# graphic-goose/ferreus_rbf_rs

Measured on AMD Instinct MI355X. Metric: BBFMM matvecs/s, higher is better.
Workload: dtype f64; 1 GPU; 10000000 uniform 3D points, LinearRbf, order 7, 1 rhs, adaptive sparse tree, ACA eps=1e-7, set_weights + evaluate at the sources; points=10000000, kernel=LinearRbf, order=7, nrhs=1, parallelism=single GPU

## Files before the change

### ferreus_rbf_rs_amd/_lib.py

```python
from __future__ import annotations

import ctypes
import os

HERE = os.path.dirname(os.path.abspath(__file__))
LIB_PATH = os.environ.get("FERREUS_BBFMM_HIP_LIB") or os.path.join(HERE, "libferreus_bbfmm_hip.so")

OK, POINT_OUTSIDE_TREE, KERNEL_NO_GRADIENTS, BAD_ARGUMENT, DEVICE_ERROR, UNSUPPORTED, CALLBACK_FAILED = range(7)
FLAG_HOST_ONLY = 1
FLAG_M2L_SHARED_BASIS = 2
FLAG_DIRECT_SMALL_W_LEAVES = 4
FLAG_DETERMINISTIC = 8
N_PHASES = 11
PHASE_NAMES = ["gather", "P2M", "M2M", "M2L_stage1", "M2L_stage2", "P2L", "L2L", "P2P", "M2P",
               "L2P", "scatter"]

c_i32, c_i64, c_f64, c_u32 = ctypes.c_int32, ctypes.c_int64, ctypes.c_double, ctypes.c_uint32
c_p = ctypes.c_void_p


class Params(ctypes.Structure):
    _fields_ = [("max_points_per_cell", c_i64), ("compression_type", c_i32),
                ("epsilon", c_f64), ("eval_chunk_size", c_i64)]

# ... 40 lines not shown
    "bbfmm_build_isosurfaces_ex": (ctypes.c_int, [c_p, c_p, c_f64, c_p, c_i32, c_p, c_p, c_i64, c_i32, c_p]),
    "bbfmm_isosurfaces_from_values_ex": (ctypes.c_int, [c_p, c_p, c_p, c_f64, c_p, c_i32, c_i64, c_i32, c_p]),
    "bbfmm_isosurface_stats": (ctypes.c_int, [c_p, c_i32, c_p]),
    "bbfmm_build_isosurfaces_opts": (ctypes.c_int, [c_p, c_p, c_f64, c_p, c_i32, c_p, c_p, c_p, c_p]),
    "bbfmm_isosurfaces_from_values_opts": (ctypes.c_int, [c_p, c_p, c_p, c_f64, c_p, c_i32, c_p, c_p]),
    "bbfmm_isosurfaces_from_fields_opts": (ctypes.c_int, [c_p, c_i32, c_p, c_i32, c_p, c_f64, c_p, c_i32, c_p, c_p, c_p]),
    "bbfmm_isosurfaces_from_function_opts": (ctypes.c_int, [c_p, c_p, c_p, c_p, c_f64, c_p, c_i32, c_p, c_p]),
    "bbfmm_debug_evaluate_fields": (ctypes.c_int, [c_p, c_i32, c_p, c_i32, c_p, c_i64, c_i64, c_p, c_p, c_i64]),
    "bbfmm_debug_field_program": (ctypes.c_int, [c_i32, c_i32, c_p, c_p, c_p, c_i32, c_p, c_p, c_i64, c_p, c_p]),
    "bbfmm_isosurface_finish_mesh": (ctypes.c_int, [c_p, c_p, c_i64, c_p, c_i64, c_p, c_p]),
    "bbfmm_isosurface_finish_stats": (ctypes.c_int, [c_p, c_i32, c_p]),
    "bbfmm_isosurface_close_mesh": (ctypes.c_int, [c_p, c_p, c_i64, c_p, c_i64, c_p, ctypes.c_double, c_i32, c_p]),
    "bbfmm_isosurface_closure_stats": (ctypes.c_int, [c_p, c_i32, c_p]),
    "bbfmm_debug_closure_triangulate": (ctypes.c_int, [c_i32, c_i32, c_p, c_p, c_p, c_i64, c_p, c_i64, c_p, c_i64, ctypes.c_double,
                                                       ctypes.c_double, c_i64, c_p, c_p, c_i64, c_p, c_p, c_p, c_i64]),
    "bbfmm_debug_orient2d": (ctypes.c_int, [c_p, c_i64, c_p]),
    "bbfmm_isosurface_follow_stats": (ctypes.c_int, [c_p, c_i32, c_p]),
    "bbfmm_isosurface_follow_times": (ctypes.c_int, [c_p, c_i32, c_p]),
    "bbfmm_isosurface_follow_bricks": (ctypes.c_int, [c_p, c_i32, c_p, c_p]),
    "bbfmm_isosurface_intersection_stats": (ctypes.c_int, [c_p, c_i32, c_p]),
    "bbfmm_isosurface_self_intersections": (ctypes.c_int, [c_p, c_p, c_i64, c_p, c_i64, c_p, c_p]),
    "bbfmm_isosurface_intersection_ids": (ctypes.c_int, [c_p, c_i32, c_p, c_p]),
    "bbfmm_isosurface_triangle_pair": (ctypes.c_int, [c_p, c_p, c_p, c_p, c_p, c_p]),
    "bbfmm_isosurface_clip_triangle": (ctypes.c_int, [c_p, c_p, c_p, c_p, c_p]),
    "bbfmm_isosurface_topology": (ctypes.c_int, [ctypes.c_uint32, c_p, c_p, c_p]),
    "bbfmm_isosurface_cluster_tables": (ctypes.c_int, [c_p, c_p, c_p]),
    "bbfmm_isosurface_curvature_tables": (ctypes.c_int, [c_p, c_p, c_p]),
    "bbfmm_isosurface_curvature_weight": (ctypes.c_int, [c_p, c_p, c_i32, c_p, c_p, c_p, c_p]),
    "bbfmm_isosurface_curvature_stats": (ctypes.c_int, [c_p, c_i32, c_p]),
    "bbfmm_isosurface_count": (c_i32, [c_p]),
    "bbfmm_isosurface_size": (ctypes.c_int, [c_p, c_i32, c_p, c_p]),
    "bbfmm_isosurface_copy": (ctypes.c_int, [c_p, c_i32, c_p, c_p]),
    "bbfmm_isosurface_error": (ctypes.c_char_p, [c_p]),
    "bbfmm_isosurface_destroy": (None, [c_p]),
    "bbfmm_prepare_target_subset": (ctypes.c_int, [c_p, c_p, c_i64]),
    "bbfmm_fast_matrix_vector_product": (ctypes.c_int, [c_p, c_p, c_i64, c_i64, c_p, c_i64, c_p,
                                                        c_i64, c_f64, c_p]),
    "bbfmm_matvec_device": (ctypes.c_int, [c_p, c_p, c_i64, c_i32, c_p, c_i64, c_i32]),
    "bbfmm_target_subset_create": (ctypes.c_int, [c_p, c_p, c_i64, c_p]),
    "bbfmm_matvec_subset_device": (ctypes.c_int, [c_p, c_i32, c_p, c_p, c_i32]),
    "bbfmm_stream": (c_p, [c_p]),
    "bbfmm_set_partition": (ctypes.c_int, [c_p, c_i32, c_i32]),
    "bbfmm_partition_row_count": (c_i64, [c_p]),
    "bbfmm_partition_rows": (ctypes.c_int, [c_p, c_p]),
    "bbfmm_partition_coarse_count": (c_i64, [c_p]),
    "bbfmm_matvec_partition_upward": (ctypes.c_int, [c_p, c_p, c_i64, c_i32, c_p, c_p]),
    "bbfmm_matvec_partition_finish": (ctypes.c_int, [c_p, c_p, c_p, c_i64, c_i32, c_p]),
    "bbfmm_partition_world": (c_i32, [c_p]),
    "bbfmm_partition_rank": (c_i32, [c_p]),
    "bbfmm_partition_bounds": (ctypes.c_int, [c_p, c_i32, c_p]),
    "bbfmm_matvec_partition_finish_sorted": (ctypes.c_int, [c_p, c_p, c_p, c_i64, c_p]),
    "bbfmm_partition_scatter": (ctypes.c_int, [c_p, c_p, c_i32, c_i32, c_i64, c_i32, c_p, c_i64]),
    "bbfmm_debug_partition_upward_counts": (ctypes.c_int, [c_p, c_p, c_p, c_p]),
    "bbfmm_debug_host_copy_rates": (ctypes.c_int, [c_i64, c_p]),
    "bbfmm_get_tree_stats": (ctypes.c_int, [c_p, c_p]),
    "bbfmm_tree_built_on_device": (ctypes.c_int, [c_p]),
    "bbfmm_last_evaluate_at_sources": (ctypes.c_int, [c_p]),
    "bbfmm_debug_targets_are_sources": (ctypes.c_int, [c_p, c_p, c_i64, c_i64]),
    "bbfmm_debug_rows_of_sources": (ctypes.c_int, [c_p, c_p, c_i64, c_i64, c_p]),
    "bbfmm_get_cells": (ctypes.c_int, [c_p, c_p, c_p]),
    "bbfmm_get_leaf_sources": (ctypes.c_int, [c_p, c_p, c_p]),
    "bbfmm_get_list": (ctypes.c_int, [c_p, ctypes.c_char, c_p, c_p, c_p]),
    "bbfmm_get_m2l_ranks": (ctypes.c_int, [c_p, c_p, c_p]),
    "bbfmm_get_m2l_operator": (ctypes.c_int, [c_p, c_i32, c_i32, c_p]),
    "bbfmm_get_m2l_factors": (ctypes.c_int, [c_p, c_i32, c_i32, c_p, c_p]),
    "bbfmm_get_permutation_tables": (ctypes.c_int, [c_p, c_p, c_p, c_p, c_p, c_p]),
    "bbfmm_points_to_leaves": (ctypes.c_int, [c_p, c_p, c_i64, c_i64, c_p, c_p]),
    "bbfmm_set_profiling": (ctypes.c_int, [c_p, c_i32]),
    "bbfmm_get_phase_ms": (ctypes.c_int, [c_p, c_p, c_p]),
    "bbfmm_reset_phase_ms": (ctypes.c_int, [c_p]),
    "bbfmm_mfma_f64_selftest": (ctypes.c_int, [c_p, c_p, c_p]),
    "bbfmm_fp64_valu_selftest": (ctypes.c_int, [c_p, c_p]),
    "bbfmm_debug_kernel_values": (ctypes.c_int, [c_i32, c_i32, ctypes.c_double, ctypes.c_double, c_p, c_i64, c_p, c_p, c_p]),
    "bbfmm_debug_math": (ctypes.c_int, [c_i32, c_i32, c_p, c_i64, c_p, c_p]),
    "bbfmm_debug_dense_m2m": (ctypes.c_int, [c_p, c_i32, c_p]),
    "bbfmm_debug_apply_m2l_tables_host": (ctypes.c_int, [c_p, c_p, c_p]),
    "bbfmm_debug_m2l_variants": (ctypes.c_int, [c_p, c_p, c_p]),
    "bbfmm_debug_m2l_pairs": (ctypes.c_int, [c_p, c_p, c_i64, c_p, c_p]),
    "bbfmm_debug_m2l_pairs_axes": (ctypes.c_int, [c_p, c_p, c_i64, c_p]),
    "bbfmm_debug_m2l_pairs_stage2": (ctypes.c_int, [c_p, c_p, c_i64, c_p, c_p]),
    "bbfmm_debug_m2l_pairs_axes_stage2": (ctypes.c_int, [c_p, c_p, c_i64, c_p]),
    "bbfmm_debug_m2l_table_digests": (ctypes.c_int, [c_p, c_p, c_i32, c_p, c_p, c_i32, c_p]),
    "bbfmm_debug_m2l_s2_last_ksplit": (ctypes.c_int, [c_p, c_p]),
    "bbfmm_debug_m2l_parity_len": (ctypes.c_int, [c_p, c_p]),
    "bbfmm_debug_get_coefficients": (ctypes.c_int, [c_p, ctypes.c_char, c_i32, c_p]),
    "bbfmm_debug_morton_encode": (ctypes.c_uint64, [c_i32, c_p, ctypes.c_uint64]),
    "bbfmm_debug_morton_decode": (None, [c_i32, ctypes.c_uint64, c_p, c_p]),
    "bbfmm_debug_morton_neighbours": (c_i32, [c_i32, ctypes.c_uint64, c_p]),
    "bbfmm_debug_direction_vectors": (c_i32, [c_i32, c_p]),
    "bbfmm_debug_reference_vectors": (ctypes.c_int, [c_p, c_p, c_p]),
    "bbfmm_givens_rotation": (None, [c_f64, c_f64, c_p, c_p, c_p]),
    "bbfmm_fgmres": (ctypes.c_int, [c_i64, c_p, c_p, c_p, c_p, c_p, c_p, c_i32, c_i32, c_i32, c_f64,
                                    c_p, c_p, c_p, c_p, c_p]),
    "bbfmm_schwarz_ddm_solver": (ctypes.c_int, [c_i64, c_p, c_p, c_p, c_p, c_p, c_i32, c_i32, c_f64,
                                                c_p, c_p, c_p, c_p, c_p]),
    "bbfmm_rbf_system_apply": (ctypes.c_int, [c_p, c_p, c_p, c_i64]),
    "bbfmm_rbf_system_device_create": (ctypes.c_int, [c_p, c_i64, c_p, c_i64, c_f64, c_p]),
    "bbfmm_rbf_system_device_destroy": (None, [c_p]),
    "bbfmm_rbf_system_apply_device": (ctypes.c_int, [c_p, c_p, c_p, c_i64, c_p]),
    "bbfmm_fgmres_device": (ctypes.c_int, [c_i64, c_p, c_p, c_p, c_p, c_p, c_p, c_i32, c_i32, c_i32, c_f64,
                                           c_p, c_p, c_p, c_p, c_p, c_p]),
    "bbfmm_schwarz_ddm_solver_device": (ctypes.c_int, [c_i64, c_p, c_p, c_p, c_p, c_p, c_i32, c_i32, c_f64,
                                                       c_p, c_p, c_p, c_p, c_p, c_p]),
    "bbfmm_debug_solver_vector_op": (ctypes.c_int, [c_i32, c_i32, c_i64, c_p, c_p, c_p, c_f64, c_i32, c_p, c_i32, c_p, c_p]),
    "bbfmm_ddm_params_defaults": (None, [c_p]),
    "bbfmm_ddm_params_for_points": (None, [c_i64, c_p]),
    "bbfmm_ddm_build": (ctypes.c_int, [c_p, c_i64, c_i32, c_i64, c_p, c_p]),
    "bbfmm_ddm_destroy": (None, [c_p]),
    "bbfmm_ddm_num_levels": (c_i32, [c_p]),
    "bbfmm_ddm_level_size": (c_i64, [c_p, c_i32]),
    "bbfmm_ddm_level_points": (ctypes.c_int, [c_p, c_i32, c_p]),
    "bbfmm_ddm_num_domains": (c_i64, [c_p, c_i32]),
    "bbfmm_ddm_domain_size": (c_i64, [c_p, c_i32, c_i64]),
    "bbfmm_ddm_domain": (ctypes.c_int, [c_p, c_i32, c_i64, c_p, c_p, c_p]),
    "bbfmm_schwarz_create": (ctypes.c_int, [c_p, c_p, c_i64, c_i32, c_i64, c_p, c_p, c_p]),
    "bbfmm_schwarz_create_sharded": (ctypes.c_int, [c_p, c_p, c_i64, c_i32, c_i64, c_p, c_p, c_i32, c_i32, c_p, c_i64, c_p, c_p, c_p]),
    "bbfmm_schwarz_factor_bytes": (c_i64, [c_p]),
    "bbfmm_schwarz_domains_owned": (c_i64, [c_p, c_i32, ctypes.POINTER(c_i64), ctypes.POINTER(c_i64)]),
    "bbfmm_schwarz_destroy": (None, [c_p]),
    "bbfmm_schwarz_basis_size": (c_i64, [c_p]),
    "bbfmm_schwarz_num_levels": (c_i32, [c_p]),
    "bbfmm_schwarz_monomial_matrix": (c_p, [c_p]),
    "bbfmm_debug_evaluate_monomials": (ctypes.c_int, [c_p, c_i64, c_i32, c_i64, c_i32, c_p, c_p, c_p]),
    "bbfmm_schwarz_apply": (ctypes.c_int, [c_p, c_p, c_p, c_i64]),
    "bbfmm_schwarz_apply_device": (ctypes.c_int, [c_p, c_p, c_p, c_i64, c_p]),
    "bbfmm_schwarz_debug_trace_steps": (c_i32, [c_p]),
    "bbfmm_schwarz_debug_apply_trace": (ctypes.c_int, [c_p, c_p, c_p, c_i64, c_i32, c_p, c_p, c_p, c_p, c_p]),
    "bbfmm_schwarz_debug_ortho_matrix": (c_p, [c_p]),
    "bbfmm_schwarz_level_size": (c_i64, [c_p, c_i32]),
    "bbfmm_schwarz_level_points": (ctypes.c_int, [c_p, c_i32, c_p]),
    "bbfmm_schwarz_debug_level_solve": (ctypes.c_int, [c_p, c_i32, c_p, c_p, c_i64, c_i32]),
    "bbfmm_ddm_debug_level_create": (ctypes.c_int, [c_p, c_i64, c_i32, c_i64, c_i64, c_p, c_p, c_p, c_p, c_i32, c_i32, c_p]),
    "bbfmm_ddm_debug_level_destroy": (None, [c_p]),
    "bbfmm_ddm_debug_level_info": (ctypes.c_int, [c_p, c_p]),
    "bbfmm_ddm_debug_level_layout": (ctypes.c_int, [c_p, c_p, c_p, c_p, c_p, c_p]),
    "bbfmm_ddm_debug_level_assembled": (ctypes.c_int, [c_p, c_p]),
    "bbfmm_ddm_debug_level_factor": (ctypes.c_int, [c_p, c_p]),
    "bbfmm_ddm_debug_level_solve": (ctypes.c_int, [c_p, c_p, c_p, c_i64, c_i32]),
    "bbfmm_schwarz_create_ex": (ctypes.c_int, [c_p, c_p, c_i64, c_i32, c_i64, c_p, c_i64, c_p, c_p, c_p]),
    "bbfmm_schwarz_create_sharded_ex": (ctypes.c_int, [c_p, c_p, c_i64, c_i32, c_i64, c_p, c_i64, c_p, c_p, c_i32, c_i32, c_p, c_i64,
                                                       c_p, c_p, c_p]),
    "bbfmm_ddm_debug_level_create_ex": (ctypes.c_int, [c_p, c_i64, c_i32, c_i64, c_p, c_i64, c_i64, c_p, c_p, c_p, c_p, c_i32, c_i32,
                                                       c_p]),
    "bbfmm_global_trend_transform": (ctypes.c_int, [c_i32, c_p, c_p, c_p, c_p]),
    "bbfmm_duplicate_cutoff_distance": (ctypes.c_int, [c_p, c_f64, c_p]),
    "bbfmm_remove_duplicates": (ctypes.c_int, [c_p, c_i64, c_i32, c_i64, c_f64, c_i32, c_p, c_p, c_p]),
    "bbfmm_debug_interpolant_terms": (ctypes.c_int, [c_i32, c_i32, c_p, c_p, c_i64, c_i64, c_p, c_i64, c_p, c_i64, c_p, c_i64]),
    "bbfmm_evaluate_interpolant": (ctypes.c_int, [c_p, c_i32, c_i32, c_p, c_i64, c_i32, c_i64, c_p, c_i64, c_i64, c_p, c_f64,
                                                  c_p, c_i64, c_p, c_i64, c_p]),
    "bbfmm_evaluate_device": (ctypes.c_int, [c_p, c_i32, c_p, c_i64, c_i64, c_p, c_p, c_i64, c_p, c_i64, c_p, c_p]),
    "bbfmm_evaluate_grid": (ctypes.c_int, [c_p, c_i32, c_p, c_p, c_p, c_i64, c_p, c_i64, c_p, c_p]),
    "bbfmm_evaluate_grid_stats": (ctypes.c_int, [c_p, c_p]),
    "bbfmm_debug_grid_coords": (ctypes.c_int, [c_i32, c_p, c_i64, c_i64, c_p, c_i64]),
    "bbfmm_debug_split_runs": (ctypes.c_int, [c_i32, c_p, c_p, c_p, c_i64, c_i32, c_p, c_p, c_p, c_i64, c_p]),
}


class Interpolant(ctypes.Structure):
    _fields_ = [("kernel_type", c_i32), ("polynomial_degree", c_i32), ("nugget", c_f64), ("base_range", c_f64),
                ("total_sill", c_f64), ("flags", c_u32)]


FLAG_GLOBAL_SCALING = 1


class IsosurfaceOptions(ctypes.Structure):
# ... 77 lines not shown
```

### ferreus_rbf_rs_amd/csrc/capi_debug.cpp

```cpp
#include <algorithm>
#include <chrono>
#include <cstring>
#include <vector>

#include "capi_handle.hpp"
#include "morton.hpp"

namespace {
template <int ID>
void debug_kernel_values_host(const bbfmm::KernelSpec &ks, const double *r2, int64_t n, double *value, double *value_g, double *factor) {
    for (int64_t i = 0; i < n; ++i) {
        value[i] = bbfmm::kernel_value_r2<ID>(ks, r2[i]);
        value_g[i] = bbfmm::kernel_value_grad_r2<ID>(ks, r2[i], &factor[i]);
    }
}
}

extern "C" {

int bbfmm_debug_targets_are_sources(const bbfmm_handle *h, const double *x, int64_t m, int64_t ldx) {
    return (h && h->tree.targets_are_sources(x, m, ldx)) ? 1 : 0;
}
int bbfmm_debug_rows_of_sources(bbfmm_handle *h, const double *x, int64_t m, int64_t ldx, int64_t *rows_out) {
    if (!h || !rows_out) return 0;
// ... 133 lines not shown
}
int32_t bbfmm_debug_direction_vectors(int32_t d, int32_t *out) {
    if (d < 1 || d > 3 || !out) return -1;
    const int(*dirs)[3];
    const int n = bbfmm::direction_vectors(d, &dirs);
    for (int i = 0; i < n; ++i)
        for (int a = 0; a < d; ++a) out[i * d + a] = dirs[i][a];
    return n;
}
int bbfmm_debug_reference_vectors(const bbfmm_handle *h, int32_t *out, int32_t *n_ref_out) {
    if (!h) return BBFMM_BAD_ARGUMENT;
    const bbfmm::Operators &ops = h->tree.ops();
    if (n_ref_out) *n_ref_out = ops.n_ref;
    if (out) std::copy(ops.ref_vecs.begin(), ops.ref_vecs.end(), out);
    return BBFMM_OK;
}

int bbfmm_debug_m2l_variants(const bbfmm_handle *h, int64_t *n_variants, int64_t *n_cells) {
    if (!h) return BBFMM_BAD_ARGUMENT;
    int64_t nv = 0, nc = 0;
    h->tree.m2l_variant_stats(&nv, &nc);
    if (n_variants) *n_variants = nv;
    if (n_cells) *n_cells = nc;
    return BBFMM_OK;
}

int bbfmm_debug_m2l_pairs(const bbfmm_handle *h, int32_t *out, int64_t cap, int64_t *n_out, int32_t *pairs_on) {
    if (!h || !n_out) return BBFMM_BAD_ARGUMENT;
    std::vector<int32_t> v;
    h->tree.debug_m2l_pairs(&v);
    *n_out = static_cast<int64_t>(v.size());
    if (pairs_on) *pairs_on = h->tree.m2l_pairs() ? 1 : 0;
    if (out) std::copy(v.begin(), v.begin() + std::min<int64_t>(cap, *n_out), out);
    return BBFMM_OK;
}

int bbfmm_debug_m2l_pairs_axes(const bbfmm_handle *h, int32_t *out, int64_t cap, int64_t *n_out) {
    if (!h || !n_out) return BBFMM_BAD_ARGUMENT;
    std::vector<int32_t> v;
    h->tree.debug_m2l_pairs_axes(&v);
    *n_out = static_cast<int64_t>(v.size());
    if (out) std::copy(v.begin(), v.begin() + std::min<int64_t>(cap, *n_out), out);
    return BBFMM_OK;
}

int bbfmm_debug_m2l_pairs_stage2(const bbfmm_handle *h, int32_t *out, int64_t cap, int64_t *n_out, int32_t *pairs_on) {
    if (!h || !n_out) return BBFMM_BAD_ARGUMENT;
    std::vector<int32_t> v;
    h->tree.debug_m2l_pairs_stage2(&v);
    *n_out = static_cast<int64_t>(v.size());
    if (pairs_on) *pairs_on = h->tree.m2l_pairs_stage2() ? 1 : 0;
    if (out) std::copy(v.begin(), v.begin() + std::min<int64_t>(cap, *n_out), out);
    return BBFMM_OK;
}

int bbfmm_debug_m2l_pairs_axes_stage2(const bbfmm_handle *h, int32_t *out, int64_t cap, int64_t *n_out) {
    if (!h || !n_out) return BBFMM_BAD_ARGUMENT;
    std::vector<int32_t> v;
    h->tree.debug_m2l_pairs_axes_stage2(&v);
    *n_out = static_cast<int64_t>(v.size());
    if (out) std::copy(v.begin(), v.begin() + std::min<int64_t>(cap, *n_out), out);
    return BBFMM_OK;
}

int bbfmm_debug_m2l_table_digests(const bbfmm_handle *h, uint64_t *digests, int32_t cap, int32_t *n_out, double *flops_level,
                                  int32_t flops_cap, int32_t *n_levels_out) {
    if (!h || !n_out) return BBFMM_BAD_ARGUMENT;
    std::vector<uint64_t> v;
    h->tree.debug_m2l_table_digests(&v);
    *n_out = static_cast<int32_t>(v.size());
    if (digests) std::copy(v.begin(), v.begin() + std::min<int32_t>(cap, *n_out), digests);
    const std::vector<double> &fl = h->tree.m2l_flops_level();
    if (n_levels_out) *n_levels_out = static_cast<int32_t>(fl.size());
    if (flops_level) std::copy(fl.begin(), fl.begin() + std::min<int32_t>(flops_cap, static_cast<int32_t>(fl.size())), flops_level);
    return BBFMM_OK;
}

int bbfmm_debug_m2l_s2_last_ksplit(const bbfmm_handle *h, int32_t *ksplit) {
    if (!h || !ksplit) return BBFMM_BAD_ARGUMENT;
    *ksplit = h->tree.debug_m2l_s2_last_ksplit();
    return BBFMM_OK;
}

int bbfmm_debug_m2l_parity_len(const bbfmm_handle *h, int32_t *len) {
    if (!h || !len) return BBFMM_BAD_ARGUMENT;
    *len = h->tree.debug_m2l_parity_len();
    return BBFMM_OK;
}

int bbfmm_debug_get_coefficients(bbfmm_handle *h, char which, int32_t k, double *out) {
    GUARD(h) return h->tree.debug_get_coefficients(which, k, out);
    END_GUARD(h)
}

}
```

### ferreus_rbf_rs_amd/csrc/device.hpp

```cpp
#pragma once
#include <hip/hip_runtime.h>

#include <cstdint>

#include "kernels.hpp"

namespace bbfmm {

constexpr int kMaxOrder = 16;
constexpr int kM2lTile = 128;
constexpr int kM2lS1Block = 176;
constexpr int kM2lS1BlockPairs = 160;
constexpr int kM2lSlotWindow = 128;
constexpr int kM2lBlkTwoDst = 1 << 30;

struct DevCheb {
    int p, d, n, n_pad;
    double polyn[kMaxOrder * kMaxOrder];
    double nodes[kMaxOrder];
    double xfer[2 * kMaxOrder * kMaxOrder];
};

struct ChebRef {
    const DevCheb *dev;
    int p, d, n, n_pad;
};

struct M2lClass {
    const double *vt_all;
    const int32_t *row_dst;
    const int32_t *row_dst2;
    const int32_t *blk_t0;
    int32_t yb0;
    int32_t n_rows;
    int32_t r_pad16;
    int32_t n_t;
    const double *u_all;
    int32_t k_pad;
    int32_t kp;
    int32_t kpy;
    const int32_t *cells;
    int32_t n_cells;
    const int32_t *cslot;
    const int64_t *cbase;
};

struct M2lTileDesc {
    int32_t level_class;
    int32_t first;
    int32_t count;
    int32_t q_first;
    int32_t q_count;
    int32_t pad;
};

void launch_gather_weights(const double *w, int64_t ldw, int K, const int32_t *order, int64_t N,
                           double *w_sorted, hipStream_t s);
void launch_gather_weights_subset(const double *w, int64_t ldw, int K, const int32_t *order, const int32_t *pos, int64_t n_pos,
                                  int64_t N, double *w_sorted, hipStream_t s);
constexpr int kMaxScatterParts = 64;
struct ScatterParts {
    int n;
    int64_t bound[kMaxScatterParts + 1];
};
void launch_scatter_parts(const double *all, const ScatterParts &parts, int64_t m_max, int K, const int32_t *order, double *out,
                          int64_t ldo, hipStream_t s);
void launch_sum_slots(const double *slots, int n_slots, int64_t len, double *out, hipStream_t s);
void launch_scatter_output(const double *out_sorted, int64_t n, int K, const int32_t *perm,
                           double *out, int64_t ldo, int accumulate, hipStream_t s);
void launch_gather_rows(const double *src, int64_t ld_src, int ncols, const int32_t *idx, int64_t n,
                        double *dst, int64_t ld_dst, hipStream_t s);

void launch_p2m(const ChebRef &ch, const double *const *src_xyz, const double *w_sorted, int64_t N,
                int K, int64_t C, const int32_t *leaf_cells, int n_leaves, const int32_t *pt_begin,
                const int32_t *pt_end, const double *centers, const double *lengths, double *M,
                hipStream_t s);
struct M2lParityRowArgs;
struct M2lUnparityRowArgs;
int launch_m2m(const ChebRef &ch, int K, int64_t C, const int32_t *parents, int n_parents,
               const int64_t *child_ptr, const int32_t *child_idx, const int32_t *octant, double *M,
               hipStream_t s, const M2lParityRowArgs *par = nullptr, double *Mp = nullptr);
bool m2m_writes_parity(const ChebRef &ch);
int launch_l2l(const ChebRef &ch, int K, int64_t C, const int32_t *cells, int n_cells,
               const int32_t *parent, const int32_t *octant, const uint8_t *active, double *L,
               hipStream_t s, const M2lUnparityRowArgs *unp = nullptr, const double *Lp = nullptr,
               const uint8_t *has_m2l = nullptr, const uint8_t *has_x = nullptr);
bool l2l_reads_parity(const ChebRef &ch);
void launch_zero_rows(const int32_t *cells, int n_cells, int n_pad, int K, int64_t C, double *L, hipStream_t s);

void launch_m2l_stage1(const M2lClass *classes, const M2lTileDesc *tiles, const int32_t *tile_idx, int n_tiles,
                       int n_pad, int max_slot_t, int K, int64_t C, const double *M, double *cbuf,
                       int64_t cbuf_len, hipStream_t s, bool own_blocks = false, int max_blocks = 8, int ne16 = 0, int s_ee = 0,
                       int s_eo = 0);
void launch_m2l_parity(const double *M, int n_pad, double *Mp, int n_par, int ne16, int n_e, int n_o, int p, int64_t rows,
                       hipStream_t s);
struct M2lParityOffsets {
    int32_t v[4];
};
void launch_m2l_parity2(const double *M, int n_pad, double *Mp, int n_par, M2lParityOffsets off, int p, int p2, int64_t rows,
                        hipStream_t s);
void launch_m2l_stage2(const M2lClass *classes, const M2lTileDesc *tiles, const int32_t *tile_idx, int n_tiles,
// ... 22 lines not shown
    int p2 = 0;
};

struct M2lUnparityRowArgs {
    int axes = 0;
    int n_par = 0;
    int p = 0;
    int ne16 = 0, n_e = 0, n_o = 0, p1 = 0;
    M2lS2PairsPlan plan{1, 1, 1, 1};
    int p2 = 0;
};
void launch_m2l_parity_cells(const double *M, int n_pad, double *Mp, const M2lParityRowArgs &par, const int32_t *cells, int n_cells,
                             int K, int64_t C, hipStream_t s);
int m2l_s2_pairs_ksplit(int n_tiles, const M2lS2PairsPlan &plan, int K, bool allow_ksplit);
bool launch_m2l_stage2_pairs(const M2lClass *classes, const M2lTileDesc *tiles, const int32_t *tile_idx, int n_tiles,
                             const M2lS2PairsPlan &plan, int K, int64_t C, const double *cbuf, int64_t cbuf_len,
                             const uint16_t *qlist, double *Lp, hipStream_t s, bool allow_ksplit = true, int *ksplit_out = nullptr);
void launch_m2l_unparity(const double *Lp, int n_par, int ne16, double *L, int n, int n_pad, int n_e, int n_o, int p, int64_t rows,
                         hipStream_t s);
void launch_m2l_unparity2(const double *Lp, const M2lS2PairsPlan &plan, double *L, int n, int n_pad, int p, int p2, int64_t rows,
                          hipStream_t s);
void launch_m2l_zero_segments(const int32_t *segs, int64_t n_segs, int K, double *cbuf, int64_t cbuf_len, hipStream_t s);
void launch_m2l_basis(const M2lClass *classes, const M2lTileDesc *tiles, int n_tiles, int in_ld, int out_ld, int K,
                      int64_t C, const double *in, double *out, hipStream_t s);
void launch_small_gemm(bool trans_a, int M, int N, int Kd, const double *A, int64_t lda, const double *B, int64_t ldb,
                       double *Cm, int64_t ldc, hipStream_t s);

struct M2lAssembleTv {
    int32_t perm;
    int32_t rank;
    int32_t row;
    int64_t vt_off;
    int64_t u_off;
};
struct M2lAssembleClass {
    const M2lAssembleTv *src, *tgt;
    int32_t n_src, n_tgt, r_pad16, k_pad, max_rank;
    int32_t n_e, n_o, ne16, n_par, p;
    int32_t u_npar, u_ne16, u_rows, u_ne, u_no;
    int32_t s1_axes;
    M2lParityOffsets s1_off;
    M2lS2PairsPlan u_plan;
};
void launch_m2l_assemble(const M2lAssembleClass &c, int n, int n_pad, bool compressed, const double *ops,
                         const int32_t *invperm, double *vt_all, double *u_all, hipStream_t s);

struct DirectJobs {
    int n_jobs;
    const int32_t *job_cell;
    const int32_t *tgt_begin, *tgt_end;
    const int64_t *run_ptr;
    const int32_t *runs;
};
void launch_p2p(const KernelSpec &ks, int d, const DirectJobs &jobs, const double *const *tgt_xyz,
                int64_t n_tgt, const double *const *src_xyz, const double *w_sorted, int64_t N, int K,
                double *out_sorted, double *grad_sorted, hipStream_t s, bool fixed_plan = false);
constexpr int kSymMaxRhs = 4;
void launch_p2p_sym(const KernelSpec &ks, int n_jobs, const int32_t *tgt_begin, const int32_t *tgt_end,
                    const int64_t *run_range, int n_leaf_jobs, const int32_t *l_tgt_begin, const int32_t *l_tgt_end,
                    const int64_t *l_run_range, int n_wave_jobs, const int32_t *w_tgt_begin, const int32_t *w_tgt_end,
                    const int64_t *w_run_range, const int32_t *runs3, int32_t tgt_off, const double *const *src_xyz,
                    const double *w_sorted, int64_t ldw, int K, double *out_sorted, int64_t ldo, hipStream_t s);
int p2p_sym_rows_per_job();
int p2p_sym3_rows_per_job();
int p2p_sym_wave_rows();
int64_t p2p_sym_wave_min_jobs();
int wx_sym_rows_per_job();
int wx_sym3_rows_per_job();
void launch_wx_sym(const KernelSpec &ks, const ChebRef &ch, int n_jobs, const int32_t *tgt_begin, const int32_t *tgt_end,
                   const int64_t *w_range, int n_leaf_jobs, const int32_t *l_tgt_begin, const int32_t *l_tgt_end,
                   const int64_t *l_w_range, const int32_t *w_cells, const double *centers, const double *lengths,
                   const double *const *src_xyz, const double *w_sorted, int64_t ldw, int K, const double *M, double *L,
                   int64_t ld_ml, double *out_sorted, int64_t ldo, int out_off, int out_n, hipStream_t s);
void launch_m2p(const KernelSpec &ks, const ChebRef &ch, int n_jobs, const int32_t *tgt_begin,
                const int32_t *tgt_end, const int64_t *w_begin, const int64_t *w_end,
                const int32_t *w_cells,
                const double *centers, const double *lengths, const double *const *tgt_xyz,
                int64_t n_tgt, int K, int64_t C, const double *M, double *out_sorted,
                double *grad_sorted, hipStream_t s, bool fixed_plan = false);
void launch_p2l(const KernelSpec &ks, const ChebRef &ch, int n_jobs, const int32_t *cells,
                const int64_t *run_ptr, const int32_t *runs, const double *centers,
                const double *lengths, const double *const *src_xyz, const double *w_sorted,
                int64_t N, int K, int64_t C, double *L, hipStream_t s);
void launch_l2p(const ChebRef &ch, int n_jobs, const int32_t *leaf_cells, const int32_t *tgt_begin,
                const int32_t *tgt_end, const double *centers, const double *lengths,
                const double *const *tgt_xyz, int64_t n_tgt, int K, int64_t C, const double *L,
                double *out_sorted, double *grad_sorted, hipStream_t s, const int32_t *perm = nullptr,
                double *user_out = nullptr, int64_t ldo = 0);

bool l2p_order_supported(int p, int d);

int mfma_f64_selftest(double *tflops, int *layout_errors, double *info);
int valu_f64_selftest(double *tflops, double *mhz);
int debug_kernel_values_device(const KernelSpec &ks, const double *r2, int64_t n, double *value, double *value_g, double *factor);
int debug_math_device(int which, const double *x, int64_t n, double *out, double *out2);

}
```

### ferreus_rbf_rs_amd/csrc/device_common.hpp

```cpp
#pragma once
#include "device.hpp"

#include <algorithm>
#include <atomic>
#include <cstdlib>
#include <type_traits>

namespace bbfmm {

typedef double v4f64 __attribute__((ext_vector_type(4)));

struct Xyz {
    const double *x, *y, *z;
};
inline Xyz make_xyz(const double *const *p) { return Xyz{p[0], p[1], p[2]}; }

__device__ inline void axis_sizes(int p, int d, int &P0, int &P1, int &P2) {
    P0 = p;
    P1 = d > 1 ? p : 1;
    P2 = d > 2 ? p : 1;
}

template <int P, bool GRAD>
__device__ inline void cheb_S_reg(double x, const double *__restrict__ polyn, double (&S)[P], double (&dS)[P]) {
    double T[P], dT[P];
    T[0] = 1.0;
    dT[0] = 0.0;
    if (P > 1) {
        T[1] = x;
        dT[1] = 1.0;
    }
#pragma unroll
    for (int j = 2; j < P; ++j) {
        T[j] = 2.0 * x * T[j - 1] - T[j - 2];
        if (GRAD) dT[j] = 2.0 * T[j - 1] + 2.0 * x * dT[j - 1] - dT[j - 2];
    }
#pragma unroll
    for (int j = 0; j < P; ++j) {
        double s = 0.0, ds = 0.0;
#pragma unroll
        for (int k = 0; k < P; ++k) {
            const double pk = polyn[j * P + k];
            s += T[k] * pk;
            if (GRAD) ds += dT[k] * pk;
        }
        S[j] = (s * 2.0 - 1.0) / (double)P;
        dS[j] = GRAD ? ds * (2.0 / (double)P) : 0.0;
    }
}

inline int env_int(const char *name, int dflt) {
    const char *e = std::getenv(name);
    return e ? std::atoi(e) : dflt;
}

template <int V> using int_c = std::integral_constant<int, V>;

template <class F> inline void dispatch_kernel_id(int id, F &&f) {
    switch (id) {
    case kLinear: f(std::integral_constant<int, kLinear>{}); break;
    case kThinPlateSpline: f(std::integral_constant<int, kThinPlateSpline>{}); break;
    case kCubic: f(std::integral_constant<int, kCubic>{}); break;
    case kSpheroidal3: f(std::integral_constant<int, kSpheroidal3>{}); break;
    case kSpheroidal5: f(std::integral_constant<int, kSpheroidal5>{}); break;
    case kSpheroidal7: f(std::integral_constant<int, kSpheroidal7>{}); break;
    case kSpheroidal9: f(std::integral_constant<int, kSpheroidal9>{}); break;
    case kLaplacian: f(std::integral_constant<int, kLaplacian>{}); break;
    case kOneOverR2: f(std::integral_constant<int, kOneOverR2>{}); break;
    case kOneOverR4: f(std::integral_constant<int, kOneOverR4>{}); break;
    case kGaussianExt: f(std::integral_constant<int, kGaussianExt>{}); break;
    case kMultiquadricExt: f(std::integral_constant<int, kMultiquadricExt>{}); break;
    default: break;
    }
}

template <int LO, int HI, class F> inline bool dispatch_order(int p, F &&f) {
    if constexpr (LO <= HI) {
        if (p != LO) return dispatch_order<LO + 1, HI>(p, f);
        f(std::integral_constant<int, LO>{});
        return true;
    }
    return false;
}

inline int device_cu_count() {
    static std::atomic<int> cache[64];
    int dev = 0;
    if (hipGetDevice(&dev) != hipSuccess) return 256;
    if (dev >= 0 && dev < 64) {
        const int c = cache[dev].load(std::memory_order_relaxed);
        if (c > 0) return c;
    }
    int n_cu = 256;
    if (hipDeviceGetAttribute(&n_cu, hipDeviceAttributeMultiprocessorCount, dev) != hipSuccess || n_cu <= 0) n_cu = 256;
    if (dev >= 0 && dev < 64) cache[dev].store(n_cu, std::memory_order_relaxed);
    return n_cu;
}

inline hipError_t allow_large_dynamic_lds(const void *fn, size_t bytes, std::atomic<uint64_t> *done) {
    if (bytes <= 64 * 1024) return hipSuccess;
    int dev = 0;
    (void)hipGetDevice(&dev);
    const bool cached = dev >= 0 && dev < 256;
    if (cached && ((done[dev >> 6].load(std::memory_order_acquire) >> (dev & 63)) & 1)) return hipSuccess;
    const hipError_t e = hipFuncSetAttribute(fn, hipFuncAttributeMaxDynamicSharedMemorySize, 160 * 1024);
    if (e == hipSuccess && cached) done[dev >> 6].fetch_or(uint64_t(1) << (dev & 63), std::memory_order_release);
    return e;
}

}
```

### ferreus_rbf_rs_amd/csrc/device_l2p.hip

```cpp
#include "device_common.hpp"

namespace bbfmm {

constexpr int L2P_WAVES = 4;
template <int P, int D> constexpr int l2p_waves() { return D == 3 && P > 12 ? (P > 14 ? 1 : 2) : L2P_WAVES; }

template <int P, int D, bool GRAD>
__global__ __launch_bounds__((64 * l2p_waves<P, D>())) void l2p_kernel(const DevCheb *__restrict__ chp, int n_jobs,
                                                             const int32_t *__restrict__ leaf_cells,
                                                             const int32_t *__restrict__ tgt_begin,
                                                             const int32_t *__restrict__ tgt_end,
                                                             const double *__restrict__ centers,
                                                             const double *__restrict__ lengths, Xyz tgt,
                                                             int64_t n_tgt, int K, int64_t C,
                                                             const double *__restrict__ L,
                                                             double *__restrict__ out, double *__restrict__ grad,
                                                             const int32_t *__restrict__ perm, double *__restrict__ user_out,
                                                             int64_t ldo) {
    constexpr int P1 = D > 1 ? P : 1, P2 = D > 2 ? P : 1, N = P * P1 * P2;
    constexpr int WAVES = l2p_waves<P, D>();
    __shared__ double s_L[WAVES][N];
    const int tid = threadIdx.x, wave = tid >> 6, lane = tid & 63;
    __shared__ double s_polyn_lds[GRAD ? P * P : 1];
    if constexpr (GRAD) {
        for (int i = tid; i < P * P; i += 64 * WAVES) s_polyn_lds[i] = chp->polyn[i];
        __syncthreads();
    }
    const double *__restrict__ s_polyn = GRAD ? s_polyn_lds : chp->polyn;
    const int job = blockIdx.x * WAVES + wave;
    if (job >= n_jobs) return;
    const int n_pad = chp->n_pad;
    const int cell = leaf_cells[job];
    const int b = tgt_begin[job], e = tgt_end[job];
    const double len = lengths[cell];
    const double cc[3] = {centers[cell * 3 + 0], centers[cell * 3 + 1], centers[cell * 3 + 2]};
    double *Lw = s_L[wave];
    for (int base = b; base < e; base += 64) {
        const int t = base + lane;
        const bool valid = t < e;
        double S0[P], S1[P1], S2[P2], D0[P], D1[P1], D2[P2];
        {
            const double x0 = valid ? (tgt.x[t] - cc[0]) / (len * 0.5) : 0.0;
            cheb_S_reg<P, GRAD>(x0, s_polyn, S0, D0);
            if (D > 1) {
                const double x1 = valid ? (tgt.y[t] - cc[1]) / (len * 0.5) : 0.0;
                double s[P], d[P];
                cheb_S_reg<P, GRAD>(x1, s_polyn, s, d);
#pragma unroll
                for (int j = 0; j < P1; ++j) { S1[j] = s[j]; D1[j] = d[j]; }
            } else {
                S1[0] = 1.0;
                D1[0] = 0.0;
            }
            if (D > 2) {
                const double x2 = valid ? (tgt.z[t] - cc[2]) / (len * 0.5) : 0.0;
                double s[P], d[P];
                cheb_S_reg<P, GRAD>(x2, s_polyn, s, d);
#pragma unroll
                for (int j = 0; j < P2; ++j) { S2[j] = s[j]; D2[j] = d[j]; }
            } else {
                S2[0] = 1.0;
                D2[0] = 0.0;
            }
        }
        const double gs = 2.0 / len;
        for (int k = 0; k < K; ++k) {
            const double *Lc = L + ((int64_t)k * C + cell) * n_pad;
            for (int I = lane; I < N; I += 64) Lw[I] = Lc[I];
            __builtin_amdgcn_s_waitcnt(0xc07f);
            double y = 0.0, gx = 0.0, gy = 0.0, gz = 0.0;
#pragma unroll
            for (int a = 0; a < P; ++a) {
                double ua = 0.0, uay = 0.0, uaz = 0.0;
#pragma unroll
                for (int bb = 0; bb < P1; ++bb) {
                    double t0 = 0.0, t0z = 0.0;
#pragma unroll
                    for (int c = 0; c < P2; ++c) {
                        const double lv = Lw[(a * P1 + bb) * P2 + c];
                        t0 += S2[c] * lv;
                        if (GRAD) t0z += D2[c] * lv;
                    }
                    ua += S1[bb] * t0;
                    if (GRAD) {
                        uay += D1[bb] * t0;
                        uaz += S1[bb] * t0z;
                    }
                }
                y += S0[a] * ua;
                if (GRAD) {
                    gx += D0[a] * ua;
                    gy += S0[a] * uay;
                    gz += S0[a] * uaz;
                }
            }
            if (valid) {
                if (!GRAD && perm) user_out[(int64_t)k * ldo + perm[t]] = out[(int64_t)k * n_tgt + t] + y;
                else out[(int64_t)k * n_tgt + t] += y;
                if (GRAD) {
                    grad[((int64_t)k * D + 0) * n_tgt + t] += gx * gs;
                    if (D > 1) grad[((int64_t)k * D + 1) * n_tgt + t] += gy * gs;
                    if (D > 2) grad[((int64_t)k * D + 2) * n_tgt + t] += gz * gs;
                }
            }
        }
    }
}

template <int P, int D>
static void l2p_launch_pd(const ChebRef &ch, int n_jobs, const int32_t *leaf_cells, const int32_t *tgt_begin,
                          const int32_t *tgt_end, const double *centers, const double *lengths, Xyz tgt,
                          int64_t n_tgt, int K, int64_t C, const double *L, double *out_sorted, double *grad_sorted,
                          hipStream_t s, const int32_t *perm, double *user_out, int64_t ldo) {
    constexpr int WAVES = l2p_waves<P, D>();
    const int blocks = (n_jobs + WAVES - 1) / WAVES;
    if (grad_sorted)
        hipLaunchKernelGGL((l2p_kernel<P, D, true>), dim3(blocks), dim3(64 * WAVES), 0, s, ch.dev, n_jobs,
                           leaf_cells, tgt_begin, tgt_end, centers, lengths, tgt, n_tgt, K, C, L, out_sorted,
                           grad_sorted, perm, user_out, ldo);
    else
        hipLaunchKernelGGL((l2p_kernel<P, D, false>), dim3(blocks), dim3(64 * WAVES), 0, s, ch.dev, n_jobs,
                           leaf_cells, tgt_begin, tgt_end, centers, lengths, tgt, n_tgt, K, C, L, out_sorted,
                           grad_sorted, perm, user_out, ldo);
}

template <int P>
static void l2p_launch_p(const ChebRef &ch, int n_jobs, const int32_t *leaf_cells, const int32_t *tgt_begin,
                         const int32_t *tgt_end, const double *centers, const double *lengths, Xyz tgt, int64_t n_tgt,
                         int K, int64_t C, const double *L, double *out_sorted, double *grad_sorted, hipStream_t s,
                         const int32_t *perm, double *user_out, int64_t ldo) {
    if (ch.d == 3) {
        l2p_launch_pd<P, 3>(ch, n_jobs, leaf_cells, tgt_begin, tgt_end, centers, lengths, tgt, n_tgt, K, C, L, out_sorted, grad_sorted, s, perm, user_out, ldo);
    } else if (ch.d == 2) {
        l2p_launch_pd<P, 2>(ch, n_jobs, leaf_cells, tgt_begin, tgt_end, centers, lengths, tgt, n_tgt, K, C, L, out_sorted, grad_sorted, s, perm, user_out, ldo);
    } else {
        l2p_launch_pd<P, 1>(ch, n_jobs, leaf_cells, tgt_begin, tgt_end, centers, lengths, tgt, n_tgt, K, C, L, out_sorted, grad_sorted, s, perm, user_out, ldo);
    }
}

bool l2p_order_supported(int p, int d) { return p >= 2 && p <= kMaxOrder && d >= 1 && d <= 3; }

void launch_l2p(const ChebRef &ch, int n_jobs, const int32_t *leaf_cells, const int32_t *tgt_begin,
                const int32_t *tgt_end, const double *centers, const double *lengths, const double *const *tgt_xyz,
                int64_t n_tgt, int K, int64_t C, const double *L, double *out_sorted, double *grad_sorted,
                hipStream_t s, const int32_t *perm, double *user_out, int64_t ldo) {
    if (n_jobs == 0) return;
    if (perm && grad_sorted) return;
    const Xyz tgt = make_xyz(tgt_xyz);
    dispatch_order<2, 16>(ch.p, [&](auto pc) {
        l2p_launch_p<decltype(pc)::value>(ch, n_jobs, leaf_cells, tgt_begin, tgt_end, centers, lengths, tgt, n_tgt, K, C, L,
                                          out_sorted, grad_sorted, s, perm, user_out, ldo);
    });
}

}
```

### ferreus_rbf_rs_amd/csrc/device_p2m.hip

```cpp
#include "device_common.hpp"

namespace bbfmm {

constexpr int P2M_WAVES = 4;
template <int P, int D> constexpr int p2m_waves() { return D == 3 && P > 12 ? 2 : P2M_WAVES; }
constexpr int P2M_PTS = 64;

template <int P, int D, int P2M_KB>
__global__ __launch_bounds__((64 * p2m_waves<P, D>())) void p2m_kernel(const DevCheb *__restrict__ chp, int n_leaves, Xyz src,
                                                             const double *__restrict__ ws, int64_t N, int K,
                                                             int64_t C, const int32_t *__restrict__ leaf_cells,
                                                             const int32_t *__restrict__ pt_begin,
                                                             const int32_t *__restrict__ pt_end,
                                                             const double *__restrict__ centers,
                                                             const double *__restrict__ lengths,
                                                             double *__restrict__ M) {
    constexpr int P1 = D > 1 ? P : 1, P2 = D > 2 ? P : 1, NPAIR = P1 * P2;
    constexpr int NPASS = (NPAIR + 63) / 64;
    constexpr int SROW = 3 * P + P2M_KB;
    __shared__ double s_polyn[P * P];
    constexpr int WAVES = p2m_waves<P, D>();
    __shared__ double s_pts[WAVES][P2M_PTS][SROW];
    const int tid = threadIdx.x, wave = tid >> 6, lane = tid & 63;
    for (int i = tid; i < P * P; i += 64 * WAVES) s_polyn[i] = chp->polyn[i];
    __syncthreads();
    const int job = blockIdx.x * WAVES + wave;
    if (job >= n_leaves) return;
    const int n_pad = chp->n_pad;
    const int cell = leaf_cells[job];
    const int b = pt_begin[cell], e = pt_end[cell];
    const double len = lengths[cell];
    const double cc[3] = {centers[cell * 3 + 0], centers[cell * 3 + 1], centers[cell * 3 + 2]};
    double(*sp)[SROW] = s_pts[wave];
    for (int k0 = 0; k0 < K; k0 += P2M_KB) {
        double acc[NPASS][P2M_KB][P];
#pragma unroll
        for (int ps = 0; ps < NPASS; ++ps)
#pragma unroll
            for (int kk = 0; kk < P2M_KB; ++kk)
#pragma unroll
                for (int i0 = 0; i0 < P; ++i0) acc[ps][kk][i0] = 0.0;
        for (int base = b; base < e; base += P2M_PTS) {
            const int npts = min(P2M_PTS, e - base);
            if (lane < npts) {
                const int pt = base + lane;
                double S[P], dS[P];
                cheb_S_reg<P, false>((src.x[pt] - cc[0]) / (len * 0.5), s_polyn, S, dS);
#pragma unroll
                for (int jx = 0; jx < P; ++jx) sp[lane][jx] = S[jx];
                if (D > 1) {
                    cheb_S_reg<P, false>((src.y[pt] - cc[1]) / (len * 0.5), s_polyn, S, dS);
#pragma unroll
                    for (int jx = 0; jx < P; ++jx) sp[lane][P + jx] = S[jx];
                } else {
                    sp[lane][P] = 1.0;
                }
                if (D > 2) {
                    cheb_S_reg<P, false>((src.z[pt] - cc[2]) / (len * 0.5), s_polyn, S, dS);
#pragma unroll
                    for (int jx = 0; jx < P; ++jx) sp[lane][2 * P + jx] = S[jx];
                } else {
                    sp[lane][2 * P] = 1.0;
                }
#pragma unroll
                for (int kk = 0; kk < P2M_KB; ++kk)
                    sp[lane][3 * P + kk] = (k0 + kk < K) ? ws[(int64_t)(k0 + kk) * N + pt] : 0.0;
            }
            __builtin_amdgcn_s_waitcnt(0xc07f);
#pragma unroll
            for (int ps = 0; ps < NPASS; ++ps) {
                const int q = lane + 64 * ps;
                if (q < NPAIR) {
                    const int i1 = q / P2, i2 = q - i1 * P2;
                    for (int pt = 0; pt < npts; ++pt) {
                        const double *row = sp[pt];
                        const double s12 = row[P + i1] * row[2 * P + i2];
#pragma unroll
                        for (int kk = 0; kk < P2M_KB; ++kk) {
                            const double v = s12 * row[3 * P + kk];
#pragma unroll
                            for (int i0 = 0; i0 < P; ++i0) acc[ps][kk][i0] += v * row[i0];
                        }
                    }
                }
            }
            __builtin_amdgcn_s_waitcnt(0xc07f);
        }
#pragma unroll
        for (int ps = 0; ps < NPASS; ++ps) {
            const int q = lane + 64 * ps;
            if (q < NPAIR) {
#pragma unroll
                for (int kk = 0; kk < P2M_KB; ++kk) {
                    if (k0 + kk < K) {
                        double *Mc = M + ((int64_t)(k0 + kk) * C + cell) * n_pad + q;
#pragma unroll
                        for (int i0 = 0; i0 < P; ++i0) Mc[i0 * NPAIR] = acc[ps][kk][i0];
                    }
                }
            }
        }
    }
}

template <int P>
__global__ __launch_bounds__(64 * P2M_WAVES) void p2m_mfma_kernel(const DevCheb *__restrict__ chp, int n_leaves, Xyz src,
                                                                 const double *__restrict__ ws, int64_t N, int K, int64_t C,
                                                                 const int32_t *__restrict__ leaf_cells,
                                                                 const int32_t *__restrict__ pt_begin,
                                                                 const int32_t *__restrict__ pt_end,
                                                                 const double *__restrict__ centers,
                                                                 const double *__restrict__ lengths, double *__restrict__ M) {
    constexpr int NPAIR = P * P, RB = (P + 3) / 4, G = (NPAIR + 15) / 16;
    constexpr int SROW = 3 * P + 2;
    __shared__ double s_pts[P2M_WAVES][64][SROW];
    const int tid = threadIdx.x, wave = tid >> 6, lane = tid & 63;
    const double *__restrict__ s_polyn = chp->polyn;
    const int job = blockIdx.x * P2M_WAVES + wave;
    if (job >= n_leaves) return;
    const int n_pad = chp->n_pad;
    const int cell = leaf_cells[job];
    const int b = pt_begin[cell], e = pt_end[cell];
    const double len = lengths[cell];
    const double cc[3] = {centers[cell * 3 + 0], centers[cell * 3 + 1], centers[cell * 3 + 2]};
    double(*sp)[SROW] = s_pts[wave];
    const int hi = lane >> 4, blk = (lane >> 2) & 3, lo = lane & 3;
    int o1[G], o2[G];
#pragma unroll
    for (int g = 0; g < G; ++g) {
        const int q = min(16 * g + 4 * blk + lo, NPAIR - 1);
        o1[g] = P + q / P;
        o2[g] = 2 * P + q % P;
    }
    for (int k = 0; k < K; ++k) {
        double acc[RB][G];
#pragma unroll
        for (int rb = 0; rb < RB; ++rb)
#pragma unroll
            for (int g = 0; g < G; ++g) acc[rb][g] = 0.0;
        for (int base = b; base < e; base += 64) {
            const int npts = min(64, e - base);
            if (k == 0 || e - b > 64) {
                double S[P], dS[P];
                const int pt = base + min(lane, npts - 1);
                const bool live = lane < npts;
                cheb_S_reg<P, false>((src.x[pt] - cc[0]) / (len * 0.5), s_polyn, S, dS);
#pragma unroll
                for (int jx = 0; jx < P; ++jx) sp[lane][jx] = live ? S[jx] : 0.0;
                cheb_S_reg<P, false>((src.y[pt] - cc[1]) / (len * 0.5), s_polyn, S, dS);
#pragma unroll
                for (int jx = 0; jx < P; ++jx) sp[lane][P + jx] = live ? S[jx] : 0.0;
                cheb_S_reg<P, false>((src.z[pt] - cc[2]) / (len * 0.5), s_polyn, S, dS);
#pragma unroll
                for (int jx = 0; jx < P; ++jx) sp[lane][2 * P + jx] = live ? S[jx] : 0.0;
            }
            sp[lane][3 * P] = lane < npts ? ws[(int64_t)k * N + base + lane] : 0.0;
            __builtin_amdgcn_s_waitcnt(0xc07f);
            const int nsteps = (npts + 3) >> 2;
            for (int st = 0; st < nsteps; ++st) {
                const double *row = sp[4 * st + hi];
                const double wv = row[3 * P];
                double av[RB], bv[G];
#pragma unroll
                for (int rb = 0; rb < RB; ++rb) av[rb] = 4 * rb + lo < P ? row[4 * rb + lo] * wv : 0.0;
#pragma unroll
                for (int g = 0; g < G; ++g) bv[g] = row[o1[g]] * row[o2[g]];
#pragma unroll
                for (int rb = 0; rb < RB; ++rb)
#pragma unroll
                    for (int g = 0; g < G; ++g) acc[rb][g] = __builtin_amdgcn_mfma_f64_4x4x4f64(av[rb], bv[g], acc[rb][g], 0, 0, 0);
            }
            __builtin_amdgcn_s_waitcnt(0xc07f);
        }
        double *Mc = M + ((int64_t)k * C + cell) * n_pad;
#pragma unroll
        for (int rb = 0; rb < RB; ++rb) {
            const int i0 = 4 * rb + hi;
#pragma unroll
            for (int g = 0; g < G; ++g) {
                const int q = 16 * g + 4 * blk + lo;
                if (i0 < P && q < NPAIR) Mc[i0 * NPAIR + q] = acc[rb][g];
            }
        }
    }
}

template <int P, int D>
static void p2m_launch_pd(const ChebRef &ch, Xyz src, const double *w_sorted, int64_t N, int K, int64_t C,
                          const int32_t *leaf_cells, int n_leaves, const int32_t *pt_begin, const int32_t *pt_end,
                          const double *centers, const double *lengths, double *M, hipStream_t s) {
    constexpr int WAVES = p2m_waves<P, D>();
    const int blocks = (n_leaves + WAVES - 1) / WAVES;
    if constexpr (D == 3 && P >= 4 && P <= 10) {
        hipLaunchKernelGGL((p2m_mfma_kernel<P>), dim3((n_leaves + P2M_WAVES - 1) / P2M_WAVES), dim3(64 * P2M_WAVES), 0, s, ch.dev,
                           n_leaves, src, w_sorted, N, K, C, leaf_cells, pt_begin, pt_end, centers, lengths, M);
        return;
    }
    if (K == 1 || (D == 3 && P > 12))
        hipLaunchKernelGGL((p2m_kernel<P, D, 1>), dim3(blocks), dim3(64 * WAVES), 0, s, ch.dev, n_leaves, src,
                           w_sorted, N, K, C, leaf_cells, pt_begin, pt_end, centers, lengths, M);
    else
        hipLaunchKernelGGL((p2m_kernel<P, D, 2>), dim3(blocks), dim3(64 * WAVES), 0, s, ch.dev, n_leaves, src,
                           w_sorted, N, K, C, leaf_cells, pt_begin, pt_end, centers, lengths, M);
}

void launch_p2m(const ChebRef &ch, const double *const *src_xyz, const double *w_sorted, int64_t N, int K, int64_t C,
                const int32_t *leaf_cells, int n_leaves, const int32_t *pt_begin, const int32_t *pt_end,
                const double *centers, const double *lengths, double *M, hipStream_t s) {
    if (n_leaves == 0) return;
    const Xyz src = make_xyz(src_xyz);
    dispatch_order<2, 16>(ch.p, [&](auto pc) {
        constexpr int P = decltype(pc)::value;
        if (ch.d == 3) p2m_launch_pd<P, 3>(ch, src, w_sorted, N, K, C, leaf_cells, n_leaves, pt_begin, pt_end, centers, lengths, M, s);
        else if (ch.d == 2) p2m_launch_pd<P, 2>(ch, src, w_sorted, N, K, C, leaf_cells, n_leaves, pt_begin, pt_end, centers, lengths, M, s);
        else p2m_launch_pd<P, 1>(ch, src, w_sorted, N, K, C, leaf_cells, n_leaves, pt_begin, pt_end, centers, lengths, M, s);
    });
}

}
```

### ferreus_rbf_rs_amd/csrc/fmm_plans.cpp

```cpp
#include "fmm_tree_impl.hpp"

namespace bbfmm {

static void add_w_jobs(const HostTree &t, int32_t c, int32_t tb, int32_t te, std::vector<int32_t> *wtb,
                       std::vector<int32_t> *wte, std::vector<int64_t> *wb, std::vector<int64_t> *we, bool whole = false) {
    const int64_t kChunk = whole ? std::max<int64_t>(t.w.ptr[c + 1] - t.w.ptr[c], 1) : 8;
    for (int64_t q = t.w.ptr[c]; q < t.w.ptr[c + 1]; q += kChunk) {
        wtb->push_back(tb);
        wte->push_back(te);
        wb->push_back(q);
        we->push_back(std::min(q + kChunk, t.w.ptr[c + 1]));
    }
}

int FmmTree::build_source_target_set() {
    const HostTree &t = tree_;
    TargetSet &ts = src_targets_;
    ts.m = t.n_points;
    for (int a = 0; a < 3; ++a) ts.xyz_ptr[a] = src_ptr_[a];
    ts.perm = d_order_;
    std::vector<int32_t> jc, tb, te, wtb, wte;
    std::vector<int64_t> wb, we;
    for (int32_t c : src_leaves_) {
        jc.push_back(c);
        tb.push_back(static_cast<int32_t>(t.pt_begin[c]));
        te.push_back(static_cast<int32_t>(t.pt_end[c]));
        add_w_jobs(t, c, tb.back(), te.back(), &wtb, &wte, &wb, &we, deterministic_);
    }
    ts.n_jobs = static_cast<int>(jc.size());
    ts.n_w_jobs = static_cast<int>(wtb.size());
    CHK(dupload(&ts.job_cell, jc));
    CHK(dupload(&ts.tgt_begin, tb));
    CHK(dupload(&ts.tgt_end, te));
    CHK(dupload(&ts.w_tgt_begin, wtb));
    CHK(dupload(&ts.w_tgt_end, wte));
    CHK(dupload(&ts.w_begin, wb));
    CHK(dupload(&ts.w_end, we));
    CHK(build_sym_runs(&ts, jc, 0, t.n_points));
    return BBFMM_OK;
}

int FmmTree::build_sym_runs(TargetSet *ts, const std::vector<int32_t> &job_cells, int64_t pb, int64_t pe,
                            const std::vector<uint8_t> *part_active) {
    const HostTree &t = tree_;
    const int64_t max_rows = p2p_sym_rows_per_job(), leaf_rows = p2p_sym3_rows_per_job();
    const int64_t nj_cells = static_cast<int64_t>(job_cells.size());
    int64_t wave_rows = p2p_sym_wave_rows();
    if (wave_rows > 0) {
        int64_t n_wave = 0;
        for (const int32_t c : job_cells) n_wave += (t.pt_end[c] - t.pt_begin[c]) <= wave_rows;
        if (n_wave < p2p_sym_wave_min_jobs()) wave_rows = 0;
    }
    constexpr int64_t kChunkS = 2048;
    const int64_t nch = (nj_cells + kChunkS - 1) / kChunkS;
    struct Part {
        std::vector<int32_t> runs, tb, te, wtb, wte, ltb, lte;
        std::vector<int64_t> range, wrange, lrange;
    };
    std::vector<Part> parts(static_cast<size_t>(std::max<int64_t>(nch, 1)));
    parallel_for_chunks(nj_cells, kChunkS, [&](int64_t lo, int64_t hi) {
        for (int64_t c0 = lo; c0 < hi; c0 += kChunkS) {
            Part &P = parts[static_cast<size_t>(c0 / kChunkS)];
            auto add = [&](int64_t b, int64_t e, int two) {
                if (e <= b) return;
                P.runs.push_back(static_cast<int32_t>(b));
                P.runs.push_back(static_cast<int32_t>(e));
                P.runs.push_back(two);
            };
            for (int64_t j = c0; j < std::min(hi, c0 + kChunkS); ++j) {
                const int32_t c = job_cells[static_cast<size_t>(j)];
                const int64_t a0 = t.pt_begin[c], a1 = t.pt_end[c];
                const int64_t first = static_cast<int64_t>(P.runs.size() / 3);
                add(a0, a1, 0);
                for (int64_t r = u_runs_.ptr[c]; r < u_runs_.ptr[c + 1]; ++r) {
                    const int64_t b = u_runs_.idx[2 * r], e = u_runs_.idx[2 * r + 1];
                    add(b, std::min({e, a0, pb}), 0);
                    add(std::max(b, a1), std::min(e, pe), 1);
                    add(std::max({b, a1, pe}), e, 0);
                }
                const int64_t last = static_cast<int64_t>(P.runs.size() / 3);
                const int64_t na = a1 - a0;
                if (na <= wave_rows) {
                    P.wtb.push_back(static_cast<int32_t>(a0 - pb));
                    P.wte.push_back(static_cast<int32_t>(a1 - pb));
                    P.wrange.push_back(first);
                    P.wrange.push_back(last);
                } else {
                    const int64_t nj = (na + max_rows - 1) / max_rows;
                    for (int64_t i = 0; i < nj; ++i) {
                        P.tb.push_back(static_cast<int32_t>(a0 - pb + na * i / nj));
                        P.te.push_back(static_cast<int32_t>(a0 - pb + na * (i + 1) / nj));
                        P.range.push_back(first);
                        P.range.push_back(last);
                    }
                    if (leaf_rows > 0) {
                        const int64_t nl = (na + leaf_rows - 1) / leaf_rows;
                        for (int64_t i = 0; i < nl; ++i) {
                            P.ltb.push_back(static_cast<int32_t>(a0 - pb + na * i / nl));
                            P.lte.push_back(static_cast<int32_t>(a0 - pb + na * (i + 1) / nl));
                            P.lrange.push_back(first);
                            P.lrange.push_back(last);
                        }
                    }
                }
            }
        }
    });
    std::vector<int64_t> range, wrange, lrange;
    std::vector<int32_t> runs, tb, te, wtb, wte, ltb, lte;
    {
        size_t nr = 0, njobs = 0, nwjobs = 0;
        for (const Part &P : parts) nr += P.runs.size(), njobs += P.tb.size(), nwjobs += P.wtb.size();
        runs.reserve(nr);
        tb.reserve(njobs);
        te.reserve(njobs);
        range.reserve(2 * njobs);
        wtb.reserve(nwjobs);
        wte.reserve(nwjobs);
        wrange.reserve(2 * nwjobs);
        for (const Part &P : parts) {
            const int64_t base = static_cast<int64_t>(runs.size() / 3);
// ... 301 lines not shown
}

int FmmTree::build_target_set_host(const double *x, int64_t m, int64_t ldx, TargetSet *ts, int64_t *bad_point_index,
                                   std::vector<int32_t> *leaves_out) {
    const HostTree &t = tree_;
    std::vector<int32_t> cell(static_cast<size_t>(m));
    const int64_t bad = points_to_leaves(t, x, m, ldx, cell.data());
    if (bad >= 0) {
        if (bad_point_index) *bad_point_index = bad;
        return fail(BBFMM_POINT_OUTSIDE_TREE, "FMM evaluation failed: target point at row " + std::to_string(bad) +
                                                  " lies outside the tree extents");
    }
    const int64_t C = t.n_cells();
    std::vector<int32_t> leaves, jc, tb, te, wtb, wte;
    std::vector<int64_t> wb, we;
    std::vector<int32_t> perm(static_cast<size_t>(m));
    if (m * 8 < C) {
        std::iota(perm.begin(), perm.end(), 0);
        std::stable_sort(perm.begin(), perm.end(), [&](int32_t a, int32_t b) { return cell[a] < cell[b]; });
        for (int64_t i = 0; i < m;) {
            const int32_t c = cell[perm[i]];
            int64_t e = i + 1;
            while (e < m && cell[perm[e]] == c) ++e;
            leaves.push_back(c);
            jc.push_back(c);
            tb.push_back(static_cast<int32_t>(i));
            te.push_back(static_cast<int32_t>(e));
            add_w_jobs(t, c, tb.back(), te.back(), &wtb, &wte, &wb, &we, deterministic_);
            i = e;
        }
    } else {
        std::vector<int64_t> cnt(static_cast<size_t>(C) + 1, 0);
        for (int64_t i = 0; i < m; ++i) ++cnt[cell[i] + 1];
        for (int64_t c = 0; c < C; ++c)
            if (cnt[c + 1] > 0) leaves.push_back(static_cast<int32_t>(c));
        std::vector<int64_t> start(static_cast<size_t>(C), 0);
        int64_t cur = 0;
        for (int32_t c : leaves) {
            start[c] = cur;
            jc.push_back(c);
            tb.push_back(static_cast<int32_t>(cur));
            cur += cnt[c + 1];
            te.push_back(static_cast<int32_t>(cur));
            add_w_jobs(t, c, tb.back(), te.back(), &wtb, &wte, &wb, &we, deterministic_);
        }
        for (int64_t i = 0; i < m; ++i) perm[start[cell[i]]++] = static_cast<int32_t>(i);
    }
    ts->m = m;
    std::vector<double> tmp(static_cast<size_t>(m));
    for (int a = 0; a < 3; ++a) {
        if (a < d_) {
            for (int64_t i = 0; i < m; ++i) tmp[i] = x[a * ldx + perm[i]];
            CHK(tupload(&ts->xyz[a], tmp));
            ts->xyz_ptr[a] = ts->xyz[a].p;
        } else {
            if (static_cast<size_t>(m) > d_zero_axis_.n) {
                CHK(talloc(&ts->xyz[a], static_cast<size_t>(m), true));
                ts->xyz_ptr[a] = ts->xyz[a].p;
            } else {
                ts->xyz_ptr[a] = d_zero_axis_.p;
            }
        }
    }
    CHK(tupload(&ts->perm, perm));
    ts->n_jobs = static_cast<int>(jc.size());
    ts->n_w_jobs = static_cast<int>(wtb.size());
    CHK(tupload(&ts->job_cell, jc));
    CHK(tupload(&ts->tgt_begin, tb));
    CHK(tupload(&ts->tgt_end, te));
    CHK(tupload(&ts->w_tgt_begin, wtb));
    CHK(tupload(&ts->w_tgt_end, wte));
    CHK(tupload(&ts->w_begin, wb));
    CHK(tupload(&ts->w_end, we));
    if (leaves_out) leaves_out->swap(leaves);
    return BBFMM_OK;
}

void FmmTree::free_target_set(TargetSet *ts) {
    for (int a = 0; a < 3; ++a) dfree(&ts->xyz[a]);
    dfree(&ts->perm);
    dfree(&ts->job_cell);
    dfree(&ts->tgt_begin);
    dfree(&ts->tgt_end);
    dfree(&ts->w_tgt_begin);
    dfree(&ts->w_tgt_end);
    dfree(&ts->w_begin);
    dfree(&ts->w_end);
    dfree(&ts->out);
    dfree(&ts->grad);
    dfree(&ts->sym_tb);
    dfree(&ts->sym_te);
    dfree(&ts->sym_ptr);
    dfree(&ts->sym_runs);
    dfree(&ts->symw_tb);
    dfree(&ts->symw_te);
    dfree(&ts->symw_ptr);
    ts->n_symw_jobs = 0;
    dfree(&ts->syml_tb);
    dfree(&ts->syml_te);
    dfree(&ts->syml_ptr);
    ts->n_syml_jobs = 0;
    dfree(&ts->wx_tb);
    dfree(&ts->wx_te);
    dfree(&ts->wx_range);
    ts->n_wx_jobs = 0;
    dfree(&ts->wxl_tb);
    dfree(&ts->wxl_te);
    dfree(&ts->wxl_range);
    ts->n_wxl_jobs = 0;
    ts->sym = false;
}

int FmmTree::build_downward_plan(const std::vector<int32_t> &target_leaves, DownwardPlan *dp, bool restrict_upward,
                                 int64_t own_b, int64_t own_e) {
    const HostTree &t = tree_;
    const int64_t C = t.n_cells();
    dp->active.assign(static_cast<size_t>(C), 0);
    for (int32_t leaf : target_leaves) {
        int32_t c = leaf;
        while (c >= 0 && !dp->active[c]) {
            dp->active[c] = 1;
            c = t.parent[c];
        }
    }
    const std::vector<uint8_t> &active = dp->active;
    std::vector<int32_t> cls_of(static_cast<size_t>(C), -1), pos_of(static_cast<size_t>(C), -1);
    for (size_t lc = 0; lc < m2l_host_.size(); ++lc) {
        const HostM2lClass &hc = m2l_host_[lc];
        for (size_t i = 0; i < hc.cells.size(); ++i) {
            cls_of[hc.cells[i]] = static_cast<int32_t>(lc);
            pos_of[hc.cells[i]] = static_cast<int32_t>(i);
        }
    }
    auto group_of_class = [&](int32_t lc) { return m2l_batches_[static_cast<size_t>(m2l_batch_of_class_[static_cast<size_t>(lc)])].group; };
    std::vector<uint8_t> needed(static_cast<size_t>(C), 0);
    auto flag = [](uint8_t *p) { __atomic_store_n(p, uint8_t(1), __ATOMIC_RELAXED); };
    parallel_for_chunks(C, 4096, [&](int64_t lo, int64_t hi) {
        for (int64_t B = lo; B < hi; ++B) {
            if (!active[B] || t.level[B] < 2 || cls_of[B] < 0) continue;
            const uint8_t bit = static_cast<uint8_t>(1u << group_of_class(cls_of[B]));
            for (int64_t q = t.v.ptr[B]; q < t.v.ptr[B + 1]; ++q) __atomic_fetch_or(&needed[t.v.idx[q]], bit, __ATOMIC_RELAXED);
        }
    });
    dp->tiles2_h.clear();
    dp->tiles1_h.clear();
    dp->tile_idx_h.clear();
    dp->qlist_h.clear();
    const size_t nb = m2l_batches_.size();
    std::vector<std::vector<M2lTileDesc>> t1b(nb), t2b(nb);
    struct SrcOp {
        int32_t dev_class;
        const HostM2lClass *h;
        uint8_t bit;
    };
    std::vector<SrcOp> sops;
    std::vector<std::vector<int32_t>> sops_of_class(m2l_host_.size());
    for (size_t lc = 0; lc < m2l_host_.size(); ++lc) {
        if (m2l_host_[lc].cells.empty()) continue;
        if (m2l_group_ops_[lc].empty()) {
            sops_of_class[lc].push_back(static_cast<int32_t>(sops.size()));
            sops.push_back(SrcOp{static_cast<int32_t>(lc), &m2l_host_[lc], uint8_t(0xff)});
        } else {
            sops_of_class[lc].assign(8, -1);
            for (int32_t v : m2l_group_ops_[lc]) {
                const int32_t dev = static_cast<int32_t>(m2l_host_.size()) + v;
                const int g = m2l_batches_[static_cast<size_t>(m2l_batch_of_class_[static_cast<size_t>(dev)])].group;
// ... 490 lines not shown
```

### ferreus_rbf_rs_amd/csrc/fmm_tree.cpp

```cpp
#include "fmm_tree_impl.hpp"
#include "interpolant_terms.hpp"

namespace bbfmm {

int FmmTree::fail(int code, const std::string &msg) {
    err_ = msg;
    return code;
}
int FmmTree::hip_fail(hipError_t e, const char *what) {
    err_ = std::string("HIP error: ") + hipGetErrorString(e) + " in " + what;
    return BBFMM_DEVICE_ERROR;
}

void FmmTree::arena_begin() {
    arena_active_ = true;
    arena_used_ = 0;
    arena_need_ = 0;
}
int FmmTree::arena_end() {
    arena_active_ = false;
    if (arena_need_ > arena_.n) {
        dfree(&arena_);
        CHK(dalloc(&arena_, arena_need_ + arena_need_ / 4));
    }
// ... 251 lines not shown
        }
    }
    if (!tree_built_on_device_)
        build_tree(pts_.data(), n, n, d, center, radius, params_.max_points_per_cell, !sparse, adaptive, &tree_);
    timer.lap("tree + interaction lists");
    if ((flags & BBFMM_FLAG_DIRECT_SMALL_W_LEAVES) && adaptive) {
        int64_t n_nodes = 1;
        for (int a = 0; a < d; ++a) n_nodes *= order;
        const int64_t moved = direct_small_w_leaves(&tree_, n_nodes);
        if (std::getenv("BBFMM_VERBOSE"))
            std::fprintf(stderr, "[bbfmm] direct small W leaves: %lld W-list entries became near field\n", static_cast<long long>(moved));
        timer.lap("W leaves -> near field");
    }
    precompute_operators(order, d, radius, tree_.depth, kernel_, params_.compression_type, params_.epsilon, &ops_);
    timer.lap("operators (ACA/SVD)");

    const HostTree &t = tree_;
    const int64_t C = t.n_cells();
    level_cells_.assign(t.depth + 1, {});
    m2m_parents_.assign(t.depth + 1, {});
    for (int64_t c = 0; c < C; ++c) {
        level_cells_[t.level[c]].push_back(static_cast<int32_t>(c));
        if (t.children.ptr[c + 1] > t.children.ptr[c]) m2m_parents_[t.level[c]].push_back(static_cast<int32_t>(c));
        if (t.is_leaf[c] && t.pt_end[c] > t.pt_begin[c]) src_leaves_.push_back(static_cast<int32_t>(c));
    }
    std::sort(src_leaves_.begin(), src_leaves_.end(),
              [&](int32_t a, int32_t b) { return t.pt_begin[a] < t.pt_begin[b]; });
    u_runs_.ptr.assign(C + 1, 0);
    x_runs_.ptr.assign(C + 1, 0);
    {
        constexpr int64_t kChunkR = 4096;
        const int64_t nch = (C + kChunkR - 1) / kChunkR;
        std::vector<std::vector<int32_t>> ub(static_cast<size_t>(nch)), xb(static_cast<size_t>(nch));
        parallel_for_chunks(C, kChunkR, [&](int64_t lo, int64_t hi) {
            for (int64_t c0 = lo; c0 < hi; c0 += kChunkR) {
                auto &uu = ub[static_cast<size_t>(c0 / kChunkR)];
                auto &xx = xb[static_cast<size_t>(c0 / kChunkR)];
                for (int64_t c = c0; c < std::min(hi, c0 + kChunkR); ++c) {
                    const size_t u0 = uu.size(), x0 = xx.size();
                    merged_runs(t, t.u.idx.data() + t.u.ptr[c], t.u.ptr[c + 1] - t.u.ptr[c], &uu);
                    merged_runs(t, t.x.idx.data() + t.x.ptr[c], t.x.ptr[c + 1] - t.x.ptr[c], &xx);
                    u_runs_.ptr[c + 1] = static_cast<int64_t>((uu.size() - u0) / 2);
                    x_runs_.ptr[c + 1] = static_cast<int64_t>((xx.size() - x0) / 2);
                }
            }
        });
        for (int64_t c = 0; c < C; ++c) {
            if (x_runs_.ptr[c + 1] > 0) x_cells_.push_back(static_cast<int32_t>(c));
            u_runs_.ptr[c + 1] += u_runs_.ptr[c];
            x_runs_.ptr[c + 1] += x_runs_.ptr[c];
        }
        u_runs_.idx.resize(static_cast<size_t>(2 * u_runs_.ptr[C]));
        x_runs_.idx.resize(static_cast<size_t>(2 * x_runs_.ptr[C]));
        parallel_for(nch, 1, [&](int64_t ch) {
            const int64_t c0 = ch * kChunkR;
            std::copy(ub[static_cast<size_t>(ch)].begin(), ub[static_cast<size_t>(ch)].end(), u_runs_.idx.begin() + 2 * u_runs_.ptr[c0]);
            std::copy(xb[static_cast<size_t>(ch)].begin(), xb[static_cast<size_t>(ch)].end(), x_runs_.idx.begin() + 2 * x_runs_.ptr[c0]);
        });
    }
    part_rows_.clear();
    timer.lap("run lists");

    CHK(build_m2l_tables());
    timer.lap("stacked M2L tables");
    if (!host_only_) {
        CHK(upload());
        CHK(build_source_target_set());
        HIPCHK(hipStreamSynchronize(stream_));
        timer.lap("upload");
    }
    return BBFMM_OK;
}

int FmmTree::upload() {
    const HostTree &t = tree_;
    const int d = d_;
    const int64_t N = t.n_points, C = t.n_cells();
    DevCheb hc{};
    hc.p = order_;
    hc.d = d;
    hc.n = ops_.n;
    hc.n_pad = round_up(ops_.n, 32);
    std::copy(ops_.polyn.begin(), ops_.polyn.end(), hc.polyn);
    std::copy(ops_.nodes.begin(), ops_.nodes.end(), hc.nodes);
    std::copy(ops_.xfer.begin(), ops_.xfer.end(), hc.xfer);
    CHK(dalloc(&d_cheb_, 1));
    HIPCHK(hipMemcpy(d_cheb_.p, &hc, sizeof hc, hipMemcpyHostToDevice));
    cheb_ = ChebRef{d_cheb_.p, hc.p, hc.d, hc.n, hc.n_pad};

    CHK(dalloc(&d_zero_axis_, static_cast<size_t>(N), true));
    if (dev_points_.order && dev_points_.n == N) {
        for (int a = 0; a < 3; ++a) {
            if (a < d) {
                CHK(dalloc(&d_src_[a], static_cast<size_t>(N)));
                src_ptr_[a] = d_src_[a].p;
            } else {
                src_ptr_[a] = d_zero_axis_.p;
            }
        }
        launch_gather_targets(dev_points_.xyz[0], dev_points_.xyz[1], dev_points_.xyz[2],
                              reinterpret_cast<const int32_t *>(dev_points_.order), N, d > 0 ? d_src_[0].p : nullptr,
                              d > 1 ? d_src_[1].p : nullptr, d > 2 ? d_src_[2].p : nullptr, stream_);
        d_order_.p = reinterpret_cast<int32_t *>(dev_points_.order);
        d_order_.n = static_cast<size_t>(N);
        owned_.push_back(dev_points_.order);
        dev_points_.order = nullptr;
        HIPCHK(hipStreamSynchronize(stream_));
        free_dev_tree_points(&dev_points_);
    } else {
        std::vector<double> tmp(static_cast<size_t>(N));
        for (int a = 0; a < 3; ++a) {
            if (a < d) {
                const double *col = &pts_[static_cast<size_t>(a) * N];
                parallel_for(N, 1 << 16, [&](int64_t i) { tmp[i] = col[t.order[i]]; });
                CHK(dupload(&d_src_[a], tmp));
                src_ptr_[a] = d_src_[a].p;
            } else {
                src_ptr_[a] = d_zero_axis_.p;
            }
        }
        std::vector<int32_t> ord(static_cast<size_t>(N));
        for (int64_t i = 0; i < N; ++i) ord[i] = static_cast<int32_t>(t.order[i]);
        CHK(dupload(&d_order_, ord));
    }
    {
        std::vector<double> c3(static_cast<size_t>(C) * 3, 0.0);
        for (int64_t c = 0; c < C; ++c)
            for (int a = 0; a < d; ++a) c3[c * 3 + a] = t.centers[c * d + a];
        CHK(dupload(&d_centers_, c3));
        CHK(dupload(&d_lengths_, t.lengths));
        std::vector<int32_t> b(C), e(C);
        for (int64_t c = 0; c < C; ++c) {
            b[c] = static_cast<int32_t>(t.pt_begin[c]);
            e[c] = static_cast<int32_t>(t.pt_end[c]);
        }
        CHK(dupload(&d_pt_begin_, b));
        CHK(dupload(&d_pt_end_, e));
        CHK(dupload(&d_parent_, t.parent));
        CHK(dupload(&d_octant_, t.octant));
        CHK(dupload(&d_child_ptr_, t.children.ptr));
        CHK(dupload(&d_child_idx_, t.children.idx));
        CHK(dupload(&d_src_leaves_, src_leaves_));
    }
    d_m2m_parents_.resize(level_cells_.size());
    d_level_cells_.resize(level_cells_.size());
    for (size_t l = 0; l < level_cells_.size(); ++l) {
        CHK(dupload(&d_m2m_parents_[l], m2m_parents_[l]));
        CHK(dupload(&d_level_cells_[l], level_cells_[l]));
    }
    CHK(dupload(&d_u_run_ptr_, u_runs_.ptr));
    CHK(dupload(&d_u_runs_, u_runs_.idx));
    CHK(dupload(&d_w_ptr_, t.w.ptr));
    CHK(dupload(&d_w_idx_, t.w.idx));
    {
        std::vector<int64_t> job_ptr(x_cells_.size() + 1, 0);
        std::vector<int32_t> job_runs;
        for (size_t j = 0; j < x_cells_.size(); ++j) {
            const int32_t c = x_cells_[j];
            for (int64_t r = x_runs_.ptr[c]; r < x_runs_.ptr[c + 1]; ++r) {
                job_runs.push_back(x_runs_.idx[2 * r]);
                job_runs.push_back(x_runs_.idx[2 * r + 1]);
            }
            job_ptr[j + 1] = static_cast<int64_t>(job_runs.size() / 2);
        }
        CHK(dupload(&d_x_cells_, x_cells_));
        CHK(dupload(&d_x_job_run_ptr_, job_ptr));
// ... 54 lines not shown
                const int ref = ops_.ref_lookup[tv];
                const int rank = lops[ref].rank;
                src_tv.push_back(M2lAssembleTv{ops_.perm_lookup[tv], rank, h.src_row0[pos], vt_off[h.level][ref], u_off[h.level][ref]});
            }
            for (size_t pos = 0; pos < h.tgt_tv.size(); ++pos) {
                if (m2l_pairs2_ && h.tgt_pair[pos] == -2) continue;
                const int tv = h.tgt_tv[pos];
                const int ref = ops_.ref_lookup[tv];
                const int rank = lops[ref].rank;
                max_rank = std::max(max_rank, rank);
                const int row = m2l_pairs2_ && h.tgt_pair[pos] < 0 ? h.tgt_off[pos] - h.kp : h.tgt_off[pos];
                tgt_tv.push_back(M2lAssembleTv{ops_.perm_lookup[tv], rank, row, vt_off[h.level][ref], u_off[h.level][ref]});
            }
            DevBuf<M2lAssembleTv> d_src, d_tgt;
            CHK(dupload(&d_src, src_tv));
            CHK(dupload(&d_tgt, tgt_tv));
            const M2lAssembleClass ac{d_src.p, d_tgt.p, static_cast<int32_t>(src_tv.size()), static_cast<int32_t>(tgt_tv.size()),
                                      h.r_pad16, h.k_pad, max_rank,
                                      m2l_pairs_ ? m2l_ne_ : 0, m2l_no_, m2l_ne16_, m2l_npar_, ops_.p,
                                      m2l_pairs2_ ? m2l_s2_plan_.n_par() : 0, m2l_s2_plan_.ne16(), h.k_pad - h.kp, m2l_ne_, m2l_no_,
                                      m2l_axes_, m2l_s1_off_, m2l_pairs2_ && m2l_s2_axes_ == 2 ? m2l_s2_plan_ : M2lS2PairsPlan{1, 1, 1, 1}};
            static const bool host_fill = std::getenv("BBFMM_M2L_ASSEMBLE_HOST") != nullptr;
            if (host_fill) {
                std::vector<double> hv, hu;
                fill_m2l_operator_arrays(h, &hv, &hu);
                HIPCHK(hipMemcpy(vt.p, hv.data(), hv.size() * sizeof(double), hipMemcpyHostToDevice));
                HIPCHK(hipMemcpy(ua.p, hu.data(), hu.size() * sizeof(double), hipMemcpyHostToDevice));
            } else {
                launch_m2l_assemble(ac, ops_.n, cheb_.n_pad, compressed, d_level_ops[h.level].p, d_invperm.p, vt.p, ua.p, stream_);
            }
            assemble_tmp.push_back(d_src);
            assemble_tmp.push_back(d_tgt);
            if (shared_basis_) {
                DevBuf<double> vt2, ua2;
                CHK(dalloc(&vt2, static_cast<size_t>(m2l_len) * h.r_pad16));
                CHK(dalloc(&ua2, static_cast<size_t>(h.k_pad) * m2l_len));
                const double *W = d_basis_c_[static_cast<size_t>(h.level)].p;
                launch_small_gemm(true, m2l_len, h.r_pad16, cheb_.n_pad, W, m2l_len, vt.p, h.r_pad16, vt2.p, h.r_pad16, stream_);
                launch_small_gemm(false, h.k_pad, m2l_len, cheb_.n_pad, ua.p, cheb_.n_pad, W, m2l_len, ua2.p, m2l_len, stream_);
                natural_tmp.push_back(vt);
                natural_tmp.push_back(ua);
                vt = vt2;
                ua = ua2;
            }
        }
        CHK(dupload(&rt, h.row_dst));
        CHK(dupload(&rt2, h.row_dst2));
        CHK(dupload(&ro, h.blk_t0));
        CHK(dupload(&ce, h.cells));
        CHK(dalloc(&cs, h.cslot.size()));
        if (!h.cslot.empty()) HIPCHK(hipMemcpy(cs.p, h.cslot.data(), h.cslot.size() * sizeof(int32_t), hipMemcpyHostToDevice));
        CHK(dupload(&cb, h.cbase));
        c.vt_all = vt.p;
        c.u_all = ua.p;
        c.row_dst = rt.p;
        c.row_dst2 = rt2.p;
        c.blk_t0 = ro.p;
        c.cells = ce.p;
        c.cslot = cs.p;
        c.cbase = cb.p;
        decltype(h.cslot)().swap(h.cslot);
    }
    HIPCHK(hipStreamSynchronize(stream_));
    HIPCHK(hipGetLastError());
    for (auto &b : assemble_tmp) dfree(&b);
    for (auto &b : natural_tmp) dfree(&b);
    for (auto &b : d_level_ops) dfree(&b);
    dfree(&d_invperm);
    ut.lap("  upload: M2L operators, tables");
    CHK(dupload(&d_m2l_classes_, m2l_classes_h_));
    CHK(dupload(&d_m2l_tiles_, m2l_tiles_h_));
    CHK(dupload(&d_m2l_tiles1_, m2l_tiles1_h_));
    CHK(dupload(&d_tile_idx1_, m2l_tile_idx1_h_));
    CHK(dupload(&d_m2l_tiles2_, m2l_tiles2_h_));
    CHK(dupload(&d_m2l_zero_, m2l_zero_h_));
    decltype(m2l_zero_h_)().swap(m2l_zero_h_);
    CHK(dupload(&d_m2l_qlist_, m2l_qlist_h_));
    std::vector<uint8_t> act(static_cast<size_t>(C), 1);
    CHK(dupload(&d_active_, act));
    {
        const char *e = std::getenv("BBFMM_FUSED_PASSES");
        fused_mask_ = e ? static_cast<unsigned>(std::atoi(e)) & 15u : 15u;
        if (!(fused_mask_ & 2u)) fused_mask_ &= ~4u;
        std::vector<uint8_t> has_m2l(static_cast<size_t>(C), 0), has_x(static_cast<size_t>(C), 0);
        fused_flags_ok_ = true;
        for (const M2lTileDesc &td : m2l_tiles2_h_) {
            const size_t lc = static_cast<size_t>(td.level_class);
            const HostM2lClass &h = lc < m2l_host_.size() ? m2l_host_[lc] : m2l_variants_[lc - m2l_host_.size()];
            if (td.pad != 0 || td.first < 0 || static_cast<size_t>(td.first) + td.count > h.cells.size()) {
                fused_flags_ok_ = false;
                break;
            }
            for (int32_t q = 0; q < td.count; ++q) has_m2l[static_cast<size_t>(h.cells[static_cast<size_t>(td.first + q)])] = 1;
        }
        for (int32_t c : x_cells_) has_x[static_cast<size_t>(c)] = 1;
        CHK(dupload(&d_has_m2l_, has_m2l));
        CHK(dupload(&d_has_x_, has_x));
        std::vector<int32_t> top;
        for (size_t l = 0; l < level_cells_.size() && l < 2; ++l) top.insert(top.end(), level_cells_[l].begin(), level_cells_[l].end());
        n_top_cells_ = static_cast<int>(top.size());
        CHK(dupload(&d_top_cells_, top));
    }
    return BBFMM_OK;
}

M2lParityRowArgs FmmTree::mp_row_args() const {
    M2lParityRowArgs a;
    a.axes = m2l_axes_;
    a.n_par = m2l_npar_;
    a.p = ops_.p;
    a.ne16 = m2l_ne16_;
    a.n_e = m2l_ne_;
    a.n_o = m2l_no_;
    a.p1 = m2l_ne_ / ((ops_.p + 1) / 2);
    a.off = m2l_s1_off_;
    a.p2 = ops_.n / (ops_.p * ops_.p);
    return a;
}

M2lUnparityRowArgs FmmTree::lp_row_args() const {
    M2lUnparityRowArgs a;
    a.axes = m2l_s2_axes_;
    a.n_par = m2l_s2_plan_.n_par();
    a.p = ops_.p;
    a.ne16 = m2l_s2_plan_.ne16();
    a.n_e = m2l_ne_;
    a.n_o = m2l_no_;
    a.p1 = m2l_ne_ / ((ops_.p + 1) / 2);
    a.plan = m2l_s2_plan_;
    a.p2 = ops_.n / (ops_.p * ops_.p);
    return a;
}

bool FmmTree::m2m_fusable() const {
    return (fused_mask_ & 1u) && m2l_pairs_ && !m2l_batches_.empty() && !shared_basis_ && ops_.d == 3 && ops_.p == cheb_.p &&
           m2m_writes_parity(cheb_);
}

bool FmmTree::l2l_fusable(int k) const {
    return (fused_mask_ & 2u) && fused_flags_ok_ && m2l_pairs2_ && !m2l_batches_.empty() && !shared_basis_ && ops_.d == 3 &&
           ops_.p == cheb_.p && l2l_reads_parity(cheb_) && k <= m2l_rhs_chunk_;
}

int FmmTree::ensure_rhs_capacity(int k) {
    if (k <= k_cap_) return BBFMM_OK;
    const int64_t N = tree_.n_points, C = tree_.n_cells();
    pin_w_k_ = 0;
    dfree(&d_w_sorted_);
    dfree(&d_M_);
    dfree(&d_L_);
    dfree(&d_cbuf_);
    dfree(&d_out_);
    dfree(&src_targets_.out);
    dfree(&src_targets_.grad);
    const size_t coef = static_cast<size_t>(k) * C * cheb_.n_pad;
    CHK(dalloc(&d_w_sorted_, static_cast<size_t>(k) * N));
    CHK(dalloc(&d_M_, coef, true));
    CHK(dalloc(&d_L_, coef, true));
    if (m2l_pairs_) {
        dfree(&d_Mp_);
        CHK(dalloc(&d_Mp_, static_cast<size_t>(k) * C * m2l_npar_, true));
        mp_current_k_ = 0;
    }
    if (shared_basis_) {
        dfree(&d_Mc_);
        dfree(&d_Lc_);
// ... 378 lines not shown
    if (t.adaptive && wx) {
        launch_wx_sym(kernel_, cheb_, wx->n_wx_jobs, wx->wx_tb.p, wx->wx_te.p, wx->wx_range.p, wx->n_wxl_jobs, wx->wxl_tb.p, wx->wxl_te.p,
                      wx->wxl_range.p, d_w_idx_.p, d_centers_.p,
                      d_lengths_.p, src_ptr_, d_w_sorted_.p, t.n_points, k, d_M_.p, d_L_.p, C * cheb_.n_pad, wx->out.p,
                      static_cast<int64_t>(wx->m), wx->sym_off, static_cast<int>(wx->m), stream_);
    } else if (t.adaptive) {
        if (dp)
            launch_p2l(kernel_, cheb_, dp->n_x_jobs, dp->d_x_cells.p, dp->d_x_ptr.p, dp->d_x_runs.p, d_centers_.p,
                       d_lengths_.p, src_ptr_, d_w_sorted_.p, t.n_points, k, C, d_L_.p, stream_);
        else
            launch_p2l(kernel_, cheb_, static_cast<int>(x_cells_.size()), d_x_cells_.p, d_x_job_run_ptr_.p,
                       d_x_runs_.p, d_centers_.p, d_lengths_.p, src_ptr_, d_w_sorted_.p, t.n_points, k, C, d_L_.p,
                       stream_);
    }
    phase_end(kPhP2L);
    phase_begin();
    for (int level = 2; level <= t.depth; ++level) {
        const int rc = launch_l2l(cheb_, k, C, d_level_cells_[level].p, static_cast<int>(level_cells_[level].size()), d_parent_.p,
                                  d_octant_.p, dp ? dp->d_active.p : d_active_.p, d_L_.p, stream_, fuse_lp ? &lp_args : nullptr,
                                  fuse_lp ? d_Lp_.p : nullptr, fuse_lp ? d_has_m2l_.p : nullptr, fuse_lp ? d_has_x_.p : nullptr);
        if (rc != 0) return hip_fail(static_cast<hipError_t>(rc), "L2L: dynamic LDS attribute");
    }
    phase_end(kPhL2L);
    HIPCHK(hipGetLastError());
    have_locals_ = dp == nullptr;
    return BBFMM_OK;
}

hipError_t FmmTree::columns_to_host(double *dst, int64_t ld, const double *d_src, int64_t m, int ncols) {
    if (m <= 0 || ncols <= 0) return hipSuccess;
    if (ld == m) return hipMemcpyAsync(dst, d_src, static_cast<size_t>(m) * ncols * sizeof(double), hipMemcpyDeviceToHost, stream_);
    for (int j = 0; j < ncols; ++j) {
        const hipError_t e = hipMemcpyAsync(dst + static_cast<size_t>(j) * ld, d_src + static_cast<size_t>(j) * m,
                                            static_cast<size_t>(m) * sizeof(double), hipMemcpyDeviceToHost, stream_);
        if (e != hipSuccess) return e;
    }
    return hipSuccess;
}

int FmmTree::leaf_pass(const TargetSet &ts, int k, bool with_grads, bool fixed_plan) {
    CHK(leaf_pass_near(ts, k, with_grads, stream_, 3, false, fixed_plan));
    return leaf_pass_far(ts, k, with_grads);
}

int FmmTree::leaf_pass_near(const TargetSet &ts, int k, bool with_grads, hipStream_t st, int parts, bool wx_done,
                            bool fixed_plan) {
    const HostTree &t = tree_;
    const int64_t C = t.n_cells();
    double *grad = with_grads ? ts.grad.p : nullptr;
    const bool timed = st == stream_;
    if (parts & 1) {
        if (!wx_done)
            HIPCHK(hipMemsetAsync(ts.out.p, 0, static_cast<size_t>(k) * ts.m * sizeof(double), st));
        if (with_grads) HIPCHK(hipMemsetAsync(grad, 0, static_cast<size_t>(k) * d_ * ts.m * sizeof(double), st));
        DirectJobs jobs{ts.n_jobs, ts.job_cell.p, ts.tgt_begin.p, ts.tgt_end.p, d_u_run_ptr_.p, d_u_runs_.p};
        static const bool sym_on = [] {
            const char *e = std::getenv("BBFMM_P2P_SYM");
            return !e || std::atoi(e) != 0;
        }();
        if (timed) phase_begin();
        if (ts.sym && sym_on && !deterministic_ && !with_grads)
            launch_p2p_sym(kernel_, ts.n_sym_jobs, ts.sym_tb.p, ts.sym_te.p, ts.sym_ptr.p, ts.n_syml_jobs, ts.syml_tb.p, ts.syml_te.p,
                           ts.syml_ptr.p, ts.n_symw_jobs, ts.symw_tb.p, ts.symw_te.p,
                           ts.symw_ptr.p, ts.sym_runs.p, ts.sym_off, src_ptr_, d_w_sorted_.p, t.n_points, k, ts.out.p, ts.m, st);
        else
            launch_p2p(kernel_, d_, jobs, ts.xyz_ptr, ts.m, src_ptr_, d_w_sorted_.p, t.n_points, k, ts.out.p, grad, st,
                       fixed_plan);
        if (timed) phase_end(kPhP2P);
    }
    if (parts & 2) {
        if (timed) phase_begin();
        if (t.adaptive && !wx_done)
            launch_m2p(kernel_, cheb_, ts.n_w_jobs, ts.w_tgt_begin.p, ts.w_tgt_end.p, ts.w_begin.p, ts.w_end.p,
                       d_w_idx_.p, d_centers_.p, d_lengths_.p, ts.xyz_ptr, ts.m, k, C, d_M_.p, ts.out.p, grad, st, fixed_plan);
        if (timed) phase_end(kPhM2P);
    }
    HIPCHK(hipGetLastError());
    return BBFMM_OK;
}

int FmmTree::leaf_pass_far(const TargetSet &ts, int k, bool with_grads, double *user_out, int64_t ldo) {
    const int64_t C = tree_.n_cells();
    double *grad = with_grads ? ts.grad.p : nullptr;
    phase_begin();
    launch_l2p(cheb_, ts.n_jobs, ts.job_cell.p, ts.tgt_begin.p, ts.tgt_end.p, d_centers_.p, d_lengths_.p, ts.xyz_ptr,
               ts.m, k, C, d_L_.p, ts.out.p, grad, stream_, user_out ? ts.perm.p : nullptr, user_out, ldo);
    phase_end(kPhL2P);
    HIPCHK(hipGetLastError());
    return BBFMM_OK;
}

int FmmTree::set_weights(const double *w, int64_t rows, int k, int64_t ldw) {
    if (host_only_) return fail(BBFMM_DEVICE_ERROR, "handle was created with BBFMM_FLAG_HOST_ONLY");
    part_pending_k_ = 0;
    pin_w_k_ = 0;
    static const bool verbose = std::getenv("BBFMM_VERBOSE") != nullptr;
    const auto t_0 = std::chrono::steady_clock::now();
    CHK(put_weights(w, rows, k, ldw));
    const auto t_1 = std::chrono::steady_clock::now();
    nrhs_ = k;
    have_locals_ = locals_requested_ = false;
    CHK(upward(k));
    const auto t_2 = std::chrono::steady_clock::now();
    HIPCHK(hipStreamSynchronize(stream_));
    if (verbose) {
        const auto t_3 = std::chrono::steady_clock::now();
        auto ms = [](auto a, auto b) { return std::chrono::duration<double, std::milli>(b - a).count(); };
        std::fprintf(stderr, "[bbfmm] set_weights: weights staged and their copies queued %.3f ms, upward pass queued %.3f ms, waited for the device %.3f ms\n",
                     ms(t_0, t_1), ms(t_1, t_2), ms(t_2, t_3));
    }
    return BBFMM_OK;
}

static const char kPartialMultipoles[] =
    "the multipoles are one partition's share (bbfmm_matvec_partition_upward ran last): bbfmm_set_weights must be called first";

int FmmTree::set_local_coefficients(const double *w, int64_t rows, int k, int64_t ldw) {
    if (host_only_) return fail(BBFMM_DEVICE_ERROR, "handle was created with BBFMM_FLAG_HOST_ONLY");
    part_pending_k_ = 0;
    if (nrhs_ == 0) return fail(BBFMM_BAD_ARGUMENT, "set_weights must be called first");
    if (multipoles_partial_) return fail(BBFMM_BAD_ARGUMENT, kPartialMultipoles);
    if (k != nrhs_) return fail(BBFMM_BAD_ARGUMENT, "weights must have the column count given to set_weights");
    CHK(put_weights(w, rows, k, ldw));
    CHK(downward(k));
    HIPCHK(hipStreamSynchronize(stream_));
    locals_requested_ = true;
    return BBFMM_OK;
}

int FmmTree::evaluate(const double *w, int64_t rows, int k, int64_t ldw, const double *x, int64_t m, int64_t ldx,
                      double *out, int64_t ldo, double *grad, int64_t ldg, bool with_grads, bool leaves_only,
                      int64_t *bad_point_index) {
    if (host_only_) return fail(BBFMM_DEVICE_ERROR, "handle was created with BBFMM_FLAG_HOST_ONLY");
    part_pending_k_ = 0;
    if (nrhs_ == 0) return fail(BBFMM_BAD_ARGUMENT, "set_weights must be called first");
    if (multipoles_partial_) return fail(BBFMM_BAD_ARGUMENT, kPartialMultipoles);
    if (k != nrhs_) return fail(BBFMM_BAD_ARGUMENT, "weights must have the column count given to set_weights");
    if (m < 0 || (m > 0 && (!x || !out || ldx < m || ldo < m))) return fail(BBFMM_BAD_ARGUMENT, "bad target/output arrays");
    if (with_grads && m > 0 && (!grad || ldg < m)) return fail(BBFMM_BAD_ARGUMENT, "bad gradient array");
    if (leaves_only && !have_locals_) return fail(BBFMM_BAD_ARGUMENT, "set_local_coefficients must be called first");
    if (m >= (int64_t(1) << 31)) return fail(BBFMM_BAD_ARGUMENT, "more than 2^31-1 target points");
    static const bool verbose = std::getenv("BBFMM_VERBOSE") != nullptr;
    const auto t_begin = std::chrono::steady_clock::now();
    static const bool sources_fast = [] {
        const char *e = std::getenv("BBFMM_EVAL_SOURCES_FAST");
        return !e || std::atoi(e) != 0;
    }();
    bool m2l_queued = false;
    last_eval_at_sources_ = false;
    if (sources_fast && !leaves_only && !with_grads && !have_part_ && !locals_requested_ && m == tree_.n_points && src_targets_.m == m && w && rows >= m &&
        ldw >= rows && static_cast<size_t>(2) * k * m <= kMaxPinnedDoubles) {
        CHK(ensure_rhs_capacity(k));
        CHK(downward_m2l(k, nullptr));
        m2l_queued = true;
        if (targets_are_sources(x, m, ldx)) {
            const int64_t N = m;
            const TargetSet &ts = src_targets_;
            const auto t_cmp = std::chrono::steady_clock::now();
            CHK(put_weights(w, rows, k, ldw));
            const auto t_put = std::chrono::steady_clock::now();
            static const bool wx_on = [] {
                const char *e = std::getenv("BBFMM_WX_FUSED");
                const char *e2 = std::getenv("BBFMM_P2P_SYM");
                return (!e || std::atoi(e) != 0) && (!e2 || std::atoi(e2) != 0);
            }();
            const bool wx = wx_on && !deterministic_ && ts.sym && ts.n_wx_jobs > 0;
            if (wx) HIPCHK(hipMemsetAsync(ts.out.p, 0, static_cast<size_t>(k) * ts.m * sizeof(double), stream_));
            CHK(downward_tail(k, nullptr, wx ? &ts : nullptr));
            CHK(leaf_pass_near(ts, k, false, stream_, 3, wx));
// ... 636 lines not shown
```

### ferreus_rbf_rs_amd/csrc/fmm_tree.hpp

```cpp
#pragma once
#include <hip/hip_runtime.h>

#include <cstdint>
#include <string>
#include <memory>
#include <vector>

#include "device.hpp"
#include "targets.hpp"
#include "ferreus_bbfmm_hip.h"
#include "kernels.hpp"
#include "operators.hpp"
#include "parallel.hpp"
#include "tree.hpp"
#include "tree_device.hpp"

namespace bbfmm {

enum Phase {
    kPhGather = 0, kPhP2M, kPhM2M, kPhM2L1, kPhM2L2, kPhP2L, kPhL2L, kPhP2P, kPhM2P, kPhL2P, kPhScatter,
    kNumPhases
};
static_assert(kNumPhases == BBFMM_N_PHASES, "phase table");

template <class T> struct DevBuf {
    T *p = nullptr;
    size_t n = 0;
    bool borrowed = false;
};

struct HostM2lClass {
    int level = 0, octant = 0;
    int n_rows = 0, r_pad16 = 16, n_t = 0, k_pad = 16;
    std::vector<double> vt_all, u_all;
    std::vector<int> src_tv, tgt_tv, tgt_off;
    std::vector<int32_t> row_tpos, row_off, row_dst, blk_t0, cells;
    std::vector<int32_t, DefaultInitAllocator<int32_t>> cslot;
    std::vector<int32_t> src_row0, src_row1;
    std::vector<int32_t> row_tpos2, row_off2, row_dst2;
    std::vector<int32_t> src_pair;
    std::vector<int8_t> src_kind;
    int yb0 = 0;
    int pad_cols = 0;
    int kp = 0;
    std::vector<int32_t> tgt_pair;
    std::vector<int8_t> tgt_kind;
    int kpy = 0;
    int tgt_pad = 0;
    std::vector<int64_t> cbase;
};

struct M2lBatch {
    int level_lo = 0, level_hi = 0;
    int groups = 1, group = 0;
    int64_t len = 0;
    int32_t t1_first = 0, t1_count = 0;
    int32_t t2_first = 0, t2_count = 0;
};

struct TargetSet {
    int64_t m = 0;
    DevBuf<double> xyz[3];
    const double *xyz_ptr[3] = {nullptr, nullptr, nullptr};
    DevBuf<int32_t> perm;
    DevBuf<int32_t> job_cell, tgt_begin, tgt_end;
    int n_jobs = 0;
    DevBuf<int32_t> w_tgt_begin, w_tgt_end;
    DevBuf<int64_t> w_begin, w_end;
    int n_w_jobs = 0;
    DevBuf<double> out, grad;
    bool sym = false;
    int32_t sym_off = 0;
    int n_sym_jobs = 0;
    DevBuf<int32_t> sym_tb, sym_te;
    DevBuf<int64_t> sym_ptr;
    DevBuf<int32_t> sym_runs;
    int n_syml_jobs = 0;
    DevBuf<int32_t> syml_tb, syml_te;
    DevBuf<int64_t> syml_ptr;
    int n_symw_jobs = 0;
    DevBuf<int32_t> symw_tb, symw_te;
    DevBuf<int64_t> symw_ptr;
    int n_wx_jobs = 0;
    DevBuf<int32_t> wx_tb, wx_te;
    DevBuf<int64_t> wx_range;
    int n_wxl_jobs = 0;
    DevBuf<int32_t> wxl_tb, wxl_te;
    DevBuf<int64_t> wxl_range;
};

struct DownwardPlan {
    std::vector<uint8_t> active;
    std::vector<M2lTileDesc> tiles2_h;
    std::vector<M2lTileDesc> tiles1_h;
    std::vector<int32_t> batch_t1, batch_t2;
    int64_t n_tiles1_blocks = 0;
    std::vector<int32_t> tile_idx_h;
    std::vector<uint16_t> qlist_h;
    int n_x_jobs = 0;
    bool restrict_upward = false;
    int coarse_level = 0;
    int64_t coarse_cells = 0;
    std::vector<int32_t> up_leaves_h;
    std::vector<std::vector<int32_t>> up_parents_h;
    std::vector<int64_t> part_child_ptr_h;
    std::vector<int32_t> part_child_idx_h;
    std::vector<uint8_t> reads_h;
    std::vector<int32_t> gather_pos_h;
    DevBuf<int32_t> d_gather_pos;
    DevBuf<int32_t> d_up_leaves;
    std::vector<DevBuf<int32_t>> d_up_parents;
    DevBuf<int64_t> d_part_child_ptr;
    DevBuf<int32_t> d_part_child_idx;
    DevBuf<uint8_t> d_active;
    DevBuf<M2lTileDesc> d_tiles2, d_tiles1;
    DevBuf<int32_t> d_tile_idx, d_x_cells, d_x_runs;
    DevBuf<int64_t> d_x_ptr;
    DevBuf<uint16_t> d_qlist;
};

struct TargetSetStats {
    int64_t runs = 0, jobs = 0, largest = 0, w_jobs = 0;
};

struct SubsetPlan {
    uint64_t key = 0;
    int64_t n_idx = 0;
    std::vector<int64_t> idx;
    uint64_t last_use = 0;
    TargetSet ts;
    DownwardPlan dp;
};

class DeviceGroup;
struct InterpolantTerms;

class FmmTree {
    friend class DeviceGroup;
  public:
    FmmTree() = default;
    ~FmmTree();
    FmmTree(const FmmTree &) = delete;
    FmmTree &operator=(const FmmTree &) = delete;

    int create(const double *pts, int64_t n, int d, int64_t ld, int order, int kernel_type, double base_range,
               double total_sill, bool adaptive, bool sparse, const double *extents, const bbfmm_params *params,
               uint32_t flags);
    int set_weights(const double *w, int64_t rows, int k, int64_t ldw);
    int set_local_coefficients(const double *w, int64_t rows, int k, int64_t ldw);
    int evaluate_leaves_device(const double *d_x0, const double *d_x1, const double *d_x2, int64_t m, double *d_out,
                               int64_t *bad_point_index, double *d_grad = nullptr, bool batch_independent = false);
    int evaluate_device(const double *d_x, int64_t m, int64_t ldx, const InterpolantTerms *terms, double *d_values, int64_t ldo,
                        double *d_grad, int64_t ldg, bool batch_independent, int32_t max_job_targets, int64_t *bad_point_index,
                        TargetSetStats *stats = nullptr);
    int nrhs() const { return nrhs_; }
    bool supports_gradients() const;
    int evaluate(const double *w, int64_t rows, int k, int64_t ldw, const double *x, int64_t m, int64_t ldx,
                 double *out, int64_t ldo, double *grad, int64_t ldg, bool with_grads, bool leaves_only,
                 int64_t *bad_point_index);
    int prepare_target_subset(const int64_t *target_indices, int64_t n_target_indices);
    bool is_identity_subset(const int64_t *idx, int64_t n_idx) const;
    int fast_matrix_vector_product(const double *w, int64_t rows, int64_t basis_size, const int64_t *target_indices,
                                   int64_t n_target_indices, const double *poly, int64_t ldp, double nugget,
                                   double *result);
    int matvec_device(const double *d_w, int64_t ldw, int k, double *d_out, int64_t ldo, bool sync);
    int64_t partition_coarse_count() const;
    int matvec_partition_upward(const double *d_w, int64_t ldw, int k, double *d_coarse, hipStream_t comm_stream, bool near_field = true);
    int partition_subset_finish(const double *d_coarse, const int64_t *idx, int64_t n_idx, double *h_out, hipStream_t comm_stream);
    int matvec_partition_finish(const double *d_coarse, double *d_out, int64_t ldo, bool sync, hipStream_t comm_stream);
    int matvec_partition_finish_sorted(const double *d_coarse, double *d_seg, int64_t ld, hipStream_t comm_stream);
    int partition_scatter(const double *d_all, int first_part, int n_parts, int64_t m_max, int k, double *d_out, int64_t ldo);
    int matvec_partition_finish_host(const double *d_coarse, double *h_seg, int64_t ld, hipStream_t comm_stream);
    const std::vector<int64_t> &partition_bounds() const { return part_bounds_; }
    int register_subset(const int64_t *idx, int64_t n_idx, int *id_out);
    int matvec_subset_device(int id, const double *d_w, double *d_y, bool sync);
    int set_partition(int rank, int world);

    const HostTree &tree() const { return tree_; }
    const Operators &ops() const { return ops_; }
    const PodDoubles &source_points() const { return pts_; }
    int order() const { return order_; }
    const char *last_error() const { return err_.c_str(); }
    hipStream_t stream() const { return stream_; }
    bool host_only() const { return host_only_; }
    bool deterministic() const { return deterministic_; }
    bool leaves_ready() const { return nrhs_ == 1 && have_locals_; }
    void bind_device() const {
        if (device_ >= 0) (void)hipSetDevice(device_);
    }
    int device() const { return device_; }
    bool tree_built_on_device() const { return tree_built_on_device_; }
    bool last_evaluate_at_sources() const { return last_eval_at_sources_; }
    int last_evaluate_path() const { return last_eval_at_sources_ ? 1 : (last_eval_rows_of_sources_ ? 2 : 0); }
    bool targets_are_rows_of_sources(const double *x, int64_t m, int64_t ldx, std::vector<int64_t> *rows);
    bool targets_are_sources(const double *x, int64_t m, int64_t ldx) const;
    void stats(bbfmm_tree_stats *out) const;
    void set_profiling(bool on) { profiling_ = on; }
    const double *phase_ms() { collect_phase_times(); return phase_ms_; }
    const int64_t *phase_count() { collect_phase_times(); return phase_count_; }
    void reset_phase_ms() {
        collect_phase_times();
        for (double &v : phase_ms_) v = 0.0;
        for (int64_t &v : phase_count_) v = 0;
    }
    const std::vector<int64_t> &partition_rows() const { return part_rows_; }
    bool partitioned() const { return part_world_ > 1; }
    int partition_rank() const { return part_rank_; }
    const std::vector<HostM2lClass> &m2l_host() const { return m2l_host_; }
    void m2l_variant_stats(int64_t *n_variants, int64_t *n_cells) const {
        *n_variants = static_cast<int64_t>(m2l_variants_.size());
        *n_cells = 0;
        for (const HostM2lClass &v : m2l_variants_) *n_cells += static_cast<int64_t>(v.cells.size());
    }
    void debug_m2l_pairs(std::vector<int32_t> *out) const;
    bool m2l_pairs() const { return m2l_pairs_; }
    void debug_m2l_pairs_axes(std::vector<int32_t> *out) const;
    void debug_m2l_pairs_stage2(std::vector<int32_t> *out) const;
    bool m2l_pairs_stage2() const { return m2l_pairs2_; }
    void debug_m2l_pairs_axes_stage2(std::vector<int32_t> *out) const;
    static constexpr int kM2lDigestFamilies = 8;
    void debug_m2l_table_digests(std::vector<uint64_t> *out) const;
    const std::vector<double> &m2l_flops_level() const { return m2l_flops_level_; }
    int debug_m2l_s2_last_ksplit() const { return m2l_s2_last_ksplit_; }
    int debug_apply_m2l_tables_host(const double *M, double *L) const;
    int debug_get_coefficients(char which, int k, double *out);
    int debug_m2l_parity_len() const { return m2l_pairs_ ? m2l_npar_ : 0; }
    int debug_partition_upward_counts(int64_t *counts_out, uint8_t *reads_out, int64_t *info_out) const;

  private:
    int fail(int code, const std::string &msg);
    int hip_fail(hipError_t e, const char *what);
    int upload();
    int build_m2l_tables();
    struct M2lSwitches;
    struct M2lLists;
    struct M2lSlotLayout;
    struct M2lPairSplit;
    struct M2lStage1Marks;
    struct M2lTargetOrder;
    struct M2lLevel;
    struct M2lBuildState;
    void clear_m2l_tables();
    void init_m2l_parity_basis(const M2lSwitches &sw);
    std::vector<int32_t> m2l_reflection_partners(int axis) const;
    M2lPairSplit m2l_split_pairs(const std::vector<int> &list, bool with_y) const;
    void m2l_order_stage1(bool with_y, std::vector<int> *list, std::vector<int> *carry) const;
    M2lStage1Marks m2l_mark_stage1(int level, int axes, const std::vector<int> &tvs) const;
    M2lTargetOrder m2l_target_order(const std::vector<std::vector<int>> &tgt, int axes) const;
    M2lSlotLayout m2l_slot_layout(int level, const M2lTargetOrder &order) const;
    std::vector<uint8_t> m2l_classes_present(int level) const;
    void choose_m2l_stage1_axes(const M2lSwitches &sw, M2lLists *lists);
    void choose_m2l_stage2_axes(const M2lSwitches &sw, M2lLists *lists, std::vector<M2lSlotLayout> *layouts);
    void plan_m2l_batches(const M2lSwitches &sw, const std::vector<M2lSlotLayout> &layouts, M2lLists *lists);
    int build_m2l_level(const M2lLevel &lv, const M2lSwitches &sw, M2lBuildState *st);
    void sort_m2l_class_cells(const M2lLevel &lv, M2lBuildState *st);
    bool m2l_stage1_rows(const M2lLevel &lv, int o, const std::vector<int> &tvs, HostM2lClass *hc);
    int fill_m2l_classes(const M2lLevel &lv);
    void fill_m2l_cslot(const M2lLevel &lv, M2lBuildState *st);
    void m2l_zero_segments(const M2lLevel &lv, M2lBuildState *st) const;
    void m2l_stage2_tiles(const M2lLevel &lv);
    bool m2l_restricted_operator(const M2lLevel &lv, const HostM2lClass &hc, const std::vector<int> &tvs, const std::vector<int> &keep,
                                 size_t first, size_t count, HostM2lClass *v);
    int m2l_group_operators(const M2lLevel &lv, M2lBuildState *st);
    int m2l_boundary_variants(const M2lLevel &lv, const M2lSwitches &sw, M2lBuildState *st);
    int finish_m2l_launch_lists(const M2lLists &lists, const M2lBuildState &st);
    void fill_m2l_operator_arrays(const HostM2lClass &hc, std::vector<double> *vt_all,
                                  std::vector<double> *u_all) const;
    void fill_m2l_operator_arrays(const HostM2lClass &hc, double *vt_all, double *u_all) const;
    int ensure_rhs_capacity(int k);
    int upward(int k, const DownwardPlan *dp = nullptr);
    int downward(int k, const DownwardPlan *dp = nullptr, const TargetSet *wx = nullptr);
    int downward_m2l(int k, const DownwardPlan *dp);
    int downward_tail(int k, const DownwardPlan *dp, const TargetSet *wx);
    int leaf_pass(const TargetSet &ts, int k, bool with_grads, bool fixed_plan = false);
    int leaf_pass_near(const TargetSet &ts, int k, bool with_grads, hipStream_t st, int parts, bool wx_done = false,
                       bool fixed_plan = false);
    int leaf_pass_far(const TargetSet &ts, int k, bool with_grads, double *user_out = nullptr, int64_t ldo = 0);
    int build_target_set(const double *x, int64_t m, int64_t ldx, TargetSet *ts, int64_t *bad_point_index,
                         std::vector<int32_t> *leaves_out = nullptr);
    int build_target_set_device(const double *x, int64_t m, int64_t ldx, TargetSet *ts, int64_t *bad_point_index,
                                std::vector<int32_t> *leaves_out, const double *const *d_x = nullptr, int32_t cap = 0,
                                TargetSetStats *stats = nullptr);
    int ensure_leaf_lookup();
    int build_target_set_host(const double *x, int64_t m, int64_t ldx, TargetSet *ts, int64_t *bad_point_index,
                              std::vector<int32_t> *leaves_out);
    int build_source_target_set();
    int build_sym_runs(TargetSet *ts, const std::vector<int32_t> &job_cells, int64_t pb, int64_t pe, const std::vector<uint8_t> *part_active = nullptr);
    void free_target_set(TargetSet *ts);
    hipError_t columns_to_host(double *dst, int64_t ld, const double *d_src, int64_t m, int ncols);
    int upload_weights(const double *w, int64_t rows, int k, int64_t ldw);
    void phase_begin();
    void phase_end(int ph);
    void collect_phase_times();
    hipEvent_t get_event();

    std::string err_;
    bool host_only_ = false;
    bool deterministic_ = false;
    bool tree_built_on_device_ = false;
    DevTreePoints dev_points_;
    int order_ = 0, d_ = 0;
    KernelSpec kernel_{};
    bbfmm_params params_{};
    PodDoubles pts_;
    HostTree tree_;
    Operators ops_;
    int nrhs_ = 0;
    bool have_locals_ = false;
    bool locals_requested_ = false;
    Csr u_runs_;
    Csr x_runs_;
    std::vector<int32_t> src_leaves_;
    std::vector<std::vector<int32_t>> m2m_parents_;
    std::vector<std::vector<int32_t>> level_cells_;
    std::vector<int32_t> x_cells_;
    std::vector<HostM2lClass> m2l_host_;
    std::vector<HostM2lClass> m2l_variants_;
    std::vector<M2lTileDesc> m2l_tiles1_h_;
    std::vector<int32_t> m2l_tile_idx1_h_;
    std::vector<M2lClass> m2l_classes_h_;
    std::vector<M2lTileDesc> m2l_tiles_h_;
    std::vector<uint16_t> m2l_qlist_h_;
    std::vector<M2lBatch> m2l_batches_;
    std::vector<int32_t> m2l_batch_of_class_;
    std::vector<std::vector<int32_t>> m2l_group_ops_;
    std::vector<int32_t> m2l_zero_h_;
    std::vector<int64_t> m2l_zero_ptr_;
    int64_t cbuf_batch_len_ = 0;
    int64_t cbuf_total_len_ = 0;
    int64_t m2l_budget_bytes_ = int64_t(16384) << 20;
    int m2l_rhs_chunk_ = 1;
    double m2l_flops_k1_ = 0;
    int n_cu_ = 256;
    int device_ = -1;
    std::vector<M2lTileDesc> m2l_tiles2_h_;
    int m2l_slot_t_ = 1;
    int m2l_max_blocks_ = 1;
    int m2l_s1_block_ = kM2lS1Block;
    bool m2l_pairs_ = false;
    int m2l_ne_ = 0, m2l_no_ = 0;
    int m2l_ne16_ = 0, m2l_npar_ = 0;
    std::vector<int32_t> m2l_partner_;
    int m2l_axes_ = 1;
    M2lParityOffsets m2l_s1_off_{{0, 0, 0, 0}};
    int m2l_s_ee_ = 0, m2l_s_eo_ = 0;
    int64_t m2l_work_[2] = {0, 0};
    std::vector<int32_t> m2l_partner_y_;
    std::vector<int32_t> m2l_par_node_;
    std::vector<int8_t> m2l_par_sign_;
    int m2l_rho_y(int m) const {
        const int p2 = ops_.n / (ops_.p * ops_.p);
        return m + (ops_.p - 1 - 2 * ((m / p2) % ops_.p)) * p2;
    }
    int m2l_rho(int m) const {
        const int p1 = ops_.n / ops_.p;
        return m + (ops_.p - 1 - 2 * (m / p1)) * p1;
    }
    DevBuf<double> d_Mp_;
    bool m2l_pairs2_ = false;
    M2lS2PairsPlan m2l_s2_plan_{1, 1, 1, 1};
    DevBuf<double> d_Lp_;
    int m2l_s2_last_ksplit_ = 0;
    int m2l_s2_axes_ = 1;
    int64_t m2l_s2_work_[2] = {0, 0};
    std::vector<int32_t> m2l_s2_node_;
    std::vector<int8_t> m2l_s2_sign_;
    std::vector<int8_t> m2l_s2_part_;
    unsigned fused_mask_ = 15;
    int mp_current_k_ = 0;
    bool lp_pending_ = false;
    bool fused_flags_ok_ = false;
    M2lParityRowArgs mp_row_args() const;
    M2lUnparityRowArgs lp_row_args() const;
    bool m2m_fusable() const;
    bool l2l_fusable(int k) const;
    DevBuf<uint8_t> d_has_m2l_, d_has_x_;
    DevBuf<int32_t> d_top_cells_;
    int n_top_cells_ = 0;
    int part_rank_ = 0, part_world_ = 1;
    std::vector<int64_t> part_rows_, part_bounds_;
    int partition_finish_core(const double *d_coarse, hipStream_t comm_stream, int *k_out);
    bool part_empty_ = false;
    DownwardPlan part_plan_;
    std::vector<std::unique_ptr<SubsetPlan>> subset_plans_;
    uint64_t subset_clock_ = 0;
    int build_downward_plan(const std::vector<int32_t> &target_leaves, DownwardPlan *dp, bool restrict_upward = false,
                            int64_t own_b = 0, int64_t own_e = 0);
    int part_pending_k_ = 0;
    bool multipoles_partial_ = false;
    void free_downward_plan(DownwardPlan *dp);
    int subset_plan(const int64_t *idx, int64_t n_idx, SubsetPlan **out);
    uint64_t subset_key(const int64_t *idx, int64_t n_idx) const;
    bool subset_plan_cached(const int64_t *idx, int64_t n_idx, uint64_t key) const;
    uint64_t last_subset_miss_ = 0;
    int fill_subset_plan(const int64_t *idx, int64_t n_idx, SubsetPlan *sp);
    std::vector<std::unique_ptr<SubsetPlan>> registered_plans_;

    hipStream_t stream_ = nullptr;
    hipEvent_t ev_pack_ = nullptr, ev_comm_ = nullptr;
    struct PendingPhase {
        int phase;
        hipEvent_t e0, e1;
    };
    std::vector<PendingPhase> pending_;
    std::vector<hipEvent_t> event_pool_;
    hipEvent_t pending_begin_ = nullptr;
    bool profiling_ = false;
    double phase_ms_[kNumPhases] = {0};
    int64_t phase_count_[kNumPhases] = {0};
    std::vector<void *> owned_;
    template <class T> int dalloc(DevBuf<T> *b, size_t n, bool zero = false);
    template <class T> int dupload(DevBuf<T> *b, const std::vector<T> &v);
    template <class T> int talloc(DevBuf<T> *b, size_t n, bool zero = false);
    template <class T> int tupload(DevBuf<T> *b, const std::vector<T> &v);
    void arena_begin();
    int arena_end();
    template <class T> void dfree(DevBuf<T> *b);

    ChebRef cheb_{};
    DevBuf<DevCheb> d_cheb_;
    DevBuf<double> d_src_[3];
    const double *src_ptr_[3] = {nullptr, nullptr, nullptr};
    DevBuf<double> d_zero_axis_;
    DevBuf<uint8_t> arena_;
    size_t arena_used_ = 0, arena_need_ = 0;
    bool arena_active_ = false;
    DevBuf<uint64_t> d_tab_keys_;
    DevBuf<int32_t> d_tab_vals_;
    DevBuf<uint8_t> d_is_leaf_;
    DevBuf<uint8_t> d_tscratch_;
    DevLeafLookup lk_;
    bool lk_ready_ = false;
    int64_t device_targets_min_ = 4096;
    DevBuf<int32_t> d_order_;
    DevBuf<double> d_centers_, d_lengths_;
    DevBuf<int32_t> d_pt_begin_, d_pt_end_, d_parent_, d_octant_;
    DevBuf<int64_t> d_child_ptr_;
    DevBuf<int32_t> d_child_idx_;
    DevBuf<int32_t> d_src_leaves_;
    std::vector<DevBuf<int32_t>> d_m2m_parents_, d_level_cells_;
    DevBuf<int64_t> d_u_run_ptr_, d_x_run_ptr_, d_w_ptr_;
    DevBuf<int32_t> d_u_runs_, d_x_runs_, d_w_idx_, d_x_cells_;
    DevBuf<int64_t> d_x_job_run_ptr_;
    DevBuf<M2lClass> d_m2l_classes_;
    DevBuf<M2lTileDesc> d_m2l_tiles_, d_m2l_tiles2_, d_m2l_tiles1_;
    DevBuf<int32_t> d_tile_idx1_;
    DevBuf<int32_t> d_m2l_zero_;
    DevBuf<uint16_t> d_m2l_qlist_;

    DevBuf<uint8_t> d_active_;
    int k_cap_ = 0;
// ... 46 lines not shown
```

### ferreus_rbf_rs_amd/csrc/operators.cpp

```cpp
#include "operators.hpp"

#include <algorithm>
#include <cmath>
#include <cstring>
#include <numeric>

#include "parallel.hpp"

namespace bbfmm {
namespace {

int ipow(int b, int e) {
    int r = 1;
    for (int i = 0; i < e; ++i) r *= b;
    return r;
}

void cheb_T(int p, double x, double *T) {
    T[0] = 1.0;
    if (p > 1) T[1] = x;
    for (int j = 2; j < p; ++j) T[j] = 2.0 * x * T[j - 1] - T[j - 2];
}

inline int cart_index(int i, int j, int base, int ncols) {
// ... 231 lines not shown
        for (int i = 0; i < k - 1; ++i) {
            double *wi = &w[static_cast<size_t>(i) * m];
            for (int j = i + 1; j < k; ++j) {
                double *wj = &w[static_cast<size_t>(j) * m];
                double alpha = 0.0, beta = 0.0, gamma = 0.0;
                for (int r = 0; r < m; ++r) {
                    alpha += wi[r] * wi[r];
                    beta += wj[r] * wj[r];
                    gamma += wi[r] * wj[r];
                }
                if (gamma == 0.0 || std::fabs(gamma) <= eps * std::sqrt(alpha * beta)) continue;
                rotated = true;
                const double zeta = (beta - alpha) / (2.0 * gamma);
                const double t = (zeta >= 0 ? 1.0 : -1.0) / (std::fabs(zeta) + std::sqrt(1.0 + zeta * zeta));
                const double c = 1.0 / std::sqrt(1.0 + t * t), s = c * t;
                for (int r = 0; r < m; ++r) {
                    const double x = wi[r], y = wj[r];
                    wi[r] = c * x - s * y;
                    wj[r] = s * x + c * y;
                }
                double *vi = &v[static_cast<size_t>(i) * k], *vj = &v[static_cast<size_t>(j) * k];
                for (int r = 0; r < k; ++r) {
                    const double x = vi[r], y = vj[r];
                    vi[r] = c * x - s * y;
                    vj[r] = s * x + c * y;
                }
            }
        }
        if (!rotated) break;
    }
    std::vector<double> sig(k);
    for (int j = 0; j < k; ++j) {
        double nn = 0.0;
        const double *wj = &w[static_cast<size_t>(j) * m];
        for (int r = 0; r < m; ++r) nn += wj[r] * wj[r];
        sig[j] = std::sqrt(nn);
    }
    std::vector<int> order(k);
    std::iota(order.begin(), order.end(), 0);
    std::stable_sort(order.begin(), order.end(), [&](int x, int y) { return sig[x] > sig[y]; });
    u_out->assign(static_cast<size_t>(m) * k, 0.0);
    s_out->assign(k, 0.0);
    vt_out->assign(static_cast<size_t>(k) * k, 0.0);
    for (int jj = 0; jj < k; ++jj) {
        const int j = order[jj];
        (*s_out)[jj] = sig[j];
        const double inv = sig[j] > 0.0 ? 1.0 / sig[j] : 0.0;
        for (int r = 0; r < m; ++r) (*u_out)[static_cast<size_t>(jj) * m + r] = w[static_cast<size_t>(j) * m + r] * inv;
        for (int r = 0; r < k; ++r) (*vt_out)[static_cast<size_t>(r) * k + jj] = v[static_cast<size_t>(j) * k + r];
    }
}

void dense_m2m_matrix(const Operators &o, int ci, std::vector<double> *out) {
    const int n = o.n, p = o.p, d = o.d;
    out->assign(static_cast<size_t>(n) * n, 0.0);
    for (int pr = 0; pr < n; ++pr)
        for (int ch = 0; ch < n; ++ch) {
            double v = 1.0;
            for (int a = 0; a < d; ++a) {
                const int ia = cart_index(pr, a, p, d), ca = cart_index(ch, a, p, d);
                const int side = (ci >> a) & 1;
                v *= o.xfer[static_cast<size_t>(side) * p * p + ca * p + ia];
            }
            (*out)[static_cast<size_t>(ch) * n + pr] = v;
        }
}

void precompute_operators(int p, int d, double radius, int depth, const KernelSpec &kernel,
                          int compression, double epsilon, Operators *out) {
    Operators &o = *out;
    o = Operators();
    o.p = p;
    o.d = d;
    const int n = o.n = ipow(p, d);
    o.compression = compression;

    o.nodes.resize(p);
    for (int i = 0; i < p; ++i) {
        const int ii = p - 1 - i;
        o.nodes[i] = std::cos(M_PI * (static_cast<double>(ii) + 0.5) / static_cast<double>(p));
    }
    o.polyn.resize(static_cast<size_t>(p) * p);
    for (int j = 0; j < p; ++j) cheb_T(p, o.nodes[j], &o.polyn[static_cast<size_t>(j) * p]);
    o.nodes_nd.resize(static_cast<size_t>(n) * d);
    for (int i = 0; i < n; ++i)
        for (int a = 0; a < d; ++a) o.nodes_nd[static_cast<size_t>(i) * d + a] = o.nodes[cart_index(i, a, p, d)];

    o.xfer.resize(static_cast<size_t>(2) * p * p);
    for (int row = 0; row < 2 * p; ++row) {
        const double child = (row < p ? o.nodes[row] - 1.0 : o.nodes[row - p] + 1.0) * 0.5;
        double T[64];
        cheb_T(p, child, T);
        for (int j = 0; j < p; ++j) {
            double s = 0.0;
            for (int k = 0; k < p; ++k) s += T[k] * o.polyn[static_cast<size_t>(j) * p + k];
            o.xfer[static_cast<size_t>(row) * p + j] = (s * 2.0 - 1.0) / static_cast<double>(p);
        }
    }

    o.n_vec = ipow(7, d);
    o.all_vecs.resize(static_cast<size_t>(o.n_vec) * d);
    for (int v = 0; v < o.n_vec; ++v)
        for (int a = 0; a < d; ++a) o.all_vecs[static_cast<size_t>(v) * d + a] = cart_index(v, a, 7, d) - 3;
    o.ref_vecs.clear();
    for (int b = 0; b < ipow(4, d); ++b) {
        int row[3];
        for (int a = 0; a < d; ++a) row[a] = cart_index(b, a, 4, d);
        bool valid = row[0] >= 2;
        for (int a = 1; a < d && valid; ++a) valid = row[a] <= row[a - 1];
        if (valid)
            for (int a = 0; a < d; ++a) o.ref_vecs.push_back(row[a]);
    }
    o.n_ref = static_cast<int>(o.ref_vecs.size()) / d;
    permutation_lookups(o);

    o.m2l.assign(static_cast<size_t>(depth) + 1, {});
    for (int level = 2; level <= depth; ++level) o.m2l[level].resize(o.n_ref);
    const int n_tasks = depth >= 2 ? (depth - 1) * o.n_ref : 0;
    parallel_for(n_tasks, 1, [&](int64_t task) {
        const int level = 2 + static_cast<int>(task) / o.n_ref;
        const int ref = static_cast<int>(task) % o.n_ref;
        const double length = radius / static_cast<double>(uint64_t(1) << (level - 1));
        std::vector<double> tp(static_cast<size_t>(n) * d), sp(static_cast<size_t>(n) * d);
        for (int i = 0; i < n; ++i)
            for (int a = 0; a < d; ++a) {
                const double node = o.nodes[cart_index(i, a, p, d)];
                tp[static_cast<size_t>(i) * d + a] = node * (0.5 * length);
                sp[static_cast<size_t>(i) * d + a] =
                    (static_cast<double>(o.ref_vecs[static_cast<size_t>(ref) * d + a]) + node * 0.5) * length;
            }
        auto entry = [&](int i, int j) {
            double r2 = 0.0;
            for (int a = 0; a < d; ++a) {
                const double df = sp[static_cast<size_t>(i) * d + a] - tp[static_cast<size_t>(j) * d + a];
                r2 += df * df;
            }
            return kernel_value_r2_rt(kernel, r2);
        };
        M2lOperator &op = o.m2l[level][ref];
        if (compression == kCompressionAca) {
            std::vector<double> u, v;
            const int k = aca_partial_pivoting(n, n, entry, epsilon, &u, &v);
            std::vector<double> qu, ru, qv, rv;
            thin_qr(u, n, k, &qu, &ru);
            thin_qr(v, n, k, &qv, &rv);
            std::vector<double> core(static_cast<size_t>(k) * k, 0.0);
            for (int c = 0; c < k; ++c)
                for (int r = 0; r < k; ++r) {
                    double s = 0.0;
                    for (int q = 0; q < k; ++q) s += ru[static_cast<size_t>(q) * k + r] * rv[static_cast<size_t>(q) * k + c];
                    core[static_cast<size_t>(c) * k + r] = s;
                }
            std::vector<double> ur, sr, vrt;
            jacobi_svd(core, k, k, &ur, &sr, &vrt);
            const int rank = singular_values_cutoff(sr, epsilon);
            op.rank = rank;
            op.u.assign(static_cast<size_t>(n) * rank, 0.0);
            op.vt.assign(static_cast<size_t>(rank) * n, 0.0);
            for (int c = 0; c < rank; ++c)
                for (int q = 0; q < k; ++q) {
                    const double f = ur[static_cast<size_t>(c) * k + q] * sr[c];
                    const double *quq = &qu[static_cast<size_t>(q) * n];
                    double *uc = &op.u[static_cast<size_t>(c) * n];
                    for (int r = 0; r < n; ++r) uc[r] += quq[r] * f;
                }
            for (int j = 0; j < n; ++j)
// ... 30 lines not shown
```

### ferreus_rbf_rs_amd/csrc/operators.hpp

```cpp
#pragma once
#include <cstdint>
#include <vector>

#include "kernels.hpp"

namespace bbfmm {

enum Compression : int { kCompressionNone = 0, kCompressionSvd = 1, kCompressionAca = 2 };

struct M2lOperator {
    int rank = 0;
    std::vector<double> u;
    std::vector<double> vt;
};

struct Operators {
    int p = 0, d = 0, n = 0;
    std::vector<double> nodes;
    std::vector<double> polyn;
    std::vector<double> nodes_nd;
    std::vector<double> xfer;
    int n_vec = 0;
    int n_ref = 0;
    int n_perm = 0;
    std::vector<int32_t> all_vecs;
    std::vector<int32_t> ref_vecs;
    std::vector<int32_t> perm;
    std::vector<int32_t> invperm;
    std::vector<int32_t> perm_lookup;
    std::vector<int32_t> ref_lookup;
    std::vector<std::vector<M2lOperator>> m2l;
    int compression = kCompressionAca;
};

void precompute_operators(int p, int d, double radius, int depth, const KernelSpec &kernel,
                          int compression, double epsilon, Operators *out);

void dense_m2m_matrix(const Operators &ops, int ci, std::vector<double> *out);

void thin_qr(const std::vector<double> &a, int m, int k, std::vector<double> *q,
             std::vector<double> *r);
void jacobi_svd(const std::vector<double> &a, int m, int k, std::vector<double> *u,
                std::vector<double> *s, std::vector<double> *vt);
int singular_values_cutoff(const std::vector<double> &sigma, double epsilon);

}
```

### ferreus_rbf_rs_amd/fmm_tree.py

```python
from __future__ import annotations

import ctypes
import enum
from typing import Optional

import numpy as np

from . import _lib as L


class KernelType(enum.IntEnum):
    LinearRbf = 0
    ThinPlateSplineRbf = 1
    CubicRbf = 2
    Spheroidal3Rbf = 3
    Spheroidal5Rbf = 4
    Spheroidal7Rbf = 5
    Spheroidal9Rbf = 6
    Laplacian = 7
    OneOverR2 = 8
    OneOverR4 = 9
    GaussianExt = 100
    MultiquadricExt = 101

# ... 549 lines not shown
        rc = self._lib.bbfmm_points_to_leaves(self._h, x.ctypes.data, m, max(m, 1),
                                              cells.ctypes.data, ctypes.byref(bad))
        self._raise(rc, bad)
        return cells[:m]

    def debug_dense_m2m(self, child_index: int):
        n = self.stats().n_nodes
        out = np.zeros((n, n), order="F")
        self._raise(self._lib.bbfmm_debug_dense_m2m(self._h, child_index, out.ctypes.data))
        return out

    def debug_m2l_variants(self):
        nv, nc = ctypes.c_int64(), ctypes.c_int64()
        self._raise(self._lib.bbfmm_debug_m2l_variants(self._h, ctypes.byref(nv), ctypes.byref(nc)))
        return nv.value, nc.value

    def debug_m2l_pairs(self, stage=1):
        fn = self._lib.bbfmm_debug_m2l_pairs if stage == 1 else self._lib.bbfmm_debug_m2l_pairs_stage2
        n, on = ctypes.c_int64(), ctypes.c_int32()
        self._raise(fn(self._h, None, 0, ctypes.byref(n), ctypes.byref(on)))
        buf = np.zeros(max(n.value, 1), dtype=np.int32)
        self._raise(fn(self._h, buf.ctypes.data, n.value, ctypes.byref(n), ctypes.byref(on)))
        d, ops, i = self.dim, [], 0
        while i < n.value:
            level, octant, kind, ne = (int(v) for v in buf[i:i + 4])
            ent = buf[i + 4:i + 4 + ne * (d + 1)].reshape(ne, d + 1)
            ops.append({"level": level, "octant": octant, "kind": kind,
                        "pairs": [tuple(int(x) for x in e[1:]) for e in ent if e[0] == 1],
                        "singles": [tuple(int(x) for x in e[1:]) for e in ent if e[0] == 0]})
            i += 4 + ne * (d + 1)
        return bool(on.value), ops

    def debug_m2l_pairs_axes(self, stage=1):
        if stage == 2:
            fn = self._lib.bbfmm_debug_m2l_pairs_axes_stage2
            n = ctypes.c_int64()
            self._raise(fn(self._h, None, 0, ctypes.byref(n)))
            buf = np.zeros(max(n.value, 1), dtype=np.int32)
            self._raise(fn(self._h, buf.ctypes.data, n.value, ctypes.byref(n)))
            info = {"axes": int(buf[0]), "work_x": int(buf[1]), "work_xy": int(buf[2])}
            d, ops, i = self.dim, [], 3
            while i < n.value:
                level, octant, kp, kpy, k_pad, pad, ne = (int(v) for v in buf[i:i + 7])
                ent = buf[i + 7:i + 7 + ne * (d + 4)].reshape(ne, d + 4)
                by_kind = [{tuple(int(x) for x in e[4:]): (int(e[1]), int(e[2]), int(e[3])) for e in ent if e[0] == k}
                           for k in range(3)]
                ops.append({"level": level, "octant": octant, "kp": kp, "kpy": kpy, "k_pad": k_pad, "pad": pad,
                            "singles": by_kind[0], "x_pairs": by_kind[1], "y_pairs": by_kind[2]})
                i += 7 + ne * (d + 4)
            return info, ops
        fn = self._lib.bbfmm_debug_m2l_pairs_axes
        n = ctypes.c_int64()
        self._raise(fn(self._h, None, 0, ctypes.byref(n)))
        buf = np.zeros(max(n.value, 1), dtype=np.int32)
        self._raise(fn(self._h, buf.ctypes.data, n.value, ctypes.byref(n)))
        info = {"axes": int(buf[0]), "work_x": int(buf[1]), "work_xy": int(buf[2])}
        d, ops, i = self.dim, [], 3
        while i < n.value:
            level, octant, kind, pad_cols, yb0, n_blk, ne = (int(v) for v in buf[i:i + 7])
            kinds = [int(v) for v in buf[i + 7:i + 7 + n_blk]]
            ent = buf[i + 7 + n_blk:i + 7 + n_blk + ne * (d + 3)].reshape(ne, d + 3)
            by_kind = [{tuple(int(x) for x in e[3:]): (int(e[1]), int(e[2])) for e in ent if e[0] == k} for k in range(3)]
            ops.append({"level": level, "octant": octant, "kind": kind, "pad_cols": pad_cols, "yb0": yb0, "block_kinds": kinds,
                        "singles": by_kind[0], "x_pairs": by_kind[1], "y_pairs": by_kind[2]})
            i += 7 + n_blk + ne * (d + 3)
        return info, ops

    M2L_DIGEST_FAMILIES = ("scalars", "partners_orbits", "class_lists", "class_rows", "class_cells", "tiles1", "tiles2", "batches")

    def debug_m2l_table_digests(self):
        n, nl = ctypes.c_int32(), ctypes.c_int32()
        self._raise(self._lib.bbfmm_debug_m2l_table_digests(self._h, None, 0, ctypes.byref(n), None, 0, ctypes.byref(nl)))
        assert n.value == len(self.M2L_DIGEST_FAMILIES)
        dig, fl = np.zeros(n.value, dtype=np.uint64), np.zeros(max(nl.value, 1))
        self._raise(self._lib.bbfmm_debug_m2l_table_digests(self._h, dig.ctypes.data, n.value, ctypes.byref(n), fl.ctypes.data,
                                                            nl.value, ctypes.byref(nl)))
        return {k: f"{int(v):016x}" for k, v in zip(self.M2L_DIGEST_FAMILIES, dig)}, [float(v) for v in fl[:nl.value]]

    def debug_m2l_s2_last_ksplit(self) -> int:
        ks = ctypes.c_int32()
        self._raise(self._lib.bbfmm_debug_m2l_s2_last_ksplit(self._h, ctypes.byref(ks)))
        return ks.value

    def debug_get_coefficients(self, which: str, k: int) -> np.ndarray:
        s = self.stats()
        n = s.n_nodes
        if which in ("P", "p"):
            ln = ctypes.c_int32(0)
            self._raise(self._lib.bbfmm_debug_m2l_parity_len(self._h, ctypes.byref(ln)))
            n = ln.value
        out = np.zeros((k, s.n_cells, n))
        self._raise(self._lib.bbfmm_debug_get_coefficients(self._h, which.encode()[0:1], k,
                                                           out.ctypes.data))
        return out

    def debug_apply_m2l_tables_host(self, M: np.ndarray) -> np.ndarray:
        M = np.ascontiguousarray(M, dtype=np.float64)
        Lc = np.zeros_like(M)
        self._raise(self._lib.bbfmm_debug_apply_m2l_tables_host(self._h, M.ctypes.data,
                                                                Lc.ctypes.data))
        return Lc


def make_grid(origin, steps, shape) -> L.Grid:
    origin = np.asarray(origin, dtype=np.float64).reshape(-1)
    d = origin.size
    steps = np.asarray(steps, dtype=np.float64)
    shape = [int(n) for n in np.asarray(shape).reshape(-1)]
    if not 1 <= d <= 3 or steps.shape != (d, d) or len(shape) != d:
        raise ValueError("a d-D grid needs an origin of d coordinates, (d, d) steps and d counts, d = 1..3")
    g = L.Grid()
    g.size, g.d = ctypes.sizeof(L.Grid), d
    for a in range(3):
        g.shape[a] = shape[a] if a < d else 1
    for j in range(d):
        g.origin[j] = origin[j]
        for a in range(d):
            g.steps[3 * j + a] = steps[j, a]
    return g


def debug_grid_coords(where: int, origin, steps, shape, r0: int, n: int) -> np.ndarray:
    g = make_grid(origin, steps, shape)
    out = np.zeros((n, g.d), order="F")
    rc = L.load().bbfmm_debug_grid_coords(int(where), ctypes.byref(g), int(r0), int(n), out.ctypes.data, max(n, 1))
    if rc != L.OK:
        raise (RuntimeError if rc == L.DEVICE_ERROR else ValueError)(f"bbfmm_debug_grid_coords failed with status {rc}")
    return out


def debug_split_runs(where: int, tgt_begin, tgt_end, job_cell, cap: int):
    tb = np.ascontiguousarray(tgt_begin, dtype=np.int32)
    te = np.ascontiguousarray(tgt_end, dtype=np.int32)
    jc = np.ascontiguousarray(job_cell, dtype=np.int32)
    if not tb.shape == te.shape == jc.shape or tb.ndim != 1:
        raise ValueError("one begin, end and cell per run")
    lib, n, nj = L.load(), tb.size, ctypes.c_int64(0)

    def check(rc):
        if rc != L.OK:
            raise (RuntimeError if rc == L.DEVICE_ERROR else ValueError)(f"bbfmm_debug_split_runs failed with status {rc}")

    check(lib.bbfmm_debug_split_runs(int(where), tb.ctypes.data, te.ctypes.data, jc.ctypes.data, n, int(cap), None, None, None, 0,
                                     ctypes.byref(nj)))
    ob, oe, oc = (np.zeros(max(nj.value, 1), dtype=np.int32) for _ in range(3))
    check(lib.bbfmm_debug_split_runs(int(where), tb.ctypes.data, te.ctypes.data, jc.ctypes.data, n, int(cap), ob.ctypes.data,
                                     oe.ctypes.data, oc.ctypes.data, nj.value, ctypes.byref(nj)))
    return ob[:nj.value], oe[:nj.value], oc[:nj.value]


def fp64_valu_selftest():
    tf, mhz = ctypes.c_double(0), ctypes.c_double(0)
    if L.load().bbfmm_fp64_valu_selftest(ctypes.byref(tf), ctypes.byref(mhz)) != L.OK:
        raise RuntimeError("the FP64 VALU microbenchmark needs a HIP device")
    return tf.value, mhz.value


def mfma_f64_selftest():
    tf = ctypes.c_double(0)
    errs = ctypes.c_int32(-1)
    info = (ctypes.c_double * 6)()
    rc = L.load().bbfmm_mfma_f64_selftest(ctypes.byref(tf), ctypes.byref(errs), info)
    if rc != L.OK:
        raise RuntimeError("MFMA self-test needs a HIP device")
    mfma_f64_selftest.info = dict(zip(["cycles_per_mfma_lone_wave", "clock_mhz_lone_wave",
                                       "cycles_per_mfma_per_simd_busy", "clock_mhz_busy",
# ... 26 lines not shown
```

### include/ferreus_bbfmm_hip.h

```cpp
#ifndef FERREUS_BBFMM_HIP_H
#define FERREUS_BBFMM_HIP_H

#include <stdint.h>

#ifdef __cplusplus
extern "C" {
#endif

typedef enum {
    BBFMM_OK = 0,
    BBFMM_POINT_OUTSIDE_TREE = 1,
    BBFMM_KERNEL_NO_GRADIENTS = 2,
    BBFMM_BAD_ARGUMENT = 3,
    BBFMM_DEVICE_ERROR = 4,
    BBFMM_UNSUPPORTED = 5,
    BBFMM_CALLBACK_FAILED = 6
} bbfmm_status;

typedef enum {
    BBFMM_KERNEL_LINEAR_RBF = 0,
    BBFMM_KERNEL_THIN_PLATE_SPLINE_RBF = 1,
    BBFMM_KERNEL_CUBIC_RBF = 2,
    BBFMM_KERNEL_SPHEROIDAL3_RBF = 3,
    BBFMM_KERNEL_SPHEROIDAL5_RBF = 4,
// ... 212 lines not shown

int bbfmm_matvec_device(bbfmm_handle *h, const double *d_w, int64_t ldw, int32_t k, double *d_out,
                        int64_t ldo, int32_t sync);

int bbfmm_target_subset_create(bbfmm_handle *h, const int64_t *target_indices, int64_t n_target_indices,
                               int32_t *subset_id);
int bbfmm_matvec_subset_device(bbfmm_handle *h, int32_t subset_id, const double *d_w, double *d_y, int32_t sync);

void *bbfmm_stream(bbfmm_handle *h);

int bbfmm_set_partition(bbfmm_handle *h, int32_t rank, int32_t world);
int64_t bbfmm_partition_row_count(const bbfmm_handle *h);
int bbfmm_partition_rows(const bbfmm_handle *h, int64_t *rows_out);

int64_t bbfmm_partition_coarse_count(const bbfmm_handle *h);
int bbfmm_matvec_partition_upward(bbfmm_handle *h, const double *d_w, int64_t ldw, int32_t k, double *d_coarse, void *comm_stream);
int bbfmm_matvec_partition_finish(bbfmm_handle *h, const double *d_coarse, double *d_out, int64_t ldo, int32_t sync, void *comm_stream);
int32_t bbfmm_partition_world(const bbfmm_handle *h);
int32_t bbfmm_partition_rank(const bbfmm_handle *h);
int bbfmm_partition_bounds(const bbfmm_handle *h, int32_t world, int64_t *bounds_out);
int bbfmm_matvec_partition_finish_sorted(bbfmm_handle *h, const double *d_coarse, double *d_seg, int64_t ld, void *comm_stream);
int bbfmm_partition_scatter(bbfmm_handle *h, const double *d_all, int32_t first_part, int32_t n_parts, int64_t m_max, int32_t k,
                            double *d_out, int64_t ldo);
int bbfmm_debug_partition_upward_counts(const bbfmm_handle *h, int64_t *counts_out, uint8_t *reads_out, int64_t *info_out);

int bbfmm_debug_host_copy_rates(int64_t n, double *out4);

typedef struct {
    int32_t d, order, n_nodes, depth;
    int64_t n_points, n_cells, n_leaves;
    int64_t n_u, n_v, n_w, n_x;
    int64_t p2p_pairs;
    int64_t p2p_tile_bytes_k1;
    double m2l_flops_k1;
    double center[3];
    double radius;
    int64_t wx_pairs;
    int64_t wx_tile_bytes_k1;
    int32_t m2l_basis_rank;
    int32_t m2l_basis_len;
    int32_t m2l_batches;
    int32_t m2l_rhs_per_pass;
    int64_t m2l_slots_bytes_per_rhs;
    int64_t m2l_intermediate_bytes;
} bbfmm_tree_stats;

int bbfmm_get_tree_stats(const bbfmm_handle *h, bbfmm_tree_stats *out);
int bbfmm_tree_built_on_device(const bbfmm_handle *h);

int bbfmm_get_cells(const bbfmm_handle *h, uint64_t *keys, uint8_t *is_leaf);
int bbfmm_get_leaf_sources(const bbfmm_handle *h, int64_t *ptr, int64_t *idx);
int bbfmm_get_list(const bbfmm_handle *h, char which, int64_t *ptr, int32_t *idx,
                   int64_t *n_entries);
int bbfmm_get_m2l_ranks(const bbfmm_handle *h, int32_t *ranks, int32_t *n_ref_out);
int bbfmm_get_m2l_operator(const bbfmm_handle *h, int32_t level, int32_t ref, double *out);
int bbfmm_get_m2l_factors(const bbfmm_handle *h, int32_t level, int32_t ref, double *u, double *vt);
int bbfmm_get_permutation_tables(const bbfmm_handle *h, int32_t *n_perm, int32_t *perm,
                                 int32_t *invperm, int32_t *perm_lookup, int32_t *ref_lookup);
int bbfmm_points_to_leaves(const bbfmm_handle *h, const double *x, int64_t m, int64_t ldx,
                           int32_t *cell_out, int64_t *bad_point_index);

#define BBFMM_N_PHASES 11
int bbfmm_set_profiling(bbfmm_handle *h, int32_t enable);
int bbfmm_get_phase_ms(bbfmm_handle *h, double *ms_out, int64_t *count_out);
int bbfmm_reset_phase_ms(bbfmm_handle *h);

int bbfmm_mfma_f64_selftest(double *tflops, int32_t *layout_errors, double *info6);
int bbfmm_fp64_valu_selftest(double *tflops, double *clock_mhz);

int bbfmm_debug_kernel_values(int32_t where, int32_t kernel_id, double base_range, double total_sill, const double *r2,
                              int64_t n, double *value_out, double *value_g_out, double *factor_out);
int bbfmm_debug_math(int32_t where, int32_t which, const double *x, int64_t n, double *out, double *out2);

int bbfmm_debug_dense_m2m(const bbfmm_handle *h, int32_t child_index, double *out);
int bbfmm_debug_apply_m2l_tables_host(const bbfmm_handle *h, const double *M, double *L);
int bbfmm_debug_m2l_variants(const bbfmm_handle *h, int64_t *n_variants, int64_t *n_cells);
int bbfmm_debug_m2l_pairs(const bbfmm_handle *h, int32_t *out, int64_t cap, int64_t *n_out, int32_t *pairs_on);
int bbfmm_debug_m2l_pairs_axes(const bbfmm_handle *h, int32_t *out, int64_t cap, int64_t *n_out);
int bbfmm_debug_m2l_pairs_stage2(const bbfmm_handle *h, int32_t *out, int64_t cap, int64_t *n_out, int32_t *pairs_on);
int bbfmm_debug_m2l_pairs_axes_stage2(const bbfmm_handle *h, int32_t *out, int64_t cap, int64_t *n_out);
int bbfmm_debug_m2l_table_digests(const bbfmm_handle *h, uint64_t *digests, int32_t cap, int32_t *n_out, double *flops_level,
                                  int32_t flops_cap, int32_t *n_levels_out);
int bbfmm_debug_m2l_s2_last_ksplit(const bbfmm_handle *h, int32_t *ksplit);

uint64_t bbfmm_debug_morton_encode(int32_t d, const uint64_t *anchor, uint64_t level);
void bbfmm_debug_morton_decode(int32_t d, uint64_t key, uint64_t *anchor_out, uint64_t *level_out);
int32_t bbfmm_debug_morton_neighbours(int32_t d, uint64_t key, uint64_t *keys_out);
int32_t bbfmm_debug_direction_vectors(int32_t d, int32_t *out);
int bbfmm_debug_reference_vectors(const bbfmm_handle *h, int32_t *out, int32_t *n_ref_out);

int bbfmm_debug_get_coefficients(bbfmm_handle *h, char which, int32_t k, double *out);
int bbfmm_debug_m2l_parity_len(const bbfmm_handle *h, int32_t *len);


typedef int (*bbfmm_apply_fn)(void *user, const double *x, double *y, int64_t n);
typedef void (*bbfmm_iteration_fn)(void *user, int64_t iter, double residual, double progress);

enum { BBFMM_ACCURACY_ABSOLUTE = 0, BBFMM_ACCURACY_RELATIVE = 1 };

void bbfmm_givens_rotation(double f, double g, double *c, double *s, double *r);

int bbfmm_fgmres(int64_t n, bbfmm_apply_fn a, void *a_user, const double *b, bbfmm_apply_fn m, void *m_user,
                 const double *x0, int32_t max_outer_iterations, int32_t max_inner_iterations,
                 int32_t tolerance_type, double tolerance, bbfmm_iteration_fn callback, void *cb_user,
                 double *x, int64_t *iterations, double *final_residual);

int bbfmm_schwarz_ddm_solver(int64_t n, bbfmm_apply_fn matvec, void *a_user, const double *rhs,
                             bbfmm_apply_fn m, void *m_user, int32_t max_iterations, int32_t tolerance_type,
                             double tolerance, bbfmm_iteration_fn callback, void *cb_user, double *x,
                             int64_t *iterations, double *final_residual);

typedef struct bbfmm_rbf_system {
    bbfmm_handle *tree;
    int64_t basis_size;
    const double *monomial_matrix;
    int64_t ld_monomial;
    double nugget;
} bbfmm_rbf_system;
int bbfmm_rbf_system_apply(void *user, const double *x, double *y, int64_t n);


typedef int (*bbfmm_apply_device_fn)(void *user, const double *d_x, double *d_y, int64_t n, void *stream);

typedef struct bbfmm_rbf_system_device bbfmm_rbf_system_device;
int bbfmm_rbf_system_device_create(bbfmm_handle *tree, int64_t basis_size, const double *monomial_matrix, int64_t ld,
                                   double nugget, bbfmm_rbf_system_device **out);
void bbfmm_rbf_system_device_destroy(bbfmm_rbf_system_device *s);
int bbfmm_rbf_system_apply_device(void *user, const double *d_x, double *d_y, int64_t n, void *stream);

int bbfmm_fgmres_device(int64_t n, bbfmm_apply_device_fn a, void *a_user, const double *d_b, bbfmm_apply_device_fn m,
                        void *m_user, const double *d_x0, int32_t max_outer_iterations, int32_t max_inner_iterations,
                        int32_t tolerance_type, double tolerance, bbfmm_iteration_fn callback, void *cb_user,
                        double *d_x, int64_t *iterations, double *final_residual, void *stream);

int bbfmm_schwarz_ddm_solver_device(int64_t n, bbfmm_apply_device_fn matvec, void *a_user, const double *d_rhs,
                                    bbfmm_apply_device_fn m, void *m_user, int32_t max_iterations,
                                    int32_t tolerance_type, double tolerance, bbfmm_iteration_fn callback,
                                    void *cb_user, double *d_x, int64_t *iterations, double *final_residual,
                                    void *stream);

int bbfmm_debug_solver_vector_op(int32_t op, int32_t alpha_mode, int64_t n, const double *a, const double *b,
                                 const double *c, double alpha, int32_t count, const double *coeffs, int32_t offset,
                                 double *out, double *scalars_out);

typedef struct bbfmm_ddm bbfmm_ddm;
typedef struct bbfmm_ddm_params {
    int64_t leaf_threshold;
    double overlap_quota;
    double coarse_ratio;
    int64_t coarse_threshold;
} bbfmm_ddm_params;
void bbfmm_ddm_params_defaults(bbfmm_ddm_params *out);
void bbfmm_ddm_params_for_points(int64_t n, bbfmm_ddm_params *out);
int bbfmm_ddm_build(const double *points, int64_t n, int32_t d, int64_t ld, const bbfmm_ddm_params *params,
                    bbfmm_ddm **out);
void bbfmm_ddm_destroy(bbfmm_ddm *t);
int32_t bbfmm_ddm_num_levels(const bbfmm_ddm *t);
int64_t bbfmm_ddm_level_size(const bbfmm_ddm *t, int32_t level);
int bbfmm_ddm_level_points(const bbfmm_ddm *t, int32_t level, int64_t *out);
int64_t bbfmm_ddm_num_domains(const bbfmm_ddm *t, int32_t level);
int64_t bbfmm_ddm_domain_size(const bbfmm_ddm *t, int32_t level, int64_t domain);
int bbfmm_ddm_domain(const bbfmm_ddm *t, int32_t level, int64_t domain, int64_t *indices, uint8_t *internal,
                     double *extents);

typedef struct bbfmm_schwarz bbfmm_schwarz;
typedef struct bbfmm_interpolant {
// ... 124 lines not shown
```

Measured before the change: 34.09 matvecs/s.

## Batch small contiguous leaves into L2P run blocks and fold Chebyshev scaling into q table

Adds a run-based L2P kernel that packs up to 8 consecutive small leaves (at most 256 targets) into one 256-thread block, so each thread handles one target and the leaves' local coefficients are staged in shared memory. Leaves that do not fit fall back to the existing per-leaf wave kernel. A precomputed q table folds the (2s-1)/P scaling of the Chebyshev interpolant into the coefficients, and divides by the cell half-length are replaced with one reciprocal multiply; both are shared by P2M and L2P. It also adds min-waves launch bounds to l2p_kernel. The intent is to stop small leaves leaving most lanes of a 64-lane wave idle, at the cost of host-side run construction and a second launch for the leftover leaves.

```diff
diff --git a/ferreus_rbf_rs_amd/_lib.py b/ferreus_rbf_rs_amd/_lib.py
--- a/ferreus_rbf_rs_amd/_lib.py
+++ b/ferreus_rbf_rs_amd/_lib.py
@@ -146,6 +146,7 @@
     "bbfmm_debug_m2l_pairs_axes_stage2": (ctypes.c_int, [c_p, c_p, c_i64, c_p]),
     "bbfmm_debug_m2l_table_digests": (ctypes.c_int, [c_p, c_p, c_i32, c_p, c_p, c_i32, c_p]),
     "bbfmm_debug_m2l_s2_last_ksplit": (ctypes.c_int, [c_p, c_p]),
+    "bbfmm_debug_leaf_runs": (ctypes.c_int, [c_p, c_p]),
     "bbfmm_debug_m2l_parity_len": (ctypes.c_int, [c_p, c_p]),
     "bbfmm_debug_get_coefficients": (ctypes.c_int, [c_p, ctypes.c_char, c_i32, c_p]),
     "bbfmm_debug_morton_encode": (ctypes.c_uint64, [c_i32, c_p, ctypes.c_uint64]),
diff --git a/ferreus_rbf_rs_amd/csrc/capi_debug.cpp b/ferreus_rbf_rs_amd/csrc/capi_debug.cpp
--- a/ferreus_rbf_rs_amd/csrc/capi_debug.cpp
+++ b/ferreus_rbf_rs_amd/csrc/capi_debug.cpp
@@ -239,6 +239,12 @@
     return BBFMM_OK;
 }
 
+int bbfmm_debug_leaf_runs(const bbfmm_handle *h, int32_t *counts) {
+    if (!h || !counts) return BBFMM_BAD_ARGUMENT;
+    h->tree.debug_leaf_runs(counts);
+    return BBFMM_OK;
+}
+
 int bbfmm_debug_m2l_parity_len(const bbfmm_handle *h, int32_t *len) {
     if (!h || !len) return BBFMM_BAD_ARGUMENT;
     *len = h->tree.debug_m2l_parity_len();
diff --git a/ferreus_rbf_rs_amd/csrc/device.hpp b/ferreus_rbf_rs_amd/csrc/device.hpp
--- a/ferreus_rbf_rs_amd/csrc/device.hpp
+++ b/ferreus_rbf_rs_amd/csrc/device.hpp
@@ -17,6 +17,7 @@
 struct DevCheb {
     int p, d, n, n_pad;
     double polyn[kMaxOrder * kMaxOrder];
+    double q[kMaxOrder * kMaxOrder];
     double nodes[kMaxOrder];
     double xfer[2 * kMaxOrder * kMaxOrder];
 };
@@ -205,11 +206,19 @@
                 const int64_t *run_ptr, const int32_t *runs, const double *centers,
                 const double *lengths, const double *const *src_xyz, const double *w_sorted,
                 int64_t N, int K, int64_t C, double *L, hipStream_t s);
+constexpr int kL2pRunLeaves = 8, kL2pRunTargets = 256, kL2pRunMaxNodes = 512;
+struct L2pRuns {
+    int n_runs = 0;
+    const int32_t *runs = nullptr;
+    int n_rest = 0;
+    const int32_t *rest_cell = nullptr, *rest_begin = nullptr, *rest_end = nullptr;
+};
+bool l2p_runs_supported(int p, int d);
 void launch_l2p(const ChebRef &ch, int n_jobs, const int32_t *leaf_cells, const int32_t *tgt_begin,
                 const int32_t *tgt_end, const double *centers, const double *lengths,
                 const double *const *tgt_xyz, int64_t n_tgt, int K, int64_t C, const double *L,
                 double *out_sorted, double *grad_sorted, hipStream_t s, const int32_t *perm = nullptr,
-                double *user_out = nullptr, int64_t ldo = 0);
+                double *user_out = nullptr, int64_t ldo = 0, const L2pRuns *runs = nullptr);
 
 bool l2p_order_supported(int p, int d);
 
diff --git a/ferreus_rbf_rs_amd/csrc/device_common.hpp b/ferreus_rbf_rs_amd/csrc/device_common.hpp
--- a/ferreus_rbf_rs_amd/csrc/device_common.hpp
+++ b/ferreus_rbf_rs_amd/csrc/device_common.hpp
@@ -22,7 +22,7 @@
 }
 
 template <int P, bool GRAD>
-__device__ inline void cheb_S_reg(double x, const double *__restrict__ polyn, double (&S)[P], double (&dS)[P]) {
+__device__ inline void cheb_S_reg(double x, const double *__restrict__ q, double (&S)[P], double (&dS)[P]) {
     double T[P], dT[P];
     T[0] = 1.0;
     dT[0] = 0.0;
@@ -37,15 +37,15 @@
     }
 #pragma unroll
     for (int j = 0; j < P; ++j) {
-        double s = 0.0, ds = 0.0;
+        double s = q[j * P], ds = 0.0;
 #pragma unroll
-        for (int k = 0; k < P; ++k) {
-            const double pk = polyn[j * P + k];
-            s += T[k] * pk;
-            if (GRAD) ds += dT[k] * pk;
+        for (int k = 1; k < P; ++k) {
+            const double qk = q[j * P + k];
+            s += T[k] * qk;
+            if (GRAD) ds += dT[k] * qk;
         }
-        S[j] = (s * 2.0 - 1.0) / (double)P;
-        dS[j] = GRAD ? ds * (2.0 / (double)P) : 0.0;
+        S[j] = s;
+        dS[j] = GRAD ? ds : 0.0;
     }
 }
 
diff --git a/ferreus_rbf_rs_amd/csrc/device_l2p.hip b/ferreus_rbf_rs_amd/csrc/device_l2p.hip
--- a/ferreus_rbf_rs_amd/csrc/device_l2p.hip
+++ b/ferreus_rbf_rs_amd/csrc/device_l2p.hip
@@ -5,8 +5,10 @@
 constexpr int L2P_WAVES = 4;
 template <int P, int D> constexpr int l2p_waves() { return D == 3 && P > 12 ? (P > 14 ? 1 : 2) : L2P_WAVES; }
 
+template <int P, bool GRAD> constexpr int l2p_min_waves() { return GRAD ? 1 : P <= 10 ? 4 : P == 11 ? 3 : P <= 14 ? 2 : 1; }
+
 template <int P, int D, bool GRAD>
-__global__ __launch_bounds__((64 * l2p_waves<P, D>())) void l2p_kernel(const DevCheb *__restrict__ chp, int n_jobs,
+__global__ __launch_bounds__((64 * l2p_waves<P, D>()), (l2p_min_waves<P, GRAD>())) void l2p_kernel(const DevCheb *__restrict__ chp, int n_jobs,
                                                              const int32_t *__restrict__ leaf_cells,
                                                              const int32_t *__restrict__ tgt_begin,
                                                              const int32_t *__restrict__ tgt_end,
@@ -21,18 +23,18 @@
     constexpr int WAVES = l2p_waves<P, D>();
     __shared__ double s_L[WAVES][N];
     const int tid = threadIdx.x, wave = tid >> 6, lane = tid & 63;
-    __shared__ double s_polyn_lds[GRAD ? P * P : 1];
+    __shared__ double s_q_lds[GRAD ? P * P : 1];
     if constexpr (GRAD) {
-        for (int i = tid; i < P * P; i += 64 * WAVES) s_polyn_lds[i] = chp->polyn[i];
+        for (int i = tid; i < P * P; i += 64 * WAVES) s_q_lds[i] = chp->q[i];
         __syncthreads();
     }
-    const double *__restrict__ s_polyn = GRAD ? s_polyn_lds : chp->polyn;
+    const double *__restrict__ s_q = GRAD ? s_q_lds : chp->q;
     const int job = blockIdx.x * WAVES + wave;
     if (job >= n_jobs) return;
     const int n_pad = chp->n_pad;
     const int cell = leaf_cells[job];
     const int b = tgt_begin[job], e = tgt_end[job];
-    const double len = lengths[cell];
+    const double r = 1.0 / (lengths[cell] * 0.5);
     const double cc[3] = {centers[cell * 3 + 0], centers[cell * 3 + 1], centers[cell * 3 + 2]};
     double *Lw = s_L[wave];
     for (int base = b; base < e; base += 64) {
@@ -40,12 +42,12 @@
         const bool valid = t < e;
         double S0[P], S1[P1], S2[P2], D0[P], D1[P1], D2[P2];
         {
-            const double x0 = valid ? (tgt.x[t] - cc[0]) / (len * 0.5) : 0.0;
-            cheb_S_reg<P, GRAD>(x0, s_polyn, S0, D0);
+            const double x0 = valid ? (tgt.x[t] - cc[0]) * r : 0.0;
+            cheb_S_reg<P, GRAD>(x0, s_q, S0, D0);
             if (D > 1) {
-                const double x1 = valid ? (tgt.y[t] - cc[1]) / (len * 0.5) : 0.0;
+                const double x1 = valid ? (tgt.y[t] - cc[1]) * r : 0.0;
                 double s[P], d[P];
-                cheb_S_reg<P, GRAD>(x1, s_polyn, s, d);
+                cheb_S_reg<P, GRAD>(x1, s_q, s, d);
 #pragma unroll
                 for (int j = 0; j < P1; ++j) { S1[j] = s[j]; D1[j] = d[j]; }
             } else {
@@ -53,9 +55,9 @@
                 D1[0] = 0.0;
             }
             if (D > 2) {
-                const double x2 = valid ? (tgt.z[t] - cc[2]) / (len * 0.5) : 0.0;
+                const double x2 = valid ? (tgt.z[t] - cc[2]) * r : 0.0;
                 double s[P], d[P];
-                cheb_S_reg<P, GRAD>(x2, s_polyn, s, d);
+                cheb_S_reg<P, GRAD>(x2, s_q, s, d);
 #pragma unroll
                 for (int j = 0; j < P2; ++j) { S2[j] = s[j]; D2[j] = d[j]; }
             } else {
@@ -63,7 +65,7 @@
                 D2[0] = 0.0;
             }
         }
-        const double gs = 2.0 / len;
+        const double gs = r;
         for (int k = 0; k < K; ++k) {
             const double *Lc = L + ((int64_t)k * C + cell) * n_pad;
             for (int I = lane; I < N; I += 64) Lw[I] = Lc[I];
@@ -140,13 +142,133 @@
 
 bool l2p_order_supported(int p, int d) { return p >= 2 && p <= kMaxOrder && d >= 1 && d <= 3; }
 
+template <int P, int D> constexpr bool l2p_runs_fit() { return (D == 1 ? P : D == 2 ? P * P : P * P * P) <= kL2pRunMaxNodes; }
+
+template <int P, int D>
+__global__ __launch_bounds__(kL2pRunTargets, 4) void l2p_runs_kernel(const DevCheb *__restrict__ chp, const int32_t *__restrict__ runs,
+                                                                 const int32_t *__restrict__ leaf_cells,
+                                                                 const int32_t *__restrict__ tgt_begin,
+                                                                 const int32_t *__restrict__ tgt_end,
+                                                                 const double *__restrict__ centers,
+                                                                 const double *__restrict__ lengths, Xyz tgt, int64_t n_tgt, int K,
+                                                                 int64_t C, const double *__restrict__ L, double *__restrict__ out,
+                                                                 const int32_t *__restrict__ perm, double *__restrict__ user_out,
+                                                                 int64_t ldo) {
+    constexpr int P1 = D > 1 ? P : 1, P2 = D > 2 ? P : 1, N = P * P1 * P2, S = N | 1;
+    __shared__ double s_L[kL2pRunLeaves * S];
+    __shared__ double s_geo[kL2pRunLeaves][4];
+    __shared__ int32_t s_bnd[kL2pRunLeaves + 1], s_cell[kL2pRunLeaves];
+    const int tid = threadIdx.x;
+    const double *__restrict__ s_q = chp->q;
+    const int first = runs[2 * blockIdx.x], n = min(runs[2 * blockIdx.x + 1], kL2pRunLeaves);
+    const int n_pad = chp->n_pad;
+    if (n < 1) return;
+    if (tid < n) {
+        const int job = first + tid, cell = leaf_cells[job];
+        s_cell[tid] = cell;
+        s_bnd[tid] = tgt_begin[job];
+        if (tid == n - 1) s_bnd[n] = tgt_end[job];
+        s_geo[tid][0] = centers[cell * 3 + 0];
+        s_geo[tid][1] = centers[cell * 3 + 1];
+        s_geo[tid][2] = centers[cell * 3 + 2];
+        s_geo[tid][3] = 1.0 / (lengths[cell] * 0.5);
+    }
+    __syncthreads();
+    const int t = s_bnd[0] + tid;
+    const bool valid = t < s_bnd[n];
+    int leaf = 0;
+#pragma unroll
+    for (int i = 1; i < kL2pRunLeaves; ++i) leaf += (i < n && t >= s_bnd[i]) ? 1 : 0;
+    double S0[P], S1[P1], S2[P2];
+    {
+        const double r = s_geo[leaf][3];
+        double dummy[P];
+        const double x0 = valid ? (tgt.x[t] - s_geo[leaf][0]) * r : 0.0;
+        cheb_S_reg<P, false>(x0, s_q, S0, dummy);
+        if (D > 1) {
+            const double x1 = valid ? (tgt.y[t] - s_geo[leaf][1]) * r : 0.0;
+            double s[P];
+            cheb_S_reg<P, false>(x1, s_q, s, dummy);
+#pragma unroll
+            for (int j = 0; j < P1; ++j) S1[j] = s[j];
+        } else {
+            S1[0] = 1.0;
+        }
+        if (D > 2) {
+            const double x2 = valid ? (tgt.z[t] - s_geo[leaf][2]) * r : 0.0;
+            double s[P];
+            cheb_S_reg<P, false>(x2, s_q, s, dummy);
+#pragma unroll
+            for (int j = 0; j < P2; ++j) S2[j] = s[j];
+        } else {
+            S2[0] = 1.0;
+        }
+    }
+    const double *Lw = s_L + leaf * S;
+    for (int k = 0; k < K; ++k) {
+        if (k) __syncthreads();
+        for (int idx = tid; idx < n * N; idx += kL2pRunTargets) {
+            const int i = idx / N, I = idx - i * N;
+            s_L[i * S + I] = L[((int64_t)k * C + s_cell[i]) * n_pad + I];
+        }
+        __syncthreads();
+        double y = 0.0;
+#pragma unroll
+        for (int a = 0; a < P; ++a) {
+            double ua = 0.0;
+#pragma unroll
+            for (int bb = 0; bb < P1; ++bb) {
+                double t0 = 0.0;
+#pragma unroll
+                for (int c = 0; c < P2; ++c) t0 += S2[c] * Lw[(a * P1 + bb) * P2 + c];
+                ua += S1[bb] * t0;
+            }
+            y += S0[a] * ua;
+        }
+        if (valid) {
+            if (perm) user_out[(int64_t)k * ldo + perm[t]] = out[(int64_t)k * n_tgt + t] + y;
+            else out[(int64_t)k * n_tgt + t] += y;
+        }
+    }
+}
+
+bool l2p_runs_supported(int p, int d) {
+    if (!l2p_order_supported(p, d)) return false;
+    int n = 1;
+    for (int a = 0; a < d; ++a) n *= p;
+    return n <= kL2pRunMaxNodes;
+}
+
+template <int P, int D>
+static void l2p_runs_launch_pd(const ChebRef &ch, const L2pRuns &r, const int32_t *leaf_cells, const int32_t *tgt_begin,
+                               const int32_t *tgt_end, const double *centers, const double *lengths, Xyz tgt, int64_t n_tgt, int K,
+                               int64_t C, const double *L, double *out_sorted, hipStream_t s, const int32_t *perm, double *user_out,
+                               int64_t ldo) {
+    if constexpr (l2p_runs_fit<P, D>())
+        hipLaunchKernelGGL((l2p_runs_kernel<P, D>), dim3(r.n_runs), dim3(kL2pRunTargets), 0, s, ch.dev, r.runs, leaf_cells, tgt_begin,
+                           tgt_end, centers, lengths, tgt, n_tgt, K, C, L, out_sorted, perm, user_out, ldo);
+}
+
 void launch_l2p(const ChebRef &ch, int n_jobs, const int32_t *leaf_cells, const int32_t *tgt_begin,
                 const int32_t *tgt_end, const double *centers, const double *lengths, const double *const *tgt_xyz,
                 int64_t n_tgt, int K, int64_t C, const double *L, double *out_sorted, double *grad_sorted,
-                hipStream_t s, const int32_t *perm, double *user_out, int64_t ldo) {
+                hipStream_t s, const int32_t *perm, double *user_out, int64_t ldo, const L2pRuns *runs) {
     if (n_jobs == 0) return;
     if (perm && grad_sorted) return;
     const Xyz tgt = make_xyz(tgt_xyz);
+    if (runs && runs->n_runs > 0 && !grad_sorted && l2p_runs_supported(ch.p, ch.d)) {
+        dispatch_order<2, 16>(ch.p, [&](auto pc) {
+            constexpr int P = decltype(pc)::value;
+            if (ch.d == 3) l2p_runs_launch_pd<P, 3>(ch, *runs, leaf_cells, tgt_begin, tgt_end, centers, lengths, tgt, n_tgt, K, C, L, out_sorted, s, perm, user_out, ldo);
+            else if (ch.d == 2) l2p_runs_launch_pd<P, 2>(ch, *runs, leaf_cells, tgt_begin, tgt_end, centers, lengths, tgt, n_tgt, K, C, L, out_sorted, s, perm, user_out, ldo);
+            else l2p_runs_launch_pd<P, 1>(ch, *runs, leaf_cells, tgt_begin, tgt_end, centers, lengths, tgt, n_tgt, K, C, L, out_sorted, s, perm, user_out, ldo);
+        });
+        n_jobs = runs->n_rest;
+        leaf_cells = runs->rest_cell;
+        tgt_begin = runs->rest_begin;
+        tgt_end = runs->rest_end;
+        if (n_jobs == 0) return;
+    }
     dispatch_order<2, 16>(ch.p, [&](auto pc) {
         l2p_launch_p<decltype(pc)::value>(ch, n_jobs, leaf_cells, tgt_begin, tgt_end, centers, lengths, tgt, n_tgt, K, C, L,
                                           out_sorted, grad_sorted, s, perm, user_out, ldo);
diff --git a/ferreus_rbf_rs_amd/csrc/device_p2m.hip b/ferreus_rbf_rs_amd/csrc/device_p2m.hip
--- a/ferreus_rbf_rs_amd/csrc/device_p2m.hip
+++ b/ferreus_rbf_rs_amd/csrc/device_p2m.hip
@@ -18,18 +18,18 @@
     constexpr int P1 = D > 1 ? P : 1, P2 = D > 2 ? P : 1, NPAIR = P1 * P2;
     constexpr int NPASS = (NPAIR + 63) / 64;
     constexpr int SROW = 3 * P + P2M_KB;
-    __shared__ double s_polyn[P * P];
+    __shared__ double s_q[P * P];
     constexpr int WAVES = p2m_waves<P, D>();
     __shared__ double s_pts[WAVES][P2M_PTS][SROW];
     const int tid = threadIdx.x, wave = tid >> 6, lane = tid & 63;
-    for (int i = tid; i < P * P; i += 64 * WAVES) s_polyn[i] = chp->polyn[i];
+    for (int i = tid; i < P * P; i += 64 * WAVES) s_q[i] = chp->q[i];
     __syncthreads();
     const int job = blockIdx.x * WAVES + wave;
     if (job >= n_leaves) return;
     const int n_pad = chp->n_pad;
     const int cell = leaf_cells[job];
     const int b = pt_begin[cell], e = pt_end[cell];
-    const double len = lengths[cell];
+    const double r = 1.0 / (lengths[cell] * 0.5);
     const double cc[3] = {centers[cell * 3 + 0], centers[cell * 3 + 1], centers[cell * 3 + 2]};
     double(*sp)[SROW] = s_pts[wave];
     for (int k0 = 0; k0 < K; k0 += P2M_KB) {
@@ -45,18 +45,18 @@
             if (lane < npts) {
                 const int pt = base + lane;
                 double S[P], dS[P];
-                cheb_S_reg<P, false>((src.x[pt] - cc[0]) / (len * 0.5), s_polyn, S, dS);
+                cheb_S_reg<P, false>((src.x[pt] - cc[0]) * r, s_q, S, dS);
 #pragma unroll
                 for (int jx = 0; jx < P; ++jx) sp[lane][jx] = S[jx];
                 if (D > 1) {
-                    cheb_S_reg<P, false>((src.y[pt] - cc[1]) / (len * 0.5), s_polyn, S, dS);
+                    cheb_S_reg<P, false>((src.y[pt] - cc[1]) * r, s_q, S, dS);
 #pragma unroll
                     for (int jx = 0; jx < P; ++jx) sp[lane][P + jx] = S[jx];
                 } else {
                     sp[lane][P] = 1.0;
                 }
                 if (D > 2) {
-                    cheb_S_reg<P, false>((src.z[pt] - cc[2]) / (len * 0.5), s_polyn, S, dS);
+                    cheb_S_reg<P, false>((src.z[pt] - cc[2]) * r, s_q, S, dS);
 #pragma unroll
                     for (int jx = 0; jx < P; ++jx) sp[lane][2 * P + jx] = S[jx];
                 } else {
@@ -115,13 +115,13 @@
     constexpr int SROW = 3 * P + 2;
     __shared__ double s_pts[P2M_WAVES][64][SROW];
     const int tid = threadIdx.x, wave = tid >> 6, lane = tid & 63;
-    const double *__restrict__ s_polyn = chp->polyn;
+    const double *__restrict__ s_q = chp->q;
     const int job = blockIdx.x * P2M_WAVES + wave;
     if (job >= n_leaves) return;
     const int n_pad = chp->n_pad;
     const int cell = leaf_cells[job];
     const int b = pt_begin[cell], e = pt_end[cell];
-    const double len = lengths[cell];
+    const double r = 1.0 / (lengths[cell] * 0.5);
     const double cc[3] = {centers[cell * 3 + 0], centers[cell * 3 + 1], centers[cell * 3 + 2]};
     double(*sp)[SROW] = s_pts[wave];
     const int hi = lane >> 4, blk = (lane >> 2) & 3, lo = lane & 3;
@@ -144,13 +144,13 @@
                 double S[P], dS[P];
                 const int pt = base + min(lane, npts - 1);
                 const bool live = lane < npts;
-                cheb_S_reg<P, false>((src.x[pt] - cc[0]) / (len * 0.5), s_polyn, S, dS);
+                cheb_S_reg<P, false>((src.x[pt] - cc[0]) * r, s_q, S, dS);
 #pragma unroll
                 for (int jx = 0; jx < P; ++jx) sp[lane][jx] = live ? S[jx] : 0.0;
-                cheb_S_reg<P, false>((src.y[pt] - cc[1]) / (len * 0.5), s_polyn, S, dS);
+                cheb_S_reg<P, false>((src.y[pt] - cc[1]) * r, s_q, S, dS);
 #pragma unroll
                 for (int jx = 0; jx < P; ++jx) sp[lane][P + jx] = live ? S[jx] : 0.0;
-                cheb_S_reg<P, false>((src.z[pt] - cc[2]) / (len * 0.5), s_polyn, S, dS);
+                cheb_S_reg<P, false>((src.z[pt] - cc[2]) * r, s_q, S, dS);
 #pragma unroll
                 for (int jx = 0; jx < P; ++jx) sp[lane][2 * P + jx] = live ? S[jx] : 0.0;
             }
diff --git a/ferreus_rbf_rs_amd/csrc/fmm_plans.cpp b/ferreus_rbf_rs_amd/csrc/fmm_plans.cpp
--- a/ferreus_rbf_rs_amd/csrc/fmm_plans.cpp
+++ b/ferreus_rbf_rs_amd/csrc/fmm_plans.cpp
@@ -36,7 +36,52 @@
     CHK(dupload(&ts.w_tgt_end, wte));
     CHK(dupload(&ts.w_begin, wb));
     CHK(dupload(&ts.w_end, we));
+    if ((leaf_mask_ & 1u) && l2p_runs_supported(cheb_.p, cheb_.d)) CHK(build_l2p_runs(&ts, jc, tb, te));
     CHK(build_sym_runs(&ts, jc, 0, t.n_points));
+    return BBFMM_OK;
+}
+
+int FmmTree::build_l2p_runs(TargetSet *ts, const std::vector<int32_t> &jc, const std::vector<int32_t> &tb,
+                            const std::vector<int32_t> &te) {
+    std::vector<int32_t> runs, rc, rb, re;
+    const int64_t nj = static_cast<int64_t>(jc.size());
+    int64_t first = 0, count = 0;
+    auto close = [&]() {
+        if (count >= 2) {
+            runs.push_back(static_cast<int32_t>(first));
+            runs.push_back(static_cast<int32_t>(count));
+        } else if (count == 1) {
+            rc.push_back(jc[static_cast<size_t>(first)]);
+            rb.push_back(tb[static_cast<size_t>(first)]);
+            re.push_back(te[static_cast<size_t>(first)]);
+        }
+        count = 0;
+    };
+    for (int64_t j = 0; j < nj; ++j) {
+        const size_t sj = static_cast<size_t>(j);
+        const int64_t size = static_cast<int64_t>(te[sj]) - tb[sj];
+        if (size < 0 || size > 64) {
+            close();
+            first = j;
+            count = 1;
+            close();
+            continue;
+        }
+        if (count > 0 && (tb[sj] != te[sj - 1] || count == kL2pRunLeaves ||
+                          static_cast<int64_t>(te[sj]) - tb[static_cast<size_t>(first)] > kL2pRunTargets))
+            close();
+        if (count == 0) first = j;
+        ++count;
+    }
+    close();
+    ts->n_l2p_runs = ts->n_l2p_rest = 0;
+    if (runs.empty() || static_cast<int64_t>(runs.size() / 2) < l2p_runs_min_) return BBFMM_OK;
+    ts->n_l2p_runs = static_cast<int>(runs.size() / 2);
+    ts->n_l2p_rest = static_cast<int>(rc.size());
+    CHK(dupload(&ts->l2p_runs, runs));
+    CHK(dupload(&ts->l2p_rest_cell, rc));
+    CHK(dupload(&ts->l2p_rest_begin, rb));
+    CHK(dupload(&ts->l2p_rest_end, re));
     return BBFMM_OK;
 }
 
@@ -504,6 +549,11 @@
     dfree(&ts->job_cell);
     dfree(&ts->tgt_begin);
     dfree(&ts->tgt_end);
+    dfree(&ts->l2p_runs);
+    dfree(&ts->l2p_rest_cell);
+    dfree(&ts->l2p_rest_begin);
+    dfree(&ts->l2p_rest_end);
+    ts->n_l2p_runs = ts->n_l2p_rest = 0;
     dfree(&ts->w_tgt_begin);
     dfree(&ts->w_tgt_end);
     dfree(&ts->w_begin);
diff --git a/ferreus_rbf_rs_amd/csrc/fmm_tree.cpp b/ferreus_rbf_rs_amd/csrc/fmm_tree.cpp
--- a/ferreus_rbf_rs_amd/csrc/fmm_tree.cpp
+++ b/ferreus_rbf_rs_amd/csrc/fmm_tree.cpp
@@ -357,6 +357,7 @@
     hc.n = ops_.n;
     hc.n_pad = round_up(ops_.n, 32);
     std::copy(ops_.polyn.begin(), ops_.polyn.end(), hc.polyn);
+    std::copy(ops_.q.begin(), ops_.q.end(), hc.q);
     std::copy(ops_.nodes.begin(), ops_.nodes.end(), hc.nodes);
     std::copy(ops_.xfer.begin(), ops_.xfer.end(), hc.xfer);
     CHK(dalloc(&d_cheb_, 1));
@@ -577,6 +578,13 @@
         const char *e = std::getenv("BBFMM_FUSED_PASSES");
         fused_mask_ = e ? static_cast<unsigned>(std::atoi(e)) & 15u : 15u;
         if (!(fused_mask_ & 2u)) fused_mask_ &= ~4u;
+        const char *lp = std::getenv("BBFMM_LEAF_PASSES");
+        leaf_mask_ = lp ? static_cast<unsigned>(std::atoi(lp)) & 1u : 1u;
+        int n_cu = 256, dev = 0;
+        if (hipGetDevice(&dev) != hipSuccess || hipDeviceGetAttribute(&n_cu, hipDeviceAttributeMultiprocessorCount, dev) != hipSuccess || n_cu <= 0)
+            n_cu = 256;
+        const char *rm = std::getenv("BBFMM_L2P_RUNS_MIN");
+        l2p_runs_min_ = rm ? std::max(0, std::atoi(rm)) : 4 * n_cu;
         std::vector<uint8_t> has_m2l(static_cast<size_t>(C), 0), has_x(static_cast<size_t>(C), 0);
         fused_flags_ok_ = true;
         for (const M2lTileDesc &td : m2l_tiles2_h_) {
@@ -1121,9 +1129,10 @@
 int FmmTree::leaf_pass_far(const TargetSet &ts, int k, bool with_grads, double *user_out, int64_t ldo) {
     const int64_t C = tree_.n_cells();
     double *grad = with_grads ? ts.grad.p : nullptr;
+    const L2pRuns runs{ts.n_l2p_runs, ts.l2p_runs.p, ts.n_l2p_rest, ts.l2p_rest_cell.p, ts.l2p_rest_begin.p, ts.l2p_rest_end.p};
     phase_begin();
     launch_l2p(cheb_, ts.n_jobs, ts.job_cell.p, ts.tgt_begin.p, ts.tgt_end.p, d_centers_.p, d_lengths_.p, ts.xyz_ptr,
-               ts.m, k, C, d_L_.p, ts.out.p, grad, stream_, user_out ? ts.perm.p : nullptr, user_out, ldo);
+               ts.m, k, C, d_L_.p, ts.out.p, grad, stream_, user_out ? ts.perm.p : nullptr, user_out, ldo, &runs);
     phase_end(kPhL2P);
     HIPCHK(hipGetLastError());
     return BBFMM_OK;
diff --git a/ferreus_rbf_rs_amd/csrc/fmm_tree.hpp b/ferreus_rbf_rs_amd/csrc/fmm_tree.hpp
--- a/ferreus_rbf_rs_amd/csrc/fmm_tree.hpp
+++ b/ferreus_rbf_rs_amd/csrc/fmm_tree.hpp
@@ -65,6 +65,8 @@
     DevBuf<int32_t> perm;
     DevBuf<int32_t> job_cell, tgt_begin, tgt_end;
     int n_jobs = 0;
+    int n_l2p_runs = 0, n_l2p_rest = 0;
+    DevBuf<int32_t> l2p_runs, l2p_rest_cell, l2p_rest_begin, l2p_rest_end;
     DevBuf<int32_t> w_tgt_begin, w_tgt_end;
     DevBuf<int64_t> w_begin, w_end;
     int n_w_jobs = 0;
@@ -222,6 +224,12 @@
     void debug_m2l_table_digests(std::vector<uint64_t> *out) const;
     const std::vector<double> &m2l_flops_level() const { return m2l_flops_level_; }
     int debug_m2l_s2_last_ksplit() const { return m2l_s2_last_ksplit_; }
+    void debug_leaf_runs(int32_t *counts) const {
+        counts[0] = static_cast<int32_t>(leaf_mask_);
+        counts[1] = src_targets_.n_l2p_runs;
+        counts[2] = src_targets_.n_l2p_rest;
+        counts[3] = src_targets_.n_jobs;
+    }
     int debug_apply_m2l_tables_host(const double *M, double *L) const;
     int debug_get_coefficients(char which, int k, double *out);
     int debug_m2l_parity_len() const { return m2l_pairs_ ? m2l_npar_ : 0; }
@@ -285,6 +293,7 @@
     int build_target_set_host(const double *x, int64_t m, int64_t ldx, TargetSet *ts, int64_t *bad_point_index,
                               std::vector<int32_t> *leaves_out);
     int build_source_target_set();
+    int build_l2p_runs(TargetSet *ts, const std::vector<int32_t> &jc, const std::vector<int32_t> &tb, const std::vector<int32_t> &te);
     int build_sym_runs(TargetSet *ts, const std::vector<int32_t> &job_cells, int64_t pb, int64_t pe, const std::vector<uint8_t> *part_active = nullptr);
     void free_target_set(TargetSet *ts);
     hipError_t columns_to_host(double *dst, int64_t ld, const double *d_src, int64_t m, int ncols);
@@ -367,6 +376,8 @@
     std::vector<int8_t> m2l_s2_sign_;
     std::vector<int8_t> m2l_s2_part_;
     unsigned fused_mask_ = 15;
+    unsigned leaf_mask_ = 1;
+    int l2p_runs_min_ = 1024;
     int mp_current_k_ = 0;
     bool lp_pending_ = false;
     bool fused_flags_ok_ = false;
diff --git a/ferreus_rbf_rs_amd/csrc/operators.cpp b/ferreus_rbf_rs_amd/csrc/operators.cpp
--- a/ferreus_rbf_rs_amd/csrc/operators.cpp
+++ b/ferreus_rbf_rs_amd/csrc/operators.cpp
@@ -337,6 +337,14 @@
     }
     o.polyn.resize(static_cast<size_t>(p) * p);
     for (int j = 0; j < p; ++j) cheb_T(p, o.nodes[j], &o.polyn[static_cast<size_t>(j) * p]);
+    o.q.resize(static_cast<size_t>(p) * p);
+    for (int j = 0; j < p; ++j) {
+        const long double theta = acosl(-1.0L) * (static_cast<long double>(p - 1 - j) + 0.5L) / static_cast<long double>(p);
+        for (int k = 0; k < p; ++k) {
+            const long double t2 = k == 0 ? 1.0L : 2.0L * cosl(static_cast<long double>(k) * theta);
+            o.q[static_cast<size_t>(j) * p + k] = static_cast<double>(t2 / static_cast<long double>(p));
+        }
+    }
     o.nodes_nd.resize(static_cast<size_t>(n) * d);
     for (int i = 0; i < n; ++i)
         for (int a = 0; a < d; ++a) o.nodes_nd[static_cast<size_t>(i) * d + a] = o.nodes[cart_index(i, a, p, d)];
diff --git a/ferreus_rbf_rs_amd/csrc/operators.hpp b/ferreus_rbf_rs_amd/csrc/operators.hpp
--- a/ferreus_rbf_rs_amd/csrc/operators.hpp
+++ b/ferreus_rbf_rs_amd/csrc/operators.hpp
@@ -18,6 +18,7 @@
     int p = 0, d = 0, n = 0;
     std::vector<double> nodes;
     std::vector<double> polyn;
+    std::vector<double> q;
     std::vector<double> nodes_nd;
     std::vector<double> xfer;
     int n_vec = 0;
diff --git a/ferreus_rbf_rs_amd/fmm_tree.py b/ferreus_rbf_rs_amd/fmm_tree.py
--- a/ferreus_rbf_rs_amd/fmm_tree.py
+++ b/ferreus_rbf_rs_amd/fmm_tree.py
@@ -655,6 +655,11 @@
         self._raise(self._lib.bbfmm_debug_m2l_s2_last_ksplit(self._h, ctypes.byref(ks)))
         return ks.value
 
+    def debug_leaf_runs(self) -> dict:
+        c = (ctypes.c_int32 * 4)()
+        self._raise(self._lib.bbfmm_debug_leaf_runs(self._h, c))
+        return {"mask": c[0], "runs": c[1], "rest": c[2], "jobs": c[3]}
+
     def debug_get_coefficients(self, which: str, k: int) -> np.ndarray:
         s = self.stats()
         n = s.n_nodes
diff --git a/include/ferreus_bbfmm_hip.h b/include/ferreus_bbfmm_hip.h
--- a/include/ferreus_bbfmm_hip.h
+++ b/include/ferreus_bbfmm_hip.h
@@ -318,6 +318,7 @@
 int bbfmm_debug_m2l_table_digests(const bbfmm_handle *h, uint64_t *digests, int32_t cap, int32_t *n_out, double *flops_level,
                                   int32_t flops_cap, int32_t *n_levels_out);
 int bbfmm_debug_m2l_s2_last_ksplit(const bbfmm_handle *h, int32_t *ksplit);
+int bbfmm_debug_leaf_runs(const bbfmm_handle *h, int32_t *counts);
 
 uint64_t bbfmm_debug_morton_encode(int32_t d, const uint64_t *anchor, uint64_t level);
 void bbfmm_debug_morton_decode(int32_t d, uint64_t key, uint64_t *anchor_out, uint64_t *level_out);
```

Measured after the change: 34.84 matvecs/s, median of 6. +2.2%, better.
